# ethanabrooks/hsr-env

Measured on AMD Instinct MI355X. Metric: env-steps/sec (whole node), HSR+1-block, steps_per_action=300, 8192 envs, higher is better.
Workload: dtype f32; 1 GPU; BASELINE config 3: cfg3, all 7 DOFs + 1 block(s), 8192 envs per GPU x 1 GPU(s), steps_per_action=300, geofence=0.05, ctrl~U(ctrlrange) per env-step, done envs reset; envs_per_gpu=8192, global_envs=8192, substeps_per_env_step=300, parallelism=env-shard x1, persistent_kernel=True, hipgraph=False

## Files before the change

### hsr_env_amd/csrc/host_access.h

```cpp

template <typename T>
static int read_drained(hsr_batch *b, T *out, T *src, size_t count, bool clear = false) {
    HIPCHK(hipStreamSynchronize(b->stream));
    HIPCHK(hipMemcpy(out, src, count * sizeof(T), hipMemcpyDeviceToHost));
    if (clear) HIPCHK(hipMemset(src, 0, count * sizeof(T)));
    return HSR_OK;
}
extern "C" int hsr_batch_size(const hsr_batch *b) { ENTER(b); return b->N; }
extern "C" void *hsr_batch_stream(const hsr_batch *b) { return b ? (void *)b->stream : nullptr; }
extern "C" int hsr_batch_sync(hsr_batch *b) { ENTER_DEV(b); HIPCHK(hipStreamSynchronize(b->stream)); return queue_error(b); }
extern "C" int hsr_batch_set_profiling(hsr_batch *b, int on) { ENTER(b); b->profiling = on == 1; b->kernel_log = on == 2; return HSR_OK; }
extern "C" int hsr_batch_kernel_times(hsr_batch *b, float *out_ms, int cap) {
    ENTER_DEV(b);
    HIPCHK(hipStreamSynchronize(b->stream));
    int n = 0;
    for (auto &pr : b->klog) {
        float ms = 0;
        if (hipEventElapsedTime(&ms, pr.first, pr.second) == hipSuccess && out_ms && n < cap) out_ms[n] = ms;
        n++;
        hipEventDestroy(pr.first); hipEventDestroy(pr.second);
    }
    b->klog.clear();
    const int qe = queue_error(b);
    return qe ? qe : n;
}
extern "C" int hsr_batch_set_graph(hsr_batch *b, int on) { ENTER(b); b->use_graph = on != 0; return HSR_OK; }
static void clear_margins(hsr_batch *b) {
    hipLaunchKernelGGL(k_clear_margins, grid1((size_t)b->ds.npair_sep * b->N), dim3(256), 0, b->stream, b->ds);
}
extern "C" int hsr_batch_set_persistent(hsr_batch *b, int on) {
    ENTER(b);
    const bool want = on != 0 && b->kernel;
    if (want && !b->persist) { hipSetDevice(b->device); clear_margins(b); }
    b->persist = want;
    return b->persist ? 1 : 0;
}
extern "C" int hsr_batch_is_persistent(const hsr_batch *b) {
    ENTER(b);
    if (!b->persist) return 0;
    return 1 | (b->const_row >= 0 ? 2 : 0) | (b->kin3 ? 4 : 0);
}
extern "C" int hsr_batch_set_debug(hsr_batch *b, int on) {
    ENTER(b);
    b->debug_store = (on & 1) != 0;
    b->test_hooks = on & (6 | 16 | 32 | 64 | 128);
    return HSR_OK;
}
extern "C" int hsr_batch_set_schedule(hsr_batch *b, int on) { ENTER(b); b->schedule = on != 0; return HSR_OK; }
extern "C" int hsr_batch_set_mpr_warm(hsr_batch *b, int on) {
    ENTER_DEV(b);
    if ((on != 0) != b->mpr_warm) clear_margins(b);
    b->mpr_warm = on != 0;
    return HSR_OK;
}
extern "C" int hsr_batch_set_solo(hsr_batch *b, int servers, float trips) {
    ENTER(b);
    if (servers < 0 || trips < 0.f) return fail(HSR_EINVAL, "hsr_batch_set_solo: servers >= 0, trips >= 0");
    b->solo_servers = servers;
    if (trips > 0.f) b->solo_trips = trips;
    return b->kernel_sv ? HSR_OK : 1;
}
extern "C" int hsr_batch_solo_handovers(hsr_batch *b, int *out) {
    ENTER_DEV(b);
    if (!out) return fail(HSR_EINVAL, "null argument");
    const int rc = read_drained(b, out, b->ds.sq_ctl + 1, 1);
    return rc ? rc : queue_error(b);
}
extern "C" int hsr_batch_set_queue(hsr_batch *b, int mode, int chunk) {
    ENTER(b);
    if (mode < -1 || mode > 1 || chunk < 0) return fail(HSR_EINVAL, "hsr_batch_set_queue: mode -1 / 0 / 1, chunk >= 0");
    b->queue = mode;
    if (chunk > 0) { b->queue_chunk = chunk; b->queue_chunk_set = true; }
    return HSR_OK;
}
extern "C" int hsr_batch_set_goals(hsr_batch *b, int n, const int *body_a, const int *body_b, const float *dist) {
    ENTER_DEV(b);
    if (n < 0 || n > 4 || (n > 0 && (!body_a || !body_b || !dist))) return fail(HSR_EINVAL, "hsr_batch_set_goals: 0..4 terms");
    for (int k = 0; k < n; k++)
        if (body_a[k] < 0 || body_a[k] >= b->dm.nbody || body_b[k] < 0 || body_b[k] >= b->dm.nbody) return fail(HSR_EINVAL, "hsr_batch_set_goals: body id out of range");
    HIPCHK(hipStreamSynchronize(b->stream));
    b->ds.ngoal = n;
    for (int k = 0; k < n; k++) { b->ds.goal_a[k] = body_a[k]; b->ds.goal_b[k] = body_b[k]; b->ds.goal_d[k] = dist[k]; }
    for (auto &kv : b->graphs) hipGraphExecDestroy(kv.second);
    b->graphs.clear();
    return HSR_OK;
}
extern "C" int hsr_batch_cap_counts(hsr_batch *b, unsigned long long *out) {
    ENTER_DEV(b);
    if (!out) return fail(HSR_EINVAL, "null argument");
    const int rc = read_drained(b, out, b->ds.capstat, 4, true);
    return rc ? rc : queue_error(b);
}
extern "C" int hsr_batch_cap_histogram(hsr_batch *b, unsigned long long *out) {
    ENTER_DEV(b);
    if (!out) return fail(HSR_EINVAL, "null argument");
    return read_drained(b, out, b->ds.capstat + 4, 8, true);
}

extern "C" int hsr_batch_newton_trips(hsr_batch *b, int32_t *out) {
    ENTER_DEV(b);
    if (!out) return fail(HSR_EINVAL, "null argument");
    return read_drained(b, out, b->ds.trips, (size_t)b->N);
}
extern "C" int hsr_batch_packing(hsr_batch *b, int32_t *out) {
    ENTER_DEV(b);
    if (!out) return fail(HSR_EINVAL, "null argument");
    if (!b->persist || !b->schedule || !b->d_slot_env) return fail(HSR_EINVAL, "hsr_batch_packing: no packed persistent launch on this batch");
    const int epb = 64 / b->group, slots = (b->N + epb - 1) / epb * epb;
    const int rc = read_drained(b, out, b->d_slot_env, (size_t)slots);
    return rc ? rc : queue_error(b);
}
static int to_device_soa(hsr_batch *b, float *dst, const float *host, int rows) {
    const size_t n = (size_t)rows * b->N;
    if (n > b->stage_floats) return fail(HSR_EINVAL, "staging overflow");
    HIPCHK(hipMemcpyAsync(b->d_stage, host, n * sizeof(float), hipMemcpyHostToDevice, b->stream));
    hipLaunchKernelGGL(k_aos_to_soa, grid1(n), dim3(256), 0, b->stream, dst, (const float *)b->d_stage, rows, b->N);
    HIPCHK(hipStreamSynchronize(b->stream));
    return HSR_OK;
}
static int to_host_aos(hsr_batch *b, float *host, const float *src, int rows) {
    const size_t n = (size_t)rows * b->N;
    if (n > b->stage_floats) return fail(HSR_EINVAL, "staging overflow");
    hipLaunchKernelGGL(k_soa_to_aos, grid1(n), dim3(256), 0, b->stream, b->d_stage, src, rows, b->N, rows, 0);
    return stage_to_host(b, host, b->d_stage, n);
}

extern "C" int hsr_batch_get_state(hsr_batch *b, float *time, float *qpos, float *qvel) {
    ENTER_DEV(b);
    int rc;
    if (time && (rc = to_host_aos(b, time, b->ds.time, 1))) return rc;
    if (qpos && (rc = to_host_aos(b, qpos, b->ds.qpos, b->dm.nq))) return rc;
    if (qvel && (rc = to_host_aos(b, qvel, b->ds.qvel, b->dm.nv))) return rc;
    return queue_error(b);
}
extern "C" int hsr_batch_set_state(hsr_batch *b, const float *time, const float *qpos, const float *qvel) {
    ENTER_DEV(b);
    clear_margins(b);
    int rc;
    if (time && (rc = to_device_soa(b, b->ds.time, time, 1))) return rc;
    if (qpos && (rc = to_device_soa(b, b->ds.qpos, qpos, b->dm.nq))) return rc;
    if (qvel && (rc = to_device_soa(b, b->ds.qvel, qvel, b->dm.nv))) return rc;
    return hsr_batch_forward(b);
}
extern "C" int hsr_batch_set_mocap(hsr_batch *b, const float *mocap) { ENTER_DEV(b); return to_device_soa(b, b->ds.mocap, mocap, 3); }
extern "C" int hsr_batch_set_warmstart(hsr_batch *b, const float *w) { ENTER_DEV(b); return to_device_soa(b, b->ds.warm, w, b->dm.nv); }
extern "C" int hsr_batch_get_warmstart(hsr_batch *b, float *w) { ENTER_DEV(b); return to_host_aos(b, w, b->ds.warm, b->dm.nv); }
extern "C" int hsr_batch_body_xpos(hsr_batch *b, int body_id, float *out) {
    ENTER_DEV(b);
    if (body_id < 0 || body_id >= b->dm.nbody) return fail(HSR_EINVAL, "body id out of range");
    hipLaunchKernelGGL(k_body_xpos, grid1(b->N), dim3(256), 0, b->stream, b->dm, b->ds, body_id, b->d_stage);
    return stage_to_host(b, out, b->d_stage, (size_t)b->N * 3);
}

static int obs_openai_launch(hsr_batch *b, const int *ids, float *d_out) {
    if (!ids) return fail(HSR_EINVAL, "null argument");
    const DevModel &d = b->dm;
    for (int k = 0; k < 3; k++) if (ids[k] < 0 || ids[k] >= d.nbody || b->model->i32("body_mocap")[ids[k]]) return fail(HSR_EINVAL, "obs_openai: bad body id");
    if (ids[3] < 0 || ids[3] >= d.nq || ids[4] < 0 || ids[4] >= d.nq || ids[5] < 0 || ids[5] >= d.nv || ids[6] < 0 || ids[6] >= d.nv)
        return fail(HSR_EINVAL, "obs_openai: bad joint address");
    hipLaunchKernelGGL(k_obs_openai, grid1(b->N), dim3(256), 0, b->stream, b->dm, b->ds, ids[0], ids[1], ids[2], ids[3], ids[4], ids[5], ids[6], d.timestep, d_out);
    HIPCHK(hipGetLastError());
    return HSR_OK;
}
extern "C" int hsr_batch_obs_openai_dev(hsr_batch *b, const int *ids, float *d_out) {
    ENTER_DEV(b);
    return obs_openai_launch(b, ids, d_out);
}
extern "C" int hsr_batch_obs_openai(hsr_batch *b, const int *ids, float *out) {
    ENTER_DEV(b);
    const int rc = obs_openai_launch(b, ids, b->d_stage);
    return rc ? rc : stage_to_host(b, out, b->d_stage, (size_t)b->N * 25);
}

extern "C" int hsr_batch_bad_state(hsr_batch *b, uint8_t *out) {
    ENTER_DEV(b);
    std::vector<int> tmp(b->N);
    const int rc = stage_to_host(b, tmp.data(), b->ds.bad, (size_t)b->N);
    if (rc) return rc;
    int any = 0;
    for (int i = 0; i < b->N; i++) { out[i] = (uint8_t)(tmp[i] != 0); any |= tmp[i]; }
    const int qe = queue_error(b);
    return qe ? qe : (any ? HSR_EBADSTATE : HSR_OK);
}

extern "C" int hsr_batch_get_field(hsr_batch *b, int field, float *out) {
    ENTER_DEV(b);
    const DevModel &d = b->dm;
    const size_t N = b->N;
    switch (field) {
    case HSR_F_XPOS: return to_host_aos(b, out, b->ds.xpos, 3 * d.nlink);
    case HSR_F_XMAT: return to_host_aos(b, out, b->ds.xmat, 9 * d.nlink);
    case HSR_F_QACC: return to_host_aos(b, out, b->ds.qacc, d.nv);
    case HSR_F_QACC_SMOOTH: return to_host_aos(b, out, b->ds.qacc_smooth, d.nv);
    case HSR_F_QFRC_SMOOTH: return to_host_aos(b, out, b->ds.qfrc_smooth, d.nv);
    case HSR_F_QFRC_CONSTRAINT: return to_host_aos(b, out, b->ds.qfrc_constraint, d.nv);
    case HSR_F_M:
        hipLaunchKernelGGL(k_expand_M, grid1(N), dim3(256), 0, b->stream, b->ds, b->d_stage, d.nv);
        return stage_to_host(b, out, b->d_stage, N * d.nv * d.nv);
    case HSR_F_NCON: case HSR_F_NEFC: case HSR_F_NITER: {
        const int *src = field == HSR_F_NCON ? b->ds.ncon : (field == HSR_F_NEFC ? b->ds.nefc : b->ds.niter);
        hipLaunchKernelGGL(k_i32_to_f32, grid1(N), dim3(256), 0, b->stream, b->d_stage, src, N);
        return stage_to_host(b, out, b->d_stage, N); }
    case HSR_F_CONTACT:
        hipLaunchKernelGGL(k_contacts_out, grid1(N), dim3(256), 0, b->stream, b->dm, b->ds, b->d_stage);
        return stage_to_host(b, out, b->d_stage, N * d.nslot * 7);
    default: return fail(HSR_EINVAL, "unknown field");
    }
}

extern "C" int hsr_batch_phase_cycles(hsr_batch *b, unsigned long long *out ) {
    ENTER_DEV(b);
    return read_drained(b, out, b->ds.phase_cyc, 32, true);
}

extern "C" int hsr_batch_block_times(hsr_batch *b, unsigned long long *out, int nblocks) {
    ENTER_DEV(b);
    if (nblocks > 8192) nblocks = 8192;
    if (nblocks < 0) return read_drained(b, out, b->ds.phase_cyc + 32 + 40 * 4096, (size_t)2 * 8192, true);
// ... 10 lines not shown
```

### hsr_env_amd/csrc/host_batch.h

```cpp
static_assert(HSR_GEOM_MESH == GEOM_MESH, "host_model.h restates model.h's GEOM_MESH");

#define HIPCHK(x) do { hipError_t e_ = (x); if (e_ != hipSuccess) return fail(HSR_EDEVICE, "HIP error: %s", hipGetErrorString(e_)); } while (0)
#define ENTER(b) do { if (!(b)) return fail(HSR_EINVAL, "null batch"); } while (0)
#define ENTER_DEV(b) do { ENTER(b); HIPCHK(hipSetDevice((b)->device)); } while (0)

typedef void (*persist_fn)(const DevModel *, DevState, int, int, float, int, StepIO);
struct GraphKey {
    int nsub, goal_body; float geofence; int cap_every, cap_n; const void *cap;
    bool operator<(const GraphKey &o) const { return std::tie(nsub, goal_body, geofence, cap_every, cap_n, cap) < std::tie(o.nsub, o.goal_body, o.geofence, o.cap_every, o.cap_n, o.cap); }
};

struct CreateSwitches {
    bool no_const = false;
    int nfb_max = 1 << 30;
    bool tables_lds = false;
    bool debug = false;
};

struct hsr_batch {
    const hsr_model *model = nullptr;
    CreateSwitches sw;
    int N = 0, device = 0;
    hipStream_t stream = nullptr;
    DevModel dm{};
    DevModel *d_dm = nullptr;
    DevState ds{};
    std::vector<void *> allocs;
    float *d_qpos0 = nullptr;
    float *d_stage = nullptr;
    size_t stage_floats = 0;
    uint8_t *d_stage_u8 = nullptr;
    int32_t *d_stage_i32 = nullptr;
    int narrow_blocks = 2048;
    int pairs_per_wave = 4;
    int group = 16;
    size_t mf_lds_bytes = 0;
    bool persist = false;
    bool use_graph = true, profiling = false, debug_store = false;
    int const_row = -1;
    bool kin3 = false;
    bool persist_tg = false;
    persist_fn kernel = nullptr;
    persist_fn kernel_sv = nullptr;
    size_t persist_lds_bytes = 0;
    bool mpr_warm = true;
    int test_hooks = 0;
    bool schedule = true;
    int *d_slot_env = nullptr;
    std::map<GraphKey, hipGraphExec_t> graphs;
    float last_total_ms = 0, last_kernel_ms[3] = {0, 0, 0};
    int last_launches[3] = {0, 0, 0};
    hipEvent_t ev0 = nullptr, ev1 = nullptr;
    std::vector<hipEvent_t> kev;
    int slots = 0;
    int queue = -1;
    int queue_chunk = 20;
    bool queue_chunk_set = false;
    int solo_servers = 0;
    float solo_trips = 3.5f;
    bool kernel_log = false;
    std::vector<std::pair<hipEvent_t, hipEvent_t>> klog;
    float4 *d_planes = nullptr;
    int2 *d_prange = nullptr;
    float4 *d_rgba = nullptr;
    std::vector<float> rgba_host;
    void *d_rimg = nullptr;
    size_t rimg_bytes = 0;
    int cap_every = 0, cap_n = 0;
    CaptureDesc *d_cap_desc = nullptr;
    int *d_cap_slot = nullptr;
    int *d_cap_env = nullptr;
    int *d_cap_cnt = nullptr;
    float *d_cap = nullptr;
    size_t cap_floats = 0;
    int cap_rows = 0;
    EpisodeDev ep{};
    bool ep_set = false;
    float *d_ep_range = nullptr;
    int *d_ep_block_qadr = nullptr;
    std::vector<hsr_snapshot *> snapshots;
    hsr_snapshot *fork_scratch = nullptr;
    SnapTable snap_tab{};
    bool snap_tab_built = false;
    std::vector<hsr_replay *> replays;
    std::vector<hsr_rollout *> rollouts;
};
static void snap_release_all(hsr_batch *b);
static void replay_release_all(hsr_batch *b);
static void rollout_release_all(hsr_batch *b);
template <typename T>
static int dalloc(hsr_batch *b, T **p, size_t count) {
    void *q = nullptr;
    HIPCHK(hipMalloc(&q, (count ? count : 1) * sizeof(T)));
    HIPCHK(hipMemset(q, 0, (count ? count : 1) * sizeof(T)));
    b->allocs.push_back(q);
    *p = (T *)q;
    return HSR_OK;
}
template <typename D, typename T>
static int upload(hsr_batch *b, D *dst, const T *src, size_t count, size_t pad = 0) {
    T *d;
    const int rc = dalloc(b, &d, count + pad);
    if (rc) return rc;
    if (count) HIPCHK(hipMemcpy(d, src, count * sizeof(T), hipMemcpyHostToDevice));
    *dst = (D)d;
    return HSR_OK;
}
template <typename D, typename T>
static int upload(hsr_batch *b, D *dst, const std::vector<T> &v, size_t pad = 0) { return upload(b, dst, v.data(), v.size(), pad); }
template <typename T>
static int stage_to_host(hsr_batch *b, T *host, const T *d_src, size_t count) {
    HIPCHK(hipMemcpyAsync(host, d_src, count * sizeof(T), hipMemcpyDeviceToHost, b->stream));
    HIPCHK(hipStreamSynchronize(b->stream));
    return HSR_OK;
}
template <typename F>
static auto by_group(int group, F f) { return group == 16 ? f(std::integral_constant<int, 16>()) : f(std::integral_constant<int, 32>()); }
static int upload_capture_desc(hsr_batch *b, int every, int n) {
    const CaptureDesc cd{b->d_cap, b->d_cap_slot, every, n};
    HIPCHK(hipMemcpy(b->d_cap_desc, &cd, sizeof cd, hipMemcpyHostToDevice));
    return HSR_OK;
}
static int require_captured_step(const hsr_batch *b, const char *who) {
    if (b->cap_every <= 0 || b->cap_rows <= 0) return fail(HSR_EINVAL, "%s: no captured step (hsr_batch_set_capture, then a step)", who);
    return HSR_OK;
}
enum { QUEUE_ROUNDS = 64 };
static inline dim3 grid1(size_t n, int t = 256) { return dim3((unsigned)((n + t - 1) / t)); }
static int queue_error(hsr_batch *b) {
    int err = 0;
    if (b->ds.q_err && hipMemcpy(&err, b->ds.q_err, sizeof err, hipMemcpyDeviceToHost) == hipSuccess && err) {
        hipMemset(b->ds.q_err, 0, sizeof err);
        return fail(HSR_EDEVICE, "persistent kernel: a work-queue ticket was never served (launch drained by its watchdog)");
    }
    return HSR_OK;
}
```

### hsr_env_amd/csrc/host_create.h

```cpp

static void read_switches(hsr_batch *b) {
    auto env = [](const char *name) { const char *v = getenv(name); return v ? v : ""; };
    auto is0 = [&](const char *name) { return strcmp(env(name), "0") == 0; };
    auto set = [&](const char *name) { return getenv(name) != nullptr; };
    b->sw.no_const = set("HSR_NO_CONST") && !is0("HSR_NO_CONST");
    if (set("HSR_NFB")) b->sw.nfb_max = std::max(atoi(env("HSR_NFB")), 0);
    b->sw.tables_lds = is0("HSR_TABLES_GLOBAL");
    b->sw.debug = set("HSR_DEBUG");
    if (set("HSR_SOLO")) b->solo_servers = atoi(env("HSR_SOLO"));
    if (atof(env("HSR_SOLO_TRIPS")) > 0) b->solo_trips = (float)atof(env("HSR_SOLO_TRIPS"));
    if (set("HSR_QUEUE")) b->queue = atoi(env("HSR_QUEUE")) != 0;
    if (atoi(env("HSR_QUEUE_CHUNK")) > 0) b->queue_chunk = atoi(env("HSR_QUEUE_CHUNK"));
    b->queue_chunk_set = atoi(env("HSR_QUEUE_CHUNK")) > 0;
    if (set("HSR_MPR_WARM")) b->mpr_warm = atoi(env("HSR_MPR_WARM")) != 0;
    b->schedule = !is0("HSR_SCHEDULE");
    if (atoi(env("HSR_NARROW_BLOCKS")) > 0) b->narrow_blocks = atoi(env("HSR_NARROW_BLOCKS"));
    if (atoi(env("HSR_PPW")) > 0) b->pairs_per_wave = atoi(env("HSR_PPW"));
}

struct PersistInstance {
    int row;
    int group, nv;
    bool tg;
    persist_fn fn, sv;
};
static const PersistInstance kPersistInstances[] = {
#ifdef HSR_DEV_CFG3
    {2, 16, -1, false, k_env_step_mf<16, 13, true, 7, false, DevModel_cfg3>, k_env_step_mf<16, 13, true, 7, false, DevModel_cfg3, true>},
#else
    {0, 16, -1, false, k_env_step_mf<16, 2, true, 0, false, DevModel_cfg1>, nullptr},
    {1, 16, -1, false, k_env_step_mf<16, 8, true, 0, false, DevModel_cfg2>, k_env_step_mf<16, 8, true, 0, false, DevModel_cfg2, true>},
    {2, 16, -1, false, k_env_step_mf<16, 13, true, 7, false, DevModel_cfg3>, k_env_step_mf<16, 13, true, 7, false, DevModel_cfg3, true>},
    {3, 32, -1, false, k_env_step_mf<32, 25, true, 7, false, DevModel_cfg4>, nullptr},
    {3, 32, -1, true, k_env_step_mf<32, 25, true, 7, true, DevModel_cfg4>, nullptr},
    {4, 16, -1, false, k_env_step_mf<16, 13, true, -1, false, DevModel_cupboard>, k_env_step_mf<16, 13, true, -1, false, DevModel_cupboard, true>},
    {4, 16, -1, true, k_env_step_mf<16, 13, true, -1, true, DevModel_cupboard>, k_env_step_mf<16, 13, true, -1, true, DevModel_cupboard, true>},
    {-1, 16, 13, false, k_env_step_mf<16, 13, true>, nullptr},
    {-1, 16, -1, false, k_env_step_mf<16, 16, false>, nullptr},
    {-1, 32, -1, false, k_env_step_mf<32, 32, false>, nullptr},
#endif
};
static const PersistInstance *find_instance(int row, int group, int nv, bool tg) {
    for (const PersistInstance &p : kPersistInstances)
        if (p.row == row && p.group == group && (p.nv < 0 || p.nv == nv) && p.tg == tg) return &p;
    return nullptr;
}
static void quat2mat_h(const double *q, float *mt) {
    double n = sqrt(q[0]*q[0] + q[1]*q[1] + q[2]*q[2] + q[3]*q[3]);
    double w = q[0]/n, x = q[1]/n, y = q[2]/n, z = q[3]/n;
    mt[0] = (float)(1 - 2*(y*y + z*z)); mt[1] = (float)(2*(x*y - w*z)); mt[2] = (float)(2*(x*z + w*y));
    mt[3] = (float)(2*(x*y + w*z)); mt[4] = (float)(1 - 2*(x*x + z*z)); mt[5] = (float)(2*(y*z - w*x));
    mt[6] = (float)(2*(x*z - w*y)); mt[7] = (float)(2*(y*z + w*x)); mt[8] = (float)(1 - 2*(x*x + y*y));
}
static int cfg_const_row(const hsr_batch *b, const hsr_model *m, const DevModel &d) {
    if (b->sw.no_const) return -1;
    int iv[sizeof kCfgConsts[0].i / sizeof(int)]; float fv[sizeof kCfgConsts[0].f / sizeof(float)];
    cfg_const_values(d, iv, fv);
    int r = 0;
    const int nrows = (int)(sizeof kCfgConsts / sizeof kCfgConsts[0]);
    while (r < nrows && !(memcmp(iv, kCfgConsts[r].i, sizeof iv) == 0 && memcmp(fv, kCfgConsts[r].f, sizeof fv) == 0)) r++;
    if (r == nrows) return -1;
    const Kin3Check &k = kKin3Checks[r];
    if (!k.i) return r;
    std::vector<int> ti = {d.nlink, d.nv};
    for (const char *n : {"link_parent", "link_free", "link_dofadr", "link_dofnum", "link_qposadr", "dof_type", "dof_qposadr", "dof_link"}) {
        size_t cnt = 0; const int *p = m->i32(n, &cnt);
        ti.insert(ti.end(), p, p + cnt);
    }
    std::vector<float> tf;
    auto addf = [&](const char *n) { size_t cnt = 0; const double *p = m->f64(n, &cnt); for (size_t i = 0; i < cnt; i++) tf.push_back((float)p[i]); };
    addf("link_pos");
    { size_t cnt = 0; const double *q = m->f64("link_quat", &cnt); for (size_t i = 0; i < cnt / 4; i++) { float mt[9]; quat2mat_h(q + 4 * i, mt); tf.insert(tf.end(), mt, mt + 9); } }
    for (const char *n : {"link_com", "link_inertia", "link_mass", "dof_axis", "dof_pos"}) addf(n);
    return k.ni == (int)ti.size() && k.nf == (int)tf.size() && memcmp(k.i, ti.data(), ti.size() * sizeof(int)) == 0
           && memcmp(k.f, tf.data(), tf.size() * sizeof(float)) == 0 ? r : -1;
}
static int upload_f(hsr_batch *b, const float **dst, const hsr_model *m, const char *name) {
    size_t cnt = 0;
    const double *src = m->f64(name, &cnt);
    if (!src) return fail(HSR_EBLOB, "blob entry '%s' missing", name);
    std::vector<float> tmp(cnt ? cnt : 1, 0.f);
    for (size_t i = 0; i < cnt; i++) tmp[i] = (float)src[i];
    return upload(b, dst, tmp);
}
static int upload_i(hsr_batch *b, const int **dst, const hsr_model *m, const char *name) {
    size_t cnt = 0;
    const int *src = m->i32(name, &cnt);
    if (!src) return fail(HSR_EBLOB, "blob entry '%s' missing", name);
    return upload(b, dst, src, cnt, 16);
}
static int upload_mats(hsr_batch *b, const float **dst, const hsr_model *m, const char *quat_name) {
    size_t cnt = 0;
    const double *q = m->f64(quat_name, &cnt);
    if (!q) return fail(HSR_EBLOB, "blob entry '%s' missing", quat_name);
    size_t n = cnt / 4;
    std::vector<float> tmp(n * 9 + 1);
    for (size_t i = 0; i < n; i++) quat2mat_h(q + 4 * i, tmp.data() + 9 * i);
    return upload(b, dst, tmp);
}

static int trailing_free_bodies(const hsr_batch *b, const hsr_model *m) {
    const DevModel &d = b->dm;
    const int *dn = m->i32("link_dofnum"), *lf = m->i32("link_free"), *da = m->i32("link_dofadr"), *dt = m->i32("dof_type"), *dl = m->i32("dof_link");
    int nfb = 0;
    for (int k = 0; 6 * (k + 1) <= d.nv; k++) {
        const int a0 = d.nv - 6 * (k + 1), l = dl[a0];
        bool fb = l > 0 && lf[l] && da[l] == a0 && dn[l] == 6;
        for (int j = 0; fb && j < 6; j++) fb = dl[a0 + j] == l && dt[a0 + j] == (j < 3 ? DOF_FREE_LIN : DOF_FREE_ANG);
        if (!fb) break;
        nfb++;
    }
    if (nfb * 28 * (64 / b->group) > 4 * 48) nfb = 0;
    return std::min(nfb, b->sw.nfb_max);
}
static int stage_hulls(hsr_batch *b, const hsr_model *m) {
    DevModel &d = b->dm;
    const int *gl = m->i32("geom_link"), *gt = m->i32("geom_type"), *ma = m->i32("geom_meshadr"), *mn = m->i32("geom_meshnum"), *lp = m->i32("link_parent");
    std::vector<int> ldsv(std::max(d.ngeom, 1), -1), src;
    if (b->kin3) {
        const int budget = KIN2_FLOATS * d.nlink / 4;
        auto depth = [&](int l) { int k = 0; while (l > 0) { l = lp[l]; k++; } return k; };
        std::vector<int> order;
        for (int g = 0; g < d.ngeom; g++) if (gt[g] == GEOM_MESH && gl[g] > 0 && mn[g] > 0) order.push_back(g);
        std::stable_sort(order.begin(), order.end(), [&](int a, int bb) { const int da = depth(gl[a]), db = depth(gl[bb]); return da != db ? da > db : mn[a] < mn[bb]; });
        for (int g : order) if ((int)src.size() + mn[g] <= budget) { ldsv[g] = (int)src.size(); for (int k = 0; k < mn[g]; k++) src.push_back(ma[g] + k); }
    }
    d.nldsv = (int)src.size();
    const int rc = upload(b, &d.geom_ldsv, ldsv);
    return rc ? rc : upload(b, &d.ldsv_src, src, 1);
}
static bool fits_persist(const hsr_batch *b, const hsr_model *m) {
    const DevModel &d = b->dm;
    const int G = b->group;
    bool ok = d.nq <= G && d.nv <= G && d.nlink <= G && d.nlink <= NLMAX && d.ngeom <= 64 && d.npair < (1 << 14) && d.maxdepth <= 9;
    {
        const int *dp = m->i32("dof_parent");
        for (int c = 0; ok && c < d.nv; c++) { int depth = 0; for (int k = c; k >= 0 && depth <= 10; k = dp[k]) depth++; if (depth > 10) ok = false; }
    }
    {
        const int *dn = m->i32("link_dofnum"), *lf = m->i32("link_free"), *lp = m->i32("link_parent"), *gl = m->i32("geom_link");
        for (int l = 1; l < d.nlink; l++) {
            if (!lf[l] && dn[l] > 3) ok = false;
            if (lf[l] && lp[l] != 0) ok = false;
            if (lf[lp[l]]) ok = false;
        }
        for (int gi = d.nstatic_geom; gi < d.ngeom; gi++) if (gl[gi] == 0) ok = false;
    }
    return ok && b->persist_lds_bytes <= 160 * 1024;
}
static int plan_persist(hsr_batch *b, const hsr_model *m) {
    DevModel &d = b->dm;
    const int G = b->group;
    auto layout = [&](auto g, bool tg) {
        return PersistLayout<decltype(g)::value>(d.njmax, b->ds.kstride, d.npair_pad, d.nlink, d.ngeom, d.nstatic_geom, tg);
    };
    d.nfb = trailing_free_bodies(b, m);
    int row = cfg_const_row(b, m, d);
    if (row >= 0 && kKin3Checks[row].i) {
        const int *lf = m->i32("link_free"), *dl = m->i32("dof_link");
        int nrd = 0;
        for (int k = 0; k < d.nv; k++) nrd += lf[dl[k]] ? 0 : 1;
        const int stage = 12 * d.nv + ((nrd + 3) & ~3) * nrd;
        const int region = by_group(G, [&](auto g) { return layout(g, false).oCnt; });
        if (stage > region) row = -1;
    }
    b->const_row = row;
    b->kin3 = row >= 0 && kKin3Checks[row].i;
    const int rc = stage_hulls(b, m);
    if (rc) return rc;
    auto lds_total = [&](bool tg) { return (size_t)sizeof(float) * by_group(G, [&](auto g) { return layout(g, tg).total; }); };
    const PersistInstance *in_lds = find_instance(row, G, d.nv, false), *in_global = find_instance(row, G, d.nv, true);
    hipFuncAttributes fa;
    b->persist_tg = in_lds && in_global && !b->sw.tables_lds
                    && hipFuncGetAttributes(&fa, (const void *)in_lds->fn) == hipSuccess && lds_total(false) + fa.sharedSizeBytes > 20480
                    && hipFuncGetAttributes(&fa, (const void *)in_global->fn) == hipSuccess && lds_total(true) + fa.sharedSizeBytes <= 20480;
    b->persist_lds_bytes = lds_total(b->persist_tg);
    const PersistInstance *inst = b->persist_tg ? in_global : in_lds;
    if (!fits_persist(b, m) || !inst) { d.nfb = 0; return HSR_OK; }
    b->kernel = inst->fn;
    b->kernel_sv = inst->sv;
    b->persist = true;
    for (persist_fn f : {b->kernel, b->kernel_sv})
        if (f && b->persist_lds_bytes > 48 * 1024) HIPCHK(hipFuncSetAttribute((const void *)f, hipFuncAttributeMaxDynamicSharedMemorySize, (int)b->persist_lds_bytes));
    int pb = -1;
    hipDeviceProp_t prop;
    if (hipOccupancyMaxActiveBlocksPerMultiprocessor(&pb, b->kernel, 64, b->persist_lds_bytes) == hipSuccess && pb > 0
        && hipGetDeviceProperties(&prop, b->device) == hipSuccess) b->slots = pb * prop.multiProcessorCount;
    if (b->sw.debug && hipFuncGetAttributes(&fa, (const void *)b->kernel) == hipSuccess)
        fprintf(stderr, "[hsrsim] k_env_step_mf<%d>: regs %d, static LDS %zu, dyn LDS %zu, scratch %zu -> %d workgroups per CU\n", G, fa.numRegs, fa.sharedSizeBytes, b->persist_lds_bytes, fa.localSizeBytes, pb);
    return HSR_OK;
}

static int upload_model(hsr_batch *b, const hsr_model *m) {
    DevModel &d = b->dm;
    const int *sz = m->sizes;
    d.nq = sz[HSR_NQ]; d.nv = sz[HSR_NV]; d.nu = sz[HSR_NU]; d.nlink = sz[HSR_NLINK]; d.nbody = sz[HSR_NBODY];
    d.ngeom = sz[HSR_NGEOM]; d.npair = sz[HSR_NPAIR]; d.nslot = sz[HSR_NSLOT]; d.nconmax = sz[HSR_NCONMAX]; d.njmax = sz[HSR_NJMAX];
    if (d.npair > 384) return fail(HSR_EINVAL, "more than 384 candidate geom pairs");
    if (d.ngeom > 255) return fail(HSR_EINVAL, "more than 255 geoms");
    d.nM = d.nv * (d.nv + 1) / 2;
    d.ndense = sz[13];
    d.timestep = (float)m->opt[0]; d.impratio = (float)m->opt[1]; d.gravz = (float)m->opt[2]; d.tolerance = (float)m->opt[3];
    d.iterations = (int)m->opt[4]; d.ls_iterations = (int)m->opt[5]; d.ls_tolerance = (float)m->opt[6];
    d.mpr_tolerance = (float)m->opt[7]; d.mpr_iterations = (int)m->opt[8]; d.meaninertia = (float)m->opt[9];
    int rc = 0;
#define UI(f) if ((rc = upload_i(b, &d.f, m, #f))) { return rc; }
#define UF(f) if ((rc = upload_f(b, &d.f, m, #f))) { return rc; }
    UI(link_parent) UI(link_dofadr) UI(link_dofnum) UI(link_qposadr) UI(link_free)
    UF(link_pos) UF(link_mass) UF(link_com) UF(link_inertia) UI(link_dofmask)
    UI(dof_link) UI(dof_type) UI(dof_parent) UI(dof_qposadr) UI(dof_limited)
    UF(dof_axis) UF(dof_pos) UF(dof_damping) UF(dof_invweight0) UF(dof_range) UF(dof_solref) UF(dof_solimp)
    UI(body_link) UI(body_mocap) UF(body_pos)
    UI(geom_type) UI(geom_link) UI(geom_meshadr) UI(geom_meshnum)
    UF(geom_pos) UF(geom_size) UF(geom_rbound) UF(geom_invweight) UF(mesh_vert) UF(geom_aabb)
    UI(pair_geom1) UI(pair_geom2) UI(pair_fn) UI(pair_condim) UI(pair_slot)
    UF(pair_friction) UF(pair_solref) UF(pair_solimp)
    UI(act_dof) UF(act_gear) UF(act_kp) UF(act_ctrlrange) UF(act_forcerange)
#undef UI
#undef UF
    return HSR_OK;
}
static int derive_pair_rec(hsr_batch *b, const hsr_model *m) {
    DevModel &d = b->dm;
    const int *g1 = m->i32("pair_geom1"), *g2 = m->i32("pair_geom2"), *cd = m->i32("pair_condim"), *gl = m->i32("geom_link"), *ad = m->i32("act_dof");
    const double *fr = m->f64("pair_friction"), *sr = m->f64("pair_solref"), *si = m->f64("pair_solimp"), *iw = m->f64("geom_invweight");
    std::vector<float> rec((size_t)std::max(d.npair, 1) * 16, 0.f);
    for (int p = 0; p < d.npair; p++) {
        float *r = rec.data() + 16 * p;
        r[0] = (float)cd[p]; r[1] = (float)gl[g1[p]]; r[2] = (float)gl[g2[p]]; r[3] = (float)(iw[2 * g1[p]] + iw[2 * g2[p]]);
        for (int j = 0; j < 5; j++) r[4 + j] = (float)fr[5 * p + j];
        const double dmax = std::min(std::max(si[5 * p + 1], (double)HSR_MINIMP), (double)HSR_MAXIMP), tc = sr[2 * p], dr = sr[2 * p + 1];
        r[9] = (float)(2.0 / (dmax * tc)); r[10] = (float)(1.0 / (dmax * dmax * tc * tc * dr * dr));
        for (int j = 0; j < 5; j++) r[11 + j] = (float)si[5 * p + j];
    }
    std::vector<int> da(std::max(d.nv, 1), -1);
    for (int a = 0; a < d.nu; a++) da[ad[a]] = a;
    const int rc = upload(b, &d.pair_rec, rec);
    return rc ? rc : upload(b, &d.dof_act, da);
}
static int derive_collision_recs(hsr_batch *b, const hsr_model *m) {
    DevModel &d = b->dm;
    const int *g1 = m->i32("pair_geom1"), *g2 = m->i32("pair_geom2"), *fn = m->i32("pair_fn"), *sl = m->i32("pair_slot");
    const int *gl = m->i32("geom_link"), *gt = m->i32("geom_type"), *ma = m->i32("geom_meshadr"), *mn = m->i32("geom_meshnum");
    const double *gp = m->f64("geom_pos"), *gq = m->f64("geom_quat"), *gs = m->f64("geom_size"), *gb = m->f64("geom_aabb"), *gr = m->f64("geom_rbound");
    std::vector<float> rec((size_t)std::max(d.npair, 1) * 8, 0.f), grec((size_t)std::max(d.ngeom, 1) * 32, 0.f);
    for (int p = 0; p < d.npair; p++) {
        float *r = rec.data() + 8 * p;
        r[0] = (float)(g1[p] + 256 * (gt[g1[p]] == GEOM_PLANE ? 1 : 0)); r[1] = (float)g2[p]; r[2] = (float)gr[g1[p]]; r[3] = (float)gr[g2[p]];
        r[4] = (float)fn[p]; r[5] = (float)sl[p]; r[6] = (float)(sl[p + 1] - sl[p]); r[7] = (float)gt[g1[p]];
    }
    for (int gg = 0; gg < d.ngeom; gg++) {
        float *o = grec.data() + 32 * gg, lm[9];
        quat2mat_h(gq + 4 * gg, lm);
        o[0] = (float)gl[gg]; o[1] = (float)gt[gg]; o[2] = (float)mn[gg]; o[3] = (float)ma[gg];
        for (int k = 0; k < 3; k++) o[4 + k] = (float)gp[3 * gg + k];
        o[7] = (float)gr[gg];
        for (int k = 0; k < 9; k++) o[8 + k] = lm[k];
        for (int k = 0; k < 3; k++) o[17 + k] = (float)gs[3 * gg + k];
        for (int k = 0; k < 3; k++) { o[20 + k] = (float)gb[6 * gg + k]; o[24 + k] = (float)gb[6 * gg + 3 + k]; }
    }
    const int rc = upload(b, &d.pair_geo, rec);
    return rc ? rc : upload(b, &d.geom_rec, grec);
}
static int derive_tables(hsr_batch *b, const hsr_model *m) {
    DevModel &d = b->dm;
    int rc = 0;
    {
        const int *lp = m->i32("link_parent");
        std::vector<int> dep(std::max(d.nlink, 1), 0);
        d.maxdepth = 0;
        for (int l = 1; l < d.nlink; l++) { dep[l] = dep[lp[l]] + 1; d.maxdepth = std::max(d.maxdepth, dep[l]); }
        if ((rc = upload(b, &d.link_depth, dep))) return rc;
    }
    {
        size_t cnt = 0;
        const double *mv = m->f64("mesh_vert", &cnt);
        const size_t nvt = cnt / 3;
        std::vector<float> v4((nvt + 1) * 4, 0.f);
        for (size_t i = 0; i < nvt; i++) for (int k = 0; k < 3; k++) v4[4 * i + k] = (float)mv[3 * i + k];
        if ((rc = upload(b, &d.mesh_vert4, v4))) return rc;
        const int *mn = m->i32("geom_meshnum");
        for (int g = 0; g < d.ngeom; g++) if (mn[g] > 256) return fail(HSR_EINVAL, "mesh hull with more than 256 vertices");
    }
    {
        const int *gl = m->i32("geom_link");
        d.nstatic_geom = 0;
        while (d.nstatic_geom < d.ngeom && gl[d.nstatic_geom] == 0) d.nstatic_geom++;
    }
    d.npair_pad = (d.npair + 7) & ~7;
    if (d.npair_pad == 0) d.npair_pad = 8;
    if ((rc = derive_pair_rec(b, m)) || (rc = derive_collision_recs(b, m))) return rc;
    if ((rc = upload_mats(b, &d.link_mat, m, "link_quat"))) return rc;
    if ((rc = upload_mats(b, &d.geom_mat, m, "geom_quat"))) return rc;
    if ((rc = upload_mats(b, &d.body_mat, m, "body_quat"))) return rc;
    d.any_damping = 0;
    { size_t cnt; const double *dmp = m->f64("dof_damping", &cnt); for (size_t i = 0; i < cnt; i++) if (dmp[i] > 0) d.any_damping = 1; }
    d.solimp_general = 0;
    for (const char *nm : {"dof_solimp", "pair_solimp"}) {
        size_t cnt; const double *si = m->f64(nm, &cnt);
        for (size_t i = 4; si && i < cnt; i += 5) { const double pw = si[i] < 1 ? 1 : si[i]; if (pw != 1 && pw != 2) d.solimp_general = 1; }
    }
    d.cv_types = 0;
    {
        const int *g1 = m->i32("pair_geom1"), *g2 = m->i32("pair_geom2"), *fn = m->i32("pair_fn"), *gt = m->i32("geom_type");
        for (int p = 0; p < d.npair; p++) if (fn[p] == FN_CONVEX) d.cv_types |= (1 << (gt[g1[p]] & 7)) | (256 << (gt[g2[p]] & 7));
    }
    return HSR_OK;
}
static int alloc_state(hsr_batch *b) {
    const DevModel &d = b->dm;
    DevState &s = b->ds;
    const size_t N = (size_t)b->N;
    int rc = 0;
    s.N = b->N;
    s.npair_sep = std::max(d.npair, 1);
#define DA(field, rows) if ((rc = dalloc(b, &s.field, (size_t)(rows) * N))) return rc;
    DA(qpos, d.nq) DA(qvel, d.nv) DA(ctrl, d.nu) DA(mocap, 3) DA(warm, d.nv) DA(time, 1)
    DA(done, 1) DA(bad, 1) DA(nsteps, 1)
    DA(xpos, 3 * d.nlink) DA(xmat, 9 * d.nlink) DA(lvel, 6 * d.nlink)
    s.kstride = (9 * d.nv + 15 * d.nlink + 15) & ~15;
    DA(kin_aos, s.kstride)
    DA(con, 8 * d.nslot) DA(ncon_pair, d.npair_pad) DA(sepax, 4 * std::max(d.npair, 1)) DA(septick, std::max(d.npair, 1)) DA(tick, 1) DA(pair_list, std::max(d.npair, 1))
    if ((rc = dalloc(b, &s.pair_count, (size_t)d.npair_pad))) return rc;
    if ((rc = dalloc(b, &s.pair_pack, (size_t)((d.npair_pad + 7) & ~7)))) return rc;
    if ((rc = dalloc(b, &s.geom_c, (size_t)8 * std::max(d.ngeom, 1)))) return rc;
    DA(M, d.nM) DA(qacc, d.nv) DA(qacc_smooth, d.nv) DA(qfrc_smooth, d.nv) DA(qfrc_constraint, d.nv)
    DA(ncon, 1) DA(nefc, 1) DA(niter, 1)
#undef DA
    if ((rc = dalloc(b, &s.phase_cyc, 32 + 40 * 8192))) return rc;
    if ((rc = dalloc(b, &s.capstat, 12))) return rc;
    if ((rc = dalloc(b, &s.trips, N))) return rc;
    if ((rc = dalloc(b, &b->d_slot_env, N + 64))) return rc;
    const size_t tasks = (N + 1) / 2;
    if ((rc = dalloc(b, &s.q_head, QUEUE_ROUNDS))) return rc;
    if ((rc = dalloc(b, &s.q_wpos, QUEUE_ROUNDS))) return rc;
    if ((rc = dalloc(b, &s.q_items, (size_t)QUEUE_ROUNDS * tasks))) return rc;
    if ((rc = dalloc(b, &s.q_err, 1))) return rc;
    s.sq_cap = (int)N + 4096;
    if ((rc = dalloc(b, &s.sq_items, (size_t)s.sq_cap))) return rc;
    if ((rc = dalloc(b, &s.sq_ctl, 4))) return rc;
    s.solo_servers = 0; s.solo_trips_x4 = 14; s.solo_min_left = 40;
    s.q_chunk = 0;
    s.slot_env = nullptr;
    return HSR_OK;
}
static int size_solver(hsr_batch *b) {
    const DevModel &d = b->dm;
    b->group = d.nv <= 16 ? 16 : 32;
    if (d.nv > 32 || d.nq > 64 || d.nlink > NLMAX || d.nconmax > b->group || b->ds.kstride > 8 * 4 * b->group)
        return fail(HSR_EINVAL, "model exceeds the lane-group solver (nv <= 32, nlink <= 16, nconmax <= lanes per env)");
    const int total = by_group(b->group, [&](auto g) { return MfLayout<decltype(g)::value>(d.njmax, b->ds.kstride).total; });
    b->mf_lds_bytes = (size_t)total * (64 / b->group) * sizeof(float);
    if (b->mf_lds_bytes > 160 * 1024) return fail(HSR_EINVAL, "model exceeds the LDS budget of the solver");
    if (b->mf_lds_bytes <= 48 * 1024) return HSR_OK;
    const void *fn = by_group(b->group, [](auto g) { return (const void *)k_solve_mf<decltype(g)::value>; });
    HIPCHK(hipFuncSetAttribute(fn, hipFuncAttributeMaxDynamicSharedMemorySize, (int)b->mf_lds_bytes));
    return HSR_OK;
}
static int size_kinematics(hsr_batch *b) {
    const size_t kb = (size_t)64 * (b->ds.kstride + 24 * b->dm.nlink + 1) * sizeof(float);
    if (kb > 160 * 1024) return fail(HSR_EINVAL, "kinematics tile exceeds LDS");
    if (kb > 48 * 1024) HIPCHK(hipFuncSetAttribute((const void *)k_kinematics, hipFuncAttributeMaxDynamicSharedMemorySize, (int)kb));
    return HSR_OK;
}
static int alloc_staging_and_reset(hsr_batch *b, const hsr_model *m) {
    const DevModel &d = b->dm;
    const size_t N = (size_t)b->N;
    int rc = 0;
    b->stage_floats = N * (size_t)(std::max(std::max(std::max(d.nq + d.nv, 25), 7 * d.nslot), std::max(d.nv * d.nv, 9 * d.nlink)) + d.nu + d.nq + d.nv + 4) + 16;
    if ((rc = dalloc(b, &b->d_stage, b->stage_floats))) return rc;
    if ((rc = dalloc(b, &b->d_stage_u8, N))) return rc;
    if ((rc = dalloc(b, &b->d_stage_i32, N))) return rc;
    HIPCHK(hipEventCreate(&b->ev0));
    HIPCHK(hipEventCreate(&b->ev1));
    if ((rc = upload(b, &b->d_qpos0, m->qpos0.data(), (size_t)d.nq))) return rc;
    hipLaunchKernelGGL(k_build_tables, grid1((size_t)std::max(d.ngeom, (d.npair_pad + 7) & ~7)), dim3(256), 0, b->stream, b->dm, b->ds);
    hipLaunchKernelGGL(k_reset, grid1(N), dim3(256), 0, b->stream, b->dm, b->ds, (const uint8_t *)nullptr, (const float *)nullptr,
                       (const float *)b->d_qpos0, (const float *)nullptr, 0);
    HIPCHK(hipStreamSynchronize(b->stream));
    return HSR_OK;
}

static int batch_init(hsr_batch *b, const hsr_model *m) {
    int rc;
    HIPCHK(hipStreamCreateWithFlags(&b->stream, hipStreamNonBlocking));
    if ((rc = upload_model(b, m)) || (rc = derive_tables(b, m)) || (rc = alloc_state(b)) || (rc = size_solver(b))) return rc;
    if ((rc = plan_persist(b, m)) || (rc = size_kinematics(b))) return rc;
    return alloc_staging_and_reset(b, m);
}
extern "C" int hsr_batch_create(const hsr_model *m, int n_envs, int device_id, hsr_batch **out) {
    if (!m || !out || n_envs <= 0) return fail(HSR_EINVAL, "bad arguments to hsr_batch_create");
    int ndev = 0;
    if (hipGetDeviceCount(&ndev) != hipSuccess || ndev <= 0) return fail(HSR_EDEVICE, "no HIP device available%s");
    if (device_id < 0 || device_id >= ndev) return fail(HSR_EINVAL, "device id out of range");
    HIPCHK(hipSetDevice(device_id));
    hsr_batch *b = new hsr_batch();
    b->model = m; b->N = n_envs; b->device = device_id;
    read_switches(b);
    const int rc = batch_init(b, m);
    if (rc) { hsr_batch_destroy(b); return rc; }
    *out = b;
    return HSR_OK;
}

extern "C" void hsr_batch_destroy(hsr_batch *b) {
    if (!b) return;
    hipSetDevice(b->device);
    if (b->stream) hipStreamSynchronize(b->stream);
    for (auto &kv : b->graphs) hipGraphExecDestroy(kv.second);
    snap_release_all(b);
    replay_release_all(b);
    rollout_release_all(b);
    for (void *p : b->allocs) hipFree(p);
    if (b->d_rimg) hipFree(b->d_rimg);
    if (b->d_cap) hipFree(b->d_cap);
    for (hipEvent_t ev : b->kev) hipEventDestroy(ev);
    for (auto &pr : b->klog) { hipEventDestroy(pr.first); hipEventDestroy(pr.second); }
    if (b->ev0) hipEventDestroy(b->ev0);
    if (b->ev1) hipEventDestroy(b->ev1);
    if (b->stream) hipStreamDestroy(b->stream);
    delete b;
}
```

### hsr_env_amd/csrc/host_step.h

```cpp

static void launch_substep(hsr_batch *b, int mode, int goal_body, float geofence, int debug, hipStream_t st, bool timed, int sub = -1) {
    const int N = b->N;
    auto rec = [&](void) { if (timed) { hipEvent_t ev; hipEventCreate(&ev); hipEventRecord(ev, st); b->kev.push_back(ev); } };
    rec();
    hipLaunchKernelGGL(k_kinematics, dim3((N + 63) / 64), dim3(64), (size_t)64 * (b->ds.kstride + 24 * b->dm.nlink + 1) * sizeof(float), st, b->dm, b->ds);
    if (sub >= 0 && b->cap_every > 0 && sub % b->cap_every == 0)
        hipLaunchKernelGGL(k_capture, grid1((size_t)12 * b->dm.nlink * b->cap_n), dim3(256), 0, st, b->ds, b->dm.nlink, (const int *)b->d_cap_env, b->cap_n, b->d_cap,
                           sub / b->cap_every, 1, b->cap_every, (int *)nullptr);
    rec();
    if (b->dm.npair > 0) {
        hipLaunchKernelGGL(k_cull, dim3((N + 63) / 64, (b->dm.npair + b->pairs_per_wave - 1) / b->pairs_per_wave), dim3(64), 0, st, b->dm, b->ds);
        hipLaunchKernelGGL(k_narrow, dim3(b->narrow_blocks), dim3(64), 0, st, b->dm, b->ds);
    }
    rec();
    by_group(b->group, [&](auto g) {
        hipLaunchKernelGGL(k_solve_mf<decltype(g)::value>, dim3((N * g() + 63) / 64), dim3(64), b->mf_lds_bytes, st, b->dm, b->ds,
                           mode, goal_body, geofence, debug);
    });
    rec();
}

extern "C" int hsr_batch_forward(hsr_batch *b) {
    ENTER_DEV(b);
    hipLaunchKernelGGL(k_clear_done, grid1(b->N), dim3(256), 0, b->stream, b->ds);
    launch_substep(b, 0, -1, 0.f, 1, b->stream, false);
    HIPCHK(hipGetLastError());
    HIPCHK(hipStreamSynchronize(b->stream));
    return HSR_OK;
}

extern "C" int hsr_batch_reset(hsr_batch *b, const uint8_t *mask, const float *qpos0, const float *mocap) {
    ENTER_DEV(b);
    const size_t N = b->N;
    const int nq = b->dm.nq;
    float *d_q = nullptr, *d_m = nullptr, *d_q0m = b->d_qpos0;
    size_t off = 0;
    if (qpos0) { d_q = b->d_stage + off; off += N * nq; HIPCHK(hipMemcpyAsync(d_q, qpos0, N * nq * sizeof(float), hipMemcpyHostToDevice, b->stream)); }
    if (mocap) { d_m = b->d_stage + off; off += N * 3; HIPCHK(hipMemcpyAsync(d_m, mocap, N * 3 * sizeof(float), hipMemcpyHostToDevice, b->stream)); }
    if (off > b->stage_floats) return fail(HSR_EINVAL, "staging overflow in reset");
    if (mask) HIPCHK(hipMemcpyAsync(b->d_stage_u8, mask, N, hipMemcpyHostToDevice, b->stream));
    hipLaunchKernelGGL(k_reset, grid1(N), dim3(256), 0, b->stream, b->dm, b->ds, mask ? (const uint8_t *)b->d_stage_u8 : (const uint8_t *)nullptr,
                       (const float *)d_q, (const float *)d_q0m, (const float *)d_m, mask ? 1 : 0);
    launch_substep(b, 0, -1, 0.f, 1, b->stream, false);
    hipLaunchKernelGGL(k_clear_done, grid1(N), dim3(256), 0, b->stream, b->ds);
    HIPCHK(hipGetLastError());
    HIPCHK(hipStreamSynchronize(b->stream));
    return HSR_OK;
}

extern "C" int hsr_batch_reset_dev(hsr_batch *b, const uint8_t *d_mask, const float *d_qpos0, const float *d_mocap) {
    ENTER_DEV(b);
    const size_t N = b->N;
    hipLaunchKernelGGL(k_reset, grid1(N), dim3(256), 0, b->stream, b->dm, b->ds, d_mask, d_qpos0, (const float *)b->d_qpos0, d_mocap, 1);
    launch_substep(b, 0, -1, 0.f, 0, b->stream, false);
    hipLaunchKernelGGL(k_clear_done, grid1(N), dim3(256), 0, b->stream, b->ds);
    HIPCHK(hipGetLastError());
    return HSR_OK;
}
static int grow_capture(hsr_batch *b, int cap_rows) {
    const size_t need = (size_t)cap_rows * 12 * b->dm.nlink * b->cap_n;
    if (need <= b->cap_floats) return HSR_OK;
    HIPCHK(hipStreamSynchronize(b->stream));
    if (b->d_cap) { HIPCHK(hipFree(b->d_cap)); b->d_cap = nullptr; b->cap_floats = 0; }
    HIPCHK(hipMalloc(&b->d_cap, need * sizeof(float)));
    HIPCHK(hipMemsetD32Async((hipDeviceptr_t)b->d_cap, 0x7fc00000, need, b->stream));
    b->cap_floats = need;
    return upload_capture_desc(b, b->cap_every, b->cap_n);
}

struct PersistLaunch {
    int tasks, grid;
    int chunk, rounds;
    int solo_servers, solo_trips_x4, solo_min_left;
};
static PersistLaunch plan_launch(int N, int group, int slots, int n_substeps, int queue, int queue_chunk, bool queue_chunk_set,
                                 int solo_servers, float solo_trips, bool has_sv, bool schedule) {
    PersistLaunch p{};
    const int epb = 64 / group, T = (N + epb - 1) / epb;
    int chunk = queue_chunk;
    if (!queue_chunk_set && slots > 0 && T >= 4 * slots) chunk = 50;
    while ((n_substeps + chunk - 1) / chunk > QUEUE_ROUNDS) chunk *= 2;
    const bool solo = has_sv && solo_servers > 0 && solo_servers <= 4096 && schedule && slots > 0 && n_substeps >= 3 * chunk && n_substeps < 2048 && N <= (1 << 20)
                      && (T + solo_servers <= slots || 4 * solo_servers <= slots);
    const bool qon = slots > 0 && n_substeps >= 2 * chunk && (solo || queue == 1 || (queue < 0 && T > slots));
    p.tasks = T;
    p.grid = T;
    p.chunk = chunk;
    if (qon) {
        p.rounds = (n_substeps + chunk - 1) / chunk;
        p.grid = T < slots ? T : slots;
        if (solo) {
            p.solo_servers = solo_servers;
            p.solo_trips_x4 = (int)(4.f * solo_trips + 0.5f);
            p.solo_min_left = 2 * chunk;
            p.grid = std::min(slots, T + solo_servers);
        }
    }
    return p;
}

static int launch_persistent(hsr_batch *b, const StepIO &io, int n_substeps, int goal_body, float geofence) {
    hipStream_t st = b->stream;
    if (b->profiling) { hipEvent_t ev; for (int k = 0; k < 3; k++) { hipEventCreate(&ev); hipEventRecord(ev, st); b->kev.push_back(ev); } }
    if (!b->d_dm) {
        const int rc = upload(b, &b->d_dm, &b->dm, 1);
        if (rc) return rc;
    }
    if (b->schedule)
        hipLaunchKernelGGL(k_schedule, dim3((b->N + SCHED_CHUNK - 1) / SCHED_CHUNK), dim3(1024), 0, st, b->ds, 64 / b->group, b->d_slot_env);
    const PersistLaunch p = plan_launch(b->N, b->group, b->slots, n_substeps, b->queue, b->queue_chunk, b->queue_chunk_set,
                                        b->solo_servers, b->solo_trips, b->kernel_sv != nullptr, b->schedule);
    DevState dsl = b->ds;
    dsl.slot_env = b->schedule ? b->d_slot_env : nullptr;
    dsl.solo_servers = p.solo_servers;
    if (p.solo_servers > 0) { dsl.solo_trips_x4 = p.solo_trips_x4; dsl.solo_min_left = p.solo_min_left; }
    if (p.rounds > 0) {
        dsl.q_chunk = p.chunk;
        hipLaunchKernelGGL(k_queue_init, grid1((size_t)p.rounds * p.tasks), dim3(256), 0, st, dsl, p.tasks, p.rounds);
    }
    hipEvent_t k0 = nullptr, k1 = nullptr;
    if (b->kernel_log) { hipEventCreate(&k0); hipEventCreate(&k1); hipEventRecord(k0, st); }
    const int debug = (b->debug_store ? 1 : 0) | (b->test_hooks & ~32) | (b->mpr_warm ? 0 : 8);
    hipLaunchKernelGGL(p.solo_servers > 0 ? b->kernel_sv : b->kernel, dim3(p.grid), dim3(64), b->persist_lds_bytes, st,
                       (const DevModel *)b->d_dm, dsl, n_substeps, goal_body, geofence, debug, io);
    if ((b->test_hooks & 32) && b->ds.q_err) HIPCHK(hipMemsetD32Async((hipDeviceptr_t)b->ds.q_err, 1, 1, st));
    if (b->kernel_log) { hipEventRecord(k1, st); b->klog.push_back({k0, k1}); }
    if (b->profiling) { hipEvent_t ev; hipEventCreate(&ev); hipEventRecord(ev, st); b->kev.push_back(ev); }
    return HSR_OK;
}
static int launch_chain(hsr_batch *b, int n_substeps, int goal_body, float geofence) {
    hipStream_t st = b->stream;
    if (!b->use_graph || b->profiling || n_substeps <= 0) {
        for (int i = 0; i < n_substeps; i++) launch_substep(b, 1, goal_body, geofence, 0, st, b->profiling, i);
        return HSR_OK;
    }
    GraphKey key{n_substeps, goal_body, geofence, b->cap_every, b->cap_n, b->d_cap};
    auto it = b->graphs.find(key);
    if (it == b->graphs.end()) {
        hipGraph_t graph;
        HIPCHK(hipStreamBeginCapture(st, hipStreamCaptureModeThreadLocal));
        for (int i = 0; i < n_substeps; i++) launch_substep(b, 1, goal_body, geofence, 0, st, false, i);
        HIPCHK(hipStreamEndCapture(st, &graph));
        hipGraphExec_t exec;
        HIPCHK(hipGraphInstantiate(&exec, graph, nullptr, nullptr, 0));
        hipGraphDestroy(graph);
        if (b->graphs.size() >= 8) { for (auto &kv : b->graphs) hipGraphExecDestroy(kv.second); b->graphs.clear(); }
        it = b->graphs.emplace(key, exec).first;
    }
    HIPCHK(hipGraphLaunch(it->second, st));
    return HSR_OK;
}
static int finish_profiling(hsr_batch *b) {
    HIPCHK(hipEventRecord(b->ev1, b->stream));
    HIPCHK(hipEventSynchronize(b->ev1));
    HIPCHK(hipEventElapsedTime(&b->last_total_ms, b->ev0, b->ev1));
    for (int k = 0; k < 3; k++) { b->last_kernel_ms[k] = 0; b->last_launches[k] = 0; }
    for (size_t i = 0; i + 3 < b->kev.size(); i += 4)
        for (int k = 0; k < 3; k++) { float ms = 0; hipEventElapsedTime(&ms, b->kev[i + k], b->kev[i + k + 1]); b->last_kernel_ms[k] += ms; b->last_launches[k]++; }
    return HSR_OK;
}

extern "C" int hsr_batch_step_dev(hsr_batch *b, const float *d_ctrl, int n_substeps, int goal_body, float geofence,
                                  float *d_obs, float *d_reward, uint8_t *d_done, int32_t *d_nsteps) {
    ENTER_DEV(b);
    if (!d_ctrl || n_substeps < 0) return fail(HSR_EINVAL, "bad arguments to hsr_batch_step");
    if (goal_body >= b->dm.nbody) return fail(HSR_EINVAL, "goal body out of range");
    const int N = b->N;
    hipStream_t st = b->stream;
    int rc;
    if (b->profiling) {
        for (hipEvent_t ev : b->kev) hipEventDestroy(ev);
        b->kev.clear();
        HIPCHK(hipEventRecord(b->ev0, st));
    }
    const int cap_rows = b->cap_every > 0 ? (n_substeps > 0 ? (n_substeps - 1) / b->cap_every + 1 : 0) + 1 : 0;
    if (cap_rows > 0 && (rc = grow_capture(b, cap_rows))) return rc;
    if (b->persist && n_substeps > 0) {
        const StepIO io{d_ctrl, d_obs, d_reward, d_done, d_nsteps, b->cap_every > 0 ? b->d_cap_desc : nullptr};
        if ((rc = launch_persistent(b, io, n_substeps, goal_body, geofence))) return rc;
    } else {
        hipLaunchKernelGGL(k_begin_step, grid1(N), dim3(256), 0, st, b->ds, d_ctrl, b->dm.nu);
        if ((rc = launch_chain(b, n_substeps, goal_body, geofence))) return rc;
        if (d_obs) {
            const int nq = b->dm.nq, nv = b->dm.nv;
            hipLaunchKernelGGL(k_soa_to_aos, grid1((size_t)nq * N), dim3(256), 0, st, d_obs, (const float *)b->ds.qpos, nq, N, nq + nv, 0);
            hipLaunchKernelGGL(k_soa_to_aos, grid1((size_t)nv * N), dim3(256), 0, st, d_obs, (const float *)b->ds.qvel, nv, N, nq + nv, nq);
        }
        hipLaunchKernelGGL(k_end_step, grid1(N), dim3(256), 0, st, b->ds, d_reward, d_done, d_nsteps);
    }
    if (cap_rows > 0)
        hipLaunchKernelGGL(k_capture, grid1((size_t)12 * b->dm.nlink * b->cap_n), dim3(256), 0, st, b->ds, b->dm.nlink, (const int *)b->d_cap_env, b->cap_n, b->d_cap,
                           cap_rows - 1, 0, b->cap_every, b->d_cap_cnt);
    b->cap_rows = cap_rows;
    HIPCHK(hipGetLastError());
    return b->profiling ? finish_profiling(b) : HSR_OK;
}

extern "C" int hsr_batch_step(hsr_batch *b, const float *ctrl, int n_substeps, int goal_body, float geofence,
                              float *obs, float *reward, uint8_t *done, int32_t *nsteps) {
    ENTER_DEV(b);
    if (!ctrl) return fail(HSR_EINVAL, "bad arguments to hsr_batch_step");
    const size_t N = b->N;
    const int nu = b->dm.nu, no = b->dm.nq + b->dm.nv;
    if (N * (size_t)(nu + no + 1) > b->stage_floats) return fail(HSR_EINVAL, "staging overflow in step");
    float *d_ctrl = b->d_stage, *d_obs = b->d_stage + N * nu, *d_rew = d_obs + N * no;
    HIPCHK(hipMemcpyAsync(d_ctrl, ctrl, N * nu * sizeof(float), hipMemcpyHostToDevice, b->stream));
    int rc = hsr_batch_step_dev(b, d_ctrl, n_substeps, goal_body, geofence, obs ? d_obs : nullptr, reward ? d_rew : nullptr,
                                done ? b->d_stage_u8 : nullptr, nsteps ? b->d_stage_i32 : nullptr);
    if (rc) return rc;
    if (obs) HIPCHK(hipMemcpyAsync(obs, d_obs, N * no * sizeof(float), hipMemcpyDeviceToHost, b->stream));
    if (reward) HIPCHK(hipMemcpyAsync(reward, d_rew, N * sizeof(float), hipMemcpyDeviceToHost, b->stream));
    if (done) HIPCHK(hipMemcpyAsync(done, b->d_stage_u8, N, hipMemcpyDeviceToHost, b->stream));
    if (nsteps) HIPCHK(hipMemcpyAsync(nsteps, b->d_stage_i32, N * sizeof(int32_t), hipMemcpyDeviceToHost, b->stream));
    HIPCHK(hipStreamSynchronize(b->stream));
    return queue_error(b);
}
```

### hsr_env_amd/csrc/hsrsim.hip

```cpp
#include <hip/hip_runtime.h>
#include <math.h>
#include <algorithm>
#include <stdio.h>
#include <stdlib.h>
#include <string.h>

#include <map>
#include <string>
#include <tuple>
#include <type_traits>
#include <vector>

#include "../../include/hsrsim.h"
#include "collide.h"
#include "model.h"
#include "solve_g.h"
#include "solve_mf.h"
#include "persist.h"
#include "render.h"
#include "episode.h"
#include "snapshot.h"
#include "replay.h"
#include "replay_prio.h"
#include "rollout.h"
#include "cfg_consts.h"

#include "host_model.h"
#include "host_batch.h"
#include "util_kernels.h"
#include "host_create.h"
#include "host_step.h"
#include "host_episode.h"
#include "host_access.h"
#include "host_render.h"
#include "host_snapshot.h"
#include "host_replay.h"
#include "host_rollout.h"
```

### hsr_env_amd/csrc/model.h

```cpp
#pragma once
#include <stdint.h>
#include <hip/hip_runtime.h>

enum { DOF_SLIDE = 0, DOF_HINGE = 1, DOF_FREE_LIN = 2, DOF_FREE_ANG = 3 };
enum { GEOM_PLANE = 0, GEOM_SPHERE = 2, GEOM_CYLINDER = 5, GEOM_BOX = 6, GEOM_MESH = 7 };
enum { FN_PLANE_BOX = 0, FN_PLANE_CONVEX = 1, FN_BOX_BOX = 2, FN_CONVEX = 3 };

struct DevModel {
    int nq, nv, nu, nlink, nbody, ngeom, npair, nslot, nconmax, njmax, nM, ndense;
    float timestep, impratio, gravz, tolerance, ls_tolerance, mpr_tolerance, meaninertia;
    int iterations, ls_iterations, mpr_iterations, any_damping;
    int solimp_general;
    int cv_types;
    const int *link_parent, *link_dofadr, *link_dofnum, *link_qposadr, *link_free;
    const float *link_pos, *link_mat, *link_mass, *link_com, *link_inertia;
    const int *link_dofmask, *link_depth;
    int maxdepth;
    const int *dof_link, *dof_type, *dof_parent, *dof_qposadr, *dof_limited;
    const float *dof_axis, *dof_pos, *dof_damping, *dof_invweight0, *dof_range, *dof_solref, *dof_solimp;
    const int *body_link, *body_mocap;
    const float *body_pos, *body_mat;
    const int *geom_type, *geom_link, *geom_meshadr, *geom_meshnum;
    const float *geom_pos, *geom_mat, *geom_size, *geom_rbound, *geom_invweight, *mesh_vert;
    const float *geom_aabb;
    const float4 *mesh_vert4;
    const int *pair_geom1, *pair_geom2, *pair_fn, *pair_condim, *pair_slot;
    const float *pair_friction, *pair_solref, *pair_solimp;
    const int *act_dof, *dof_act;
    const float *pair_rec;
    const float *pair_geo;
    const float *geom_rec;
    int npair_pad;
    int nstatic_geom;
    int nfb;
    const float *act_gear, *act_kp, *act_ctrlrange, *act_forcerange;
    const int *geom_ldsv;
    const int *ldsv_src;
    int nldsv;
};

struct CaptureDesc { float *cap; const int *slot; int every, R; };
struct StepIO { const float *ctrl; float *obs, *reward; uint8_t *done; int32_t *nsteps; const CaptureDesc *cap; };

struct DevState {
    int N;
    float *qpos, *qvel, *ctrl, *mocap, *warm, *time;
    int *done, *bad, *nsteps;
    float *xpos, *xmat;
    float *lvel;
    float *kin_aos;
    int kstride;
    float *con;
    int *ncon_pair;
    int *pair_count, *pair_list;
    float *sepax;
    int npair_sep;
    int *septick, *tick;
    unsigned *pair_pack;
    float *geom_c;
    float *M, *qacc, *qacc_smooth, *qfrc_smooth, *qfrc_constraint;
    int *ncon, *nefc, *niter;
    int ngoal, goal_a[4], goal_b[4];
    float goal_d[4];
    int *slot_env, *trips;
    int q_chunk;
    int *q_head, *q_wpos, *q_items, *q_err;
    int solo_servers, solo_trips_x4, solo_min_left, sq_cap;
    int *sq_items, *sq_ctl;
    unsigned long long *capstat;
    unsigned long long *phase_cyc;
};
```

### hsr_env_amd/csrc/persist.h

```cpp
#pragma once
#include "collide.h"
#include "kin2.h"
#include "kin3.h"
#include "solve_mf.h"

template <int G> struct PersistLayout {
    int R, MS, oRows, oCnt, oB, envf, oPoly, oKin, oPair, oGeomC, oGeomS, oLinkTab, total;
    __host__ __device__ PersistLayout(int rows, int kstride, int npair_pad, int nlink, int ngeom, int nstatic, bool tables_global = false) {
        R = rows; MS = G + 1;
        int a = 5 * R > kstride ? 5 * R : kstride;
        oRows = 0; oCnt = (a + 3) & ~3;
        a = oCnt + (npair_pad + 3) / 4;
        int b = G * MS > C2_SIZE * G ? G * MS : C2_SIZE * G;
        const int nmov = ngeom - nstatic;
        const int kin_tmp = 24 * nlink + 2 * G + (16 * nmov > 8 * G ? 16 * nmov : 8 * G);
        if (kin_tmp > b) b = kin_tmp;
        oB = (a + 3) & ~3;
        envf = (oB + b + 3) & ~3;
        oPoly = envf * (64 / G);
        oKin = oPoly + 4 * 48;
        oPair = oKin + KIN2_FLOATS * nlink;
        oGeomC = oPair + (tables_global ? 0 : ((npair_pad + 7) & ~7));
        oGeomS = oGeomC + (tables_global ? 0 : 8 * ngeom);
        oLinkTab = oGeomS + 16 * nstatic;
        total = (oLinkTab + 2 * nlink + 3) & ~3;
    }
};

__device__ __forceinline__ bool q_claim(const DevState &s, int T, int R, int &rlo, int &task, int &round) {
    int t = -1, r = rlo;
    if (threadIdx.x == 0) {
        int h = 0;
        for (; r < R; r++) {
            if (__hip_atomic_load(&s.q_head[r], __ATOMIC_RELAXED, __HIP_MEMORY_SCOPE_AGENT) >= T) continue;
            h = __hip_atomic_fetch_add(&s.q_head[r], 1, __ATOMIC_RELAXED, __HIP_MEMORY_SCOPE_AGENT);
            if (h < T) break;
        }
        if (r < R) {
            const int *slot = s.q_items + (size_t)r * T + h;
            int spins = 0;
            while ((t = __hip_atomic_load(slot, __ATOMIC_RELAXED, __HIP_MEMORY_SCOPE_AGENT)) < 0) {
                __builtin_amdgcn_s_sleep(16);
                if (++spins > (1 << 22) || __hip_atomic_load(s.q_err, __ATOMIC_RELAXED, __HIP_MEMORY_SCOPE_AGENT) != 0) {
                    __hip_atomic_store(s.q_err, 1, __ATOMIC_RELAXED, __HIP_MEMORY_SCOPE_AGENT);
                    t = -1; r = R;
                    break;
                }
            }
        }
    }
    t = __builtin_amdgcn_readfirstlane(t); r = __builtin_amdgcn_readfirstlane(r);
    rlo = r;
    if (t < 0) return false;
    __builtin_amdgcn_fence(__ATOMIC_ACQUIRE, "agent");
    task = t; round = r;
    return true;
}
__device__ __forceinline__ void q_push(const DevState &s, int T, int task, int round, bool last) {
    __builtin_amdgcn_fence(__ATOMIC_RELEASE, "agent");
    __builtin_amdgcn_wave_barrier();
    if (threadIdx.x == 0 && !last) {
        const int p = __hip_atomic_fetch_add(&s.q_wpos[round + 1], 1, __ATOMIC_RELAXED, __HIP_MEMORY_SCOPE_AGENT);
        __hip_atomic_store(s.q_items + (size_t)(round + 1) * T + p, task, __ATOMIC_RELEASE, __HIP_MEMORY_SCOPE_AGENT);
    }
    if (threadIdx.x == 0 && last && s.sq_ctl) __hip_atomic_fetch_add(&s.sq_ctl[3], 1, __ATOMIC_RELEASE, __HIP_MEMORY_SCOPE_AGENT);
}

template <int G, int NVT, bool EXACT, int NDT = -1, bool TG = false, class MT = DevModel, bool SV = false>
__global__ void __launch_bounds__(64, 2) k_env_step_mf(const DevModel *__restrict__ mp, DevState s, int n_substeps, int goal_body, float geofence, int flags, StepIO io) {
    const MT &m = *static_cast<const MT *>(mp);
    extern __shared__ __align__(16) float lds[];
    constexpr int EPB = 64 / G, NK = NVT, NDK = EXACT ? NDT : -1;
    const PersistLayout<G> L(m.njmax, (9 * (EXACT ? NVT : m.nv) + 15 * m.nlink + 15) & ~15, m.npair_pad, m.nlink, m.ngeom, m.nstatic_geom, TG);
    const int tid0 = threadIdx.x;
    const int N = s.N, nv = EXACT ? NVT : m.nv, nq = m.nq, R = L.R, MS = L.MS;
    const int mode = 1, debug = 0;
    const bool dbg_store = flags & 1;
    const bool hook_jv_per_contact = flags & 2, hook_majorant = flags & 4;
    const bool hook_dense_chol = flags & 128;
    constexpr bool EXACT_CT = EXACT && !std::is_same<MT, DevModel>::value;
    const bool hook_no_item_list = flags & 64;
    const bool hook_ignore_stamps = flags & 16;
    const bool mpr_warm = !(flags & 8);
    int cap_con = 0, cap_row = 0, cap_item = 0, nsub_run = 0;
    int own_trips = 0;
    int task = s.q_chunk ? 0 : blockIdx.x, q_round = 0, q_rlo = 0;
    constexpr bool SOLO = false, REP = false;
    const int solo_env = -1;
    (void)solo_env;
#define PERSIST_LANE_VIEW(TID)                                                                                              \
    const int tid = (TID), g = tid / G, c = tid % G;                                                                         \
    const int e_raw = SOLO ? ((REP || g == 0) ? solo_env : -1) : (s.slot_env ? s.slot_env[task * EPB + g] : task * EPB + g); \
    const bool in_range = e_raw >= 0 && e_raw < N;                                                                           \
    const int e = in_range ? e_raw : 0;                                                                                      \
    float *E = lds + (size_t)g * L.envf;                                                                                     \
    float *rD = E + L.oRows, *rAref = rD + R, *rJar = rAref + R, *rJv = rJar + R, *rDw = rJv + R;            \
    float *kAng = E + L.oRows, *kLin = kAng + 3 * nv, *kAnc = kAng + 6 * nv, *lk = kAng + 9 * nv;                            \
    unsigned char *pcnt = reinterpret_cast<unsigned char *>(E + L.oCnt);                                                                       \
    float *M = E + L.oB, *con = E + L.oB;                                                                                    \
                                            \
    float *poseL = E + L.oB, *recL = poseL + 12 * m.nlink, *qposL = recL + 12 * m.nlink, *qvelL = qposL + G; \
    float *poly = lds + L.oPoly;                                                                                             \
    const bool isdof = c < nv;                                                                                               \
    (void)rD; (void)rAref; (void)rJar; (void)rJv; (void)rDw; (void)kLin; (void)kAnc; (void)lk; (void)pcnt; (void)M; (void)con; \
    (void)poseL; (void)recL; (void)qvelL; (void)poly; (void)isdof; (void)e; (void)in_range;
    int bad_acc = 0, trips_acc = 0;
    (void)q_rlo;
    __shared__ signed char sParent[32];
    int *sMask = reinterpret_cast<int *>(lds + L.oLinkTab);
    float *sMass = lds + L.oLinkTab + m.nlink;
    __shared__ unsigned short sItems[64 * (64 / G)];
    __shared__ unsigned char sMpr[64];
#ifdef HSR_PHASE_TIMING
    __shared__ int sDbg[4];
    if (tid0 < 4) sDbg[tid0] = 0;
#endif
    if (tid0 < nv) sParent[tid0] = (signed char)m.dof_parent[tid0];
    if (tid0 < m.nlink && tid0 < NLMAX) { sMask[tid0] = m.link_dofmask[tid0]; sMass[tid0] = m.link_mass[tid0]; }
    __shared__ unsigned char sDofLink[32];
    __shared__ int sEnv[64 / G];
    __shared__ int sTick[64 / G];
    if (tid0 < nv) sDofLink[tid0] = (unsigned char)m.dof_link[tid0];
    constexpr bool KIN3_INST = Kin3Of<MT>::type::ok && EXACT;
    const float4 *ldsv = reinterpret_cast<const float4 *>(lds + L.oKin);
    if constexpr (KIN3_INST) { for (int i = tid0; i < m.nldsv; i += 64) reinterpret_cast<float4 *>(lds + L.oKin)[i] = m.mesh_vert4[m.ldsv_src[i]]; }
    else if (tid0 < m.nlink) kin2_store(m, tid0, lds + L.oKin + KIN2_FLOATS * tid0);
    for (int gi = tid0; gi < m.ngeom; gi += 64) {
        if constexpr (!TG) { geom_consts_store(m.geom_rec + 32 * gi, lds + L.oGeomC + 8 * gi); if (KIN3_INST && m.geom_ldsv[gi] >= 0) hull_lds_patch(lds + L.oGeomC + 8 * gi, m.geom_ldsv[gi]); }
        if (gi < m.nstatic_geom) {
            m3 I3;
#pragma unroll
            for (int k = 0; k < 9; k++) I3.a[k] = (k % 4 == 0) ? 1.f : 0.f;
            geom_place3(geom_place_consts(m.geom_rec + 32 * gi), I3, mk3(0, 0, 0), lds + L.oGeomS + 16 * gi);
        }
    }
    if constexpr (!TG) for (int p = tid0; p < ((m.npair_pad + 7) & ~7); p += 64) {
        unsigned pk = 0;
        if (p < m.npair) {
            const float4 a = reinterpret_cast<const float4 *>(m.pair_geo)[2 * p], b = reinterpret_cast<const float4 *>(m.pair_geo)[2 * p + 1];
            const int code = (int)a.x;
            pk = pair_pack(code & 255, (int)a.y, (int)b.x, (code >> 8) ? a.w : a.z + a.w);
        }
        reinterpret_cast<unsigned *>(lds + L.oPair)[p] = pk;
    }

    float qpos_c = 0, qvel_c = 0, warm_c = 0;
    bool done;
    v3 goal;
    float time_e;
    int nsteps_e = 0;
    float my_ctrl = 0, damp_c = 0;
    int my_type = -1, my_qadr = 0, my_quat_lane = -1, my_limited = 0, my_act = -1;
    float act_p[6] = {0, 0, 0, 0, 0, 0};
    unsigned sub_c = 0;
    unsigned long long anc_c = 0;
    {
        PERSIST_LANE_VIEW(tid0)
        if (isdof) {
            for (int l = 1; l < m.nlink && l < 32; l++) sub_c |= ((unsigned)(m.link_dofmask[l] >> c) & 1u) << l;
            int sh = 0;
            for (int k = c; k >= 0 && sh < 60; k = m.dof_parent[k], sh += 6) anc_c |= (unsigned long long)(k + 1) << sh;
            my_type = m.dof_type[c]; my_qadr = m.dof_qposadr[c]; my_limited = m.dof_limited[c]; my_act = m.dof_act[c];
            my_quat_lane = m.link_dofadr[m.dof_link[c]] + 3;
            damp_c = m.dof_damping[c];
            if (my_act >= 0) {
                act_p[0] = m.act_kp[my_act]; act_p[1] = m.act_gear[my_act];
                act_p[2] = m.act_ctrlrange[2 * my_act]; act_p[3] = m.act_ctrlrange[2 * my_act + 1];
                act_p[4] = m.act_forcerange[2 * my_act]; act_p[5] = m.act_forcerange[2 * my_act + 1];
            }
        }
    }
    const int goal_link = (goal_body >= 0 && !m.body_mocap[goal_body]) ? m.body_link[goal_body] : -1;
    const v3 goal_off = goal_body >= 0 ? ld3(m.body_pos, goal_body) : mk3(0, 0, 0);
    PHASE_T0();

  constexpr bool HAS_SOLO = SV && EXACT && G == 16 && !std::is_same<MT, DevModel>::value;
  auto run_task = [&](auto solo_c, const int sub0, const int sub1, const int solo_env) {
    constexpr bool SOLO = decltype(solo_c)::value;
    constexpr bool REP = SOLO;
    (void)solo_env;
    const bool first_run = sub0 == 0, last_run = sub1 >= n_substeps;
    const bool fresh = io.ctrl != nullptr && first_run;
    cap_con = cap_row = cap_item = nsub_run = own_trips = 0; bad_acc = trips_acc = 0; nsteps_e = 0;
    int run_trips = 0;
    int nitems = 0;
    int trunc_mask = 0;
    bool list_ok = false;
    float acc_move = 0.f;
    {
        PERSIST_LANE_VIEW(tid0)
        if (c == 0) { sEnv[g] = e; sTick[g] = s.tick[e]; }
        done = !in_range || (fresh ? false : s.done[e] != 0);
        qpos_c = 0; qvel_c = 0; warm_c = 0;
        if (c < nq) qpos_c = s.qpos[(size_t)c * N + e];
        if (isdof) { qvel_c = s.qvel[(size_t)c * N + e]; warm_c = s.warm[(size_t)c * N + e]; }
        goal = mk3(s.mocap[e], s.mocap[N + e], s.mocap[2 * N + e]);
        time_e = s.time[e];
        if (isdof && my_act >= 0) {
            if (fresh) { my_ctrl = in_range ? io.ctrl[(size_t)e * m.nu + my_act] : 0.f; if (in_range) s.ctrl[(size_t)my_act * N + e] = my_ctrl; }
            else my_ctrl = s.ctrl[(size_t)my_act * N + e];
        }
    }
    wave_sync();

    for (int sub = sub0; sub < sub1; sub++) {
        if (sub - sub0 >= 4 && 2 * trips_acc > 5 * (sub - sub0)) __builtin_amdgcn_s_setprio(3); else __builtin_amdgcn_s_setprio(0);
        int tid_l = tid0;
        asm volatile("" : "+v"(tid_l));
        PERSIST_LANE_VIEW(tid_l)
        const bool valid = !done;
        if (!wave_any(valid)) break;
        if (valid && c == 0) sTick[g] += 1;
        int bad = 0;
        asm volatile("" ::: "memory");
        const int nstat = m.nstatic_geom, nmov = m.ngeom - nstat;
        const GeomPlaceC gpc = geom_place_consts(m.geom_rec + 32 * (nstat + (c < nmov ? c : 0)));
        qposL[c] = qpos_c; qvelL[c] = qvel_c;
        wave_sync();
        typedef typename Kin3Of<MT>::type KD;
        constexpr bool KIN3 = KD::ok && EXACT;
        if constexpr (KIN3) {
            static_assert(KD::NL <= G, "kin3_run: one lane per link");
            static_assert(16 * KD::NL <= (16 * (MT::ngeom - MT::nstatic_geom) > 8 * G ? 16 * (MT::ngeom - MT::nstatic_geom) : 8 * G),
                          "kin3_run: the link records fit the moving-geom placement area (PersistLayout: kin_tmp)");
#ifndef HSR_K3_NORUN
            kin3_run<KD, G, NK>(c, m.gravz, qposL, qvelL, poseL, recL, kAng, qvelL + G, m.link_com, m.link_inertia, m.link_mass);
#endif
            wave_sync();
            PHASE_K(26);
        } else {
            float *dwL = qvelL + G;
            Kin2 kin;
            kin.stageA(lds + L.oKin, m.nlink, c, qposL, recL);
            wave_sync();
            PHASE_K(26);
            kin.stageB(m.maxdepth, recL, poseL);
            wave_sync();
            PHASE_K(27);
            kin.stageC(lds + L.oKin, sDofLink, nv, poseL, qvelL, kAng, kLin, kAnc, dwL);
            wave_sync();
            PHASE_K(28);
            kin.stageD((c < m.nlink && c < NLMAX) ? sMask[c] : 0, qvelL, dwL, recL);
            PHASE_K(29);
            kin.stageE(m.gravz, lk);
            wave_sync();
        }
        PHASE(24);
        PHASE(16);
        if (valid) qpos_c = qposL[c];
        if (!(fabsf(qpos_c) <= 1e10f) || !(fabsf(qvel_c) <= 1e10f)) bad = 1;
        bool reach = false;
        if (goal_body >= 0 || s.ngoal > 0) {
            reach = true;
            if (goal_body >= 0) {
                v3 bp = goal;
                if (goal_link >= 0) { m3 Rg; v3 pg; pose_load(poseL + 12 * goal_link, Rg, pg); bp = pg + mulmv(Rg, goal_off); }
                reach = norm(bp - goal) < geofence;
            }
            for (int k = 0; k < s.ngoal; k++) {
                v3 pt[2];
#pragma unroll
                for (int w = 0; w < 2; w++) {
                    const int body = w == 0 ? s.goal_a[k] : s.goal_b[k];
                    pt[w] = goal;
                    if (!m.body_mocap[body]) { m3 Rg; v3 pg; pose_load(poseL + 12 * m.body_link[body], Rg, pg); pt[w] = pg + mulmv(Rg, ld3(m.body_pos, body)); }
                }
                reach = reach && norm(pt[0] - pt[1]) < s.goal_d[k];
            }
        }
        if (valid && (sub == n_substeps - 1 || reach)) {
            for (int i = c; i < 3 * m.nlink; i += G) s.xpos[(size_t)i * N + e] = poseL[12 * (i / 3) + 9 + i % 3];
            for (int i = c; i < 9 * m.nlink; i += G) s.xmat[(size_t)i * N + e] = poseL[12 * (i / 9) + i % 9];
            for (int i = c; i < 6 * m.nlink; i += G) { const int l = (i % (3 * m.nlink)) / 3; s.lvel[(size_t)i * N + e] = recL[12 * l + (i < 3 * m.nlink ? 0 : 3) + i % 3]; }
        }
        if (io.cap && valid && (!REP || g == 0)) {
            const CaptureDesc cd = *io.cap;
            const int slot = sub % cd.every == 0 ? cd.slot[e] : -1;
            if (slot >= 0) {
                float *f = cd.cap + (size_t)(sub / cd.every) * 12 * m.nlink * cd.R + slot;
                for (int i = c; i < 3 * m.nlink; i += G) f[(size_t)i * cd.R] = poseL[12 * (i / 3) + 9 + i % 3];
                for (int i = c; i < 9 * m.nlink; i += G) f[(size_t)(3 * m.nlink + i) * cd.R] = poseL[12 * (i / 9) + i % 9];
            }
        }
        PHASE_K(31);
        {
            float *gw = qvelL + G;
            const int oGw = (int)(gw - E);
            auto gaddr = [&](int gi, const float *Ei) -> const float * { return gi < nstat ? lds + L.oGeomS + 16 * gi : Ei + oGw + 16 * (gi - nstat); };
            const float *gcc;
            if constexpr (TG) gcc = s.geom_c; else gcc = lds + L.oGeomC;
            float mymove = 0.f;
            if (valid) {
                for (int gm = c; gm < nmov; gm += G) {
                    const GeomPlaceC k2 = gm < G ? gpc : geom_place_consts(m.geom_rec + 32 * (nstat + gm));
                    m3 Rl; v3 pl;
                    pose_load(poseL + 12 * k2.link, Rl, pl);
                    const float4 lv0 = kl4(recL + 12 * k2.link);
                    const v3 lw = mk3(lv0.x, lv0.y, lv0.z), lvo = mk3(lv0.w, recL[12 * k2.link + 4], recL[12 * k2.link + 5]);
                    const v3 vg = lvo + cross(lw, mulmv(Rl, mk3(k2.q1.x, k2.q1.y, k2.q1.z)));
                    const float smove = 1.25f * m.timestep * (norm(vg) + norm(lw) * k2.q1.w) + 1e-7f;
                    geom_place3(k2, Rl, pl, gw + 16 * gm, smove);
                    mymove = fmaxf(mymove, smove);
                }
            }
            acc_move += __int_as_float(gmax<G>(__float_as_int(mymove)));
            const float skin = hook_no_item_list ? 0.f : HSR_SKIN;
            const bool rebuild = skin <= 0.f || !list_ok || wave_any(valid && 2.f * acc_move >= skin);
            for (int p0 = 0; p0 < m.npair_pad / 4; p0 += G) { const int p = p0 + c; if (p < m.npair_pad / 4) reinterpret_cast<int *>(pcnt)[p] = 0; }
            wave_sync();
            PHASE_K(30);
            const float4 *pg4 = reinterpret_cast<const float4 *>(m.pair_geo);
            const unsigned *sPair;
            if constexpr (TG) sPair = s.pair_pack; else sPair = reinterpret_cast<const unsigned *>(lds + L.oPair);
            unsigned short *sCand = reinterpret_cast<unsigned short *>(poly);
            if (rebuild) {
            int ncand = 0;
            nitems = 0;
            int nit_env[EPB];
#pragma unroll
            for (int j = 0; j < EPB; j++) nit_env[j] = 0;
            auto box_round = [&]() {
                const int take = ncand < 64 ? ncand : 64;
                bool pass = false;
                int it = 0;
                if (tid < take) {
                    it = sCand[tid];
                    const float *Ei = lds + (size_t)(it >> 14) * L.envf;
                    const unsigned pk = sPair[it & 0x3fff];
                    const int g1 = pk_g1(pk), g2 = pk_g2(pk);
                    float rb1, rb2;
                    const Geom A = geom_cached3(gaddr(g1, Ei), gcc + 8 * g1, m.mesh_vert4, rb1, ldsv), B = geom_cached3(gaddr(g2, Ei), gcc + 8 * g2, m.mesh_vert4, rb2, ldsv);
                    pass = pair_cull_box_nb(A, B, rb1, rb2, skin);
                }
                PHASE_S(2, 28);
                const unsigned long long lower = (1ull << tid) - 1ull;
                const int ig = it >> 14;
                bool accept = false;
#pragma unroll
                for (int j = 0; j < EPB; j++) {
                    const unsigned long long bj = __ballot(pass && ig == j);
                    if (pass && ig == j) accept = nit_env[j] + __popcll(bj & lower) < 64;
                    nit_env[j] += __popcll(bj);
                }
                const unsigned long long bal = __ballot(accept);
                if (accept) sItems[nitems + __popcll(bal & lower)] = (unsigned short)it;
                nitems += __popcll(bal);
                const int rest = ncand - take;
                unsigned short mv = 0;
                if (tid < rest) mv = sCand[take + tid];
                wave_sync();
                if (tid < rest) sCand[tid] = mv;
                wave_sync();
                ncand = rest;
                PHASE_S(2, 29);
            };
            {
                const int npair8 = (m.npair_pad + 7) & ~7;
                int pb = 0, u = 8, p0 = 0;
                unsigned mybits = 0;
                for (;;) {
                    if (u == 8 && pb < m.npair) {
                        p0 = pb + 8 * c;
                        uint4 k0 = make_uint4(0, 0, 0, 0), k1 = k0;
                        if (p0 < npair8) { k0 = *reinterpret_cast<const uint4 *>(sPair + p0); k1 = *reinterpret_cast<const uint4 *>(sPair + p0 + 4); }
// ... 83 lines not shown
#ifdef HSR_PAIR_HIST
                        atomicAdd(&s.phase_cyc[32 + 40 * 4096 + p1], 1ull);
#endif
                    }
                    const unsigned long long cbal = __ballot(need);
                    if (need) sMpr[__popcll(cbal & ((1ull << tid) - 1ull))] = (unsigned char)tid;
                    const int ncv = __popcll(cbal);
                    wave_sync();
                    PHASE_M(26);
                    for (int r0 = 0; r0 < ncv; r0 += 64 / MW) {
                        const int k = r0 + tid / MW;
                        const int srcl = 4 * (int)sMpr[k < ncv ? k : 0];
                        v3 d = mk3(__int_as_float(__builtin_amdgcn_ds_bpermute(srcl, __float_as_int(cdx))), __int_as_float(__builtin_amdgcn_ds_bpermute(srcl, __float_as_int(cdy))),
                                   __int_as_float(__builtin_amdgcn_ds_bpermute(srcl, __float_as_int(cdz))));
                        const float mg0 = __int_as_float(__builtin_amdgcn_ds_bpermute(srcl, __float_as_int(cmg)));
                        const bool fresh_cache = __builtin_amdgcn_ds_bpermute(srcl, cfresh) != 0;
                        if (k < ncv) {
                            const int it2 = sItems[ib + sMpr[k]];
                            Geom H1, H2; ContactOut o2; unsigned char *cntp;
                            item_geoms(it2, H1, H2, o2, cntp);
                            float *sx = s.sepax + (size_t)(4 * (it2 & 0x3fff)) * N + sEnv[it2 >> 14];
                            int *stampp = s.septick + (size_t)(it2 & 0x3fff) * N + sEnv[it2 >> 14];
                            const int tick_now = sTick[it2 >> 14];
                            float mg = 0.f;
                            int wid[3] = {0, 0, 0};
                            if (mg0 < 0.f) {
                                if (fresh_cache && mpr_warm) { wid[0] = __float_as_int(d.x); wid[1] = __float_as_int(d.y); wid[2] = __float_as_int(d.z); }
                                d = mk3(0, 0, 0);
                            }
                            const bool have = d.x != 0.f || d.y != 0.f || d.z != 0.f;
                            bool still = false;
                            PHASE_M(27);
                            if (have) {
                                const float gap = -dot(support<MW, TM1>(H1, d) - support<MW, TM2>(H2, -d), d);
                                still = gap > 1e-7f;
                                mg = still ? 0.98f * gap : 0.f;
                            }
                            PHASE_M(28);
                            if (!still) {
                                float depth; v3 dir, pos, sep;
                                int nsup = 0;
                                const bool hit = mpr_penetration<MW, TM1, TM2>(H1, H2, m.mpr_tolerance, m.mpr_iterations, depth, dir, pos, sep, nsup, wid);
#ifdef HSR_PHASE_TIMING
                                if ((tid & (MW - 1)) == 0) { atomicAdd(&sDbg[0], nsup); atomicAdd(&sDbg[1], 1); atomicMax(&sDbg[2], nsup); }
#endif
#ifdef HSR_PAIR_HIST
                                if ((tid & (MW - 1)) == 0) atomicAdd(&s.phase_cyc[32 + 40 * 4096 + 512 + (it2 & 0x3fff)], 1ull);
#endif
                                PHASE_M(29);
                                mg = 0.f;
                                if ((tid & (MW - 1)) == 0) {
                                    if (hit) { o2.add(pos, dir, -depth); sep = mk3(0, 0, 0); }
                                    if (hit && wid[0] > 0 && mpr_warm) sep = mk3(__int_as_float(wid[0]), __int_as_float(wid[1]), __int_as_float(wid[2]));
                                    sx[0] = sep.x; sx[N] = sep.y; sx[2 * (size_t)N] = sep.z;
                                }
                                if (hit && wid[0] > 0 && mpr_warm) mg = -1.f;
                            }
                            if ((tid & (MW - 1)) == 0) { sx[3 * (size_t)N] = mg; *stampp = tick_now; }
                            if ((tid & (MW - 1)) == 0) *cntp = (unsigned char)o2.cnt;
                            PHASE_M(30);
                        }
                    }
                }
                PHASE(22);
                {
                    const bool bb = fn == FN_BOX_BOX;
                    const unsigned long long bbal = __ballot(bb);
                    wave_sync();
                    if (bb) sMpr[__popcll(bbal & ((1ull << tid) - 1ull))] = (unsigned char)tid;
                    const int nbb = __popcll(bbal);
                    wave_sync();
                    PHASE_S(3, 26);
                    for (int r0 = 0; r0 < nbb; r0 += 8) {
                        const int k = r0 + tid / 8;
                        if (k < nbb) {
                            Geom G1, G2; ContactOut out; unsigned char *cntp;
                            item_geoms(sItems[ib + sMpr[k]], G1, G2, out, cntp);
                            PHASE_S(3, 27);
                            const int cnt = collide_box_box_w8(G1, G2, out.con, out.slot, out.maxcnt, poly + 24 * (tid / 8), [&](int idx) { (void)idx; if (idx == 28) { PHASE_S(3, 28); } else if (idx == 29) { PHASE_S(3, 29); } else if (idx == 30) { PHASE_S(3, 30); } else { PHASE_S(3, 31); } });
                            if ((tid & 7) == 0) *cntp = (unsigned char)cnt;
                        }
                    }
                }
                PHASE(23);
            }
        }
        __threadfence_block();
        __syncthreads();
        if constexpr (REP) {
            if (g > 0) for (int i = c; i < m.npair_pad / 4; i += G) reinterpret_cast<int *>(pcnt)[i] = reinterpret_cast<const int *>(lds + L.oCnt)[i];
            wave_sync();
        }
        if (dbg_store && valid) for (int p = c; p < m.npair; p += G) s.ncon_pair[(size_t)e * m.npair_pad + p] = pcnt[p];
        PHASE(17);
        float my_q = 0;
        q4 quat0; quat0.w = 1; quat0.x = quat0.y = quat0.z = 0;
        if (isdof) {
            my_q = qposL[my_qadr];
            if (c == my_quat_lane && my_type == DOF_FREE_ANG) { quat0.w = qposL[my_qadr]; quat0.x = qposL[my_qadr + 1]; quat0.y = qposL[my_qadr + 2]; quat0.z = qposL[my_qadr + 3]; }
        }
        wave_sync();
        const int nfb = (EXACT && G == 32) ? m.nfb : 0;
        float *fbK = poly + (size_t)g * 28 * nfb;
        float *lvbuf = rAref;
        const int lvcap = (2 * R) / 6 < 16 ? (2 * R) / 6 : 16;
        {
#define SOLVE_STORE_DIAG dbg_store
#define SOLVE_COUNT_CAPS 1
#define PAIR_CNT8(p) (*reinterpret_cast<const unsigned long long *>(pcnt + (p)))
#define SOLVE_LANE_TABLES 1
#define SOLVE_LIMITS_FROM_MODEL 1
#include "solve_body.inc"
#undef SOLVE_LANE_TABLES
#undef SOLVE_LIMITS_FROM_MODEL
#undef PAIR_CNT8
#undef SOLVE_COUNT_CAPS
#undef SOLVE_STORE_DIAG
            const float v1 = __shfl_down(vnew, 1, G), v2 = __shfl_down(vnew, 2, G);
            wave_sync();
            float *qn = rJv;
            if (valid && isdof) {
                if (my_type == DOF_SLIDE || my_type == DOF_HINGE || my_type == DOF_FREE_LIN) qn[my_qadr] = my_q + h * vnew;
                else if (c == my_quat_lane) {
                    const v3 w = mk3(vnew, v1, v2);
                    const float wn = norm(w), angle = wn * h;
                    q4 q = quat0;
                    if (angle > 0) {
                        const v3 ax = w * (1.0f / wn);
                        float sn, cs;
                        fast_sincos(0.5f * angle, &sn, &cs);
                        q4 qr;
                        qr.w = cs; qr.x = ax.x * sn; qr.y = ax.y * sn; qr.z = ax.z * sn;
                        q = qnormalized(qmul(quat0, qr));
                    }
                    qn[my_qadr] = q.w; qn[my_qadr + 1] = q.x; qn[my_qadr + 2] = q.y; qn[my_qadr + 3] = q.z;
                }
            }
            wave_sync();
            if (valid) {
                if (c < nq) qpos_c = qn[c];
                qvel_c = vnew; warm_c = qacc_c;
                time_e += h; nsteps_e += 1; nsub_run += 1;
                if (bad) bad_acc = 1;
                if (reach) done = true;
            }
            if (wave_any(valid && reach)) list_ok = false;
            trips_acc += newton_trips;
            if (valid && n_substeps - sub <= 100) own_trips += iter;
            if (valid) run_trips += iter;
            wave_sync();
            PHASE(18);
        }
    }
    {
    PERSIST_LANE_VIEW(tid0)
    const int was_done = in_range ? s.done[e] : 0;
    if (in_range && (fresh || !(was_done != 0 && nsteps_e == 0))) {
        if (c < nq) s.qpos[(size_t)c * N + e] = qpos_c;
        if (isdof) { s.qvel[(size_t)c * N + e] = qvel_c; s.warm[(size_t)c * N + e] = warm_c; }
        const float bsum = gsum<G>((float)bad_acc);
        if (c == 0 && (!REP || g == 0)) {
            if (cap_con) atomicAdd(&s.capstat[0], (unsigned long long)cap_con);
            if (cap_row) atomicAdd(&s.capstat[1], (unsigned long long)cap_row);
            if (cap_item) atomicAdd(&s.capstat[2], (unsigned long long)cap_item);
            atomicAdd(&s.capstat[3], (unsigned long long)nsub_run);
            s.trips[e] = (sub0 <= n_substeps - 100 || first_run) ? own_trips : s.trips[e] + own_trips;
            s.tick[e] = sTick[g];
            s.time[e] = time_e;
            if (bsum > 0) s.bad[e] = 1;
            s.nsteps[e] = (fresh ? 0 : s.nsteps[e]) + nsteps_e;
            if (fresh) s.done[e] = done ? 1 : 0; else if (done) s.done[e] = 1;
        }
    }
    if (in_range && io.ctrl && last_run) {
        if (io.obs) {
            float *o = io.obs + (size_t)e * (nq + nv);
            if (c < nq) o[c] = qpos_c;
            if (isdof) o[nq + c] = qvel_c;
        }
        if (c == 0) {
            if (io.reward) io.reward[e] = done ? 1.f : 0.f;
            if (io.done) io.done[e] = done ? 1 : 0;
            if (io.nsteps) io.nsteps[e] = s.nsteps[e];
            ENV_STAMP(0, e, __builtin_amdgcn_s_memrealtime());
        }
    }
    if constexpr (!SOLO && HAS_SOLO) {
        if (s.q_chunk && s.solo_servers > 0 && !last_run) {
            const bool hard = in_range && !done && n_substeps - sub1 >= s.solo_min_left && 4 * run_trips >= s.solo_trips_x4 * (sub1 - sub0);
            if (wave_any(hard)) {
                __builtin_amdgcn_fence(__ATOMIC_RELEASE, "agent");
                __builtin_amdgcn_wave_barrier();
                if (hard && c == 0) {
                    const int old = __hip_atomic_fetch_sub(&s.sq_ctl[2], 1, __ATOMIC_RELAXED, __HIP_MEMORY_SCOPE_AGENT);
                    if (old > 0) {
                        const int pos = __hip_atomic_fetch_add(&s.sq_ctl[1], 1, __ATOMIC_RELAXED, __HIP_MEMORY_SCOPE_AGENT);
                        s.slot_env[task * EPB + g] = -1;
                        ENV_STAMP(1, e, (unsigned long long)sub1 | (__builtin_amdgcn_s_memrealtime() << 16));
                        __hip_atomic_store(&s.sq_items[pos], e | (sub1 << 20), __ATOMIC_RELEASE, __HIP_MEMORY_SCOPE_AGENT);
                    } else __hip_atomic_fetch_add(&s.sq_ctl[2], 1, __ATOMIC_RELAXED, __HIP_MEMORY_SCOPE_AGENT);
                }
            }
        }
    }
    }
  };
  if (HAS_SOLO && s.q_chunk && s.solo_servers > 0 && (int)blockIdx.x < s.solo_servers) {
    if constexpr (HAS_SOLO) {
      const int T = (N + EPB - 1) / EPB;
      for (;;) {
        int item = -1;
        if (threadIdx.x == 0) {
            const int h = __hip_atomic_fetch_add(&s.sq_ctl[0], 1, __ATOMIC_RELAXED, __HIP_MEMORY_SCOPE_AGENT);
            int spins = 0;
            for (; h < s.sq_cap;) {
                item = __hip_atomic_load(&s.sq_items[h], __ATOMIC_RELAXED, __HIP_MEMORY_SCOPE_AGENT);
                if (item >= 0) break;
                if (__hip_atomic_load(&s.sq_ctl[3], __ATOMIC_ACQUIRE, __HIP_MEMORY_SCOPE_AGENT) >= T) {
                    item = __hip_atomic_load(&s.sq_items[h], __ATOMIC_RELAXED, __HIP_MEMORY_SCOPE_AGENT);
                    break;
                }
                __builtin_amdgcn_s_sleep(32);
                if (++spins > (1 << 22) || __hip_atomic_load(s.q_err, __ATOMIC_RELAXED, __HIP_MEMORY_SCOPE_AGENT) != 0) {
                    __hip_atomic_store(s.q_err, 1, __ATOMIC_RELAXED, __HIP_MEMORY_SCOPE_AGENT);
                    break;
                }
            }
        }
        item = __builtin_amdgcn_readfirstlane(item);
        if (item < 0) break;
        __builtin_amdgcn_fence(__ATOMIC_ACQUIRE, "agent");
        run_task(std::true_type{}, item >> 20, n_substeps, item & 0xfffff);
        __builtin_amdgcn_fence(__ATOMIC_RELEASE, "agent");
        __builtin_amdgcn_wave_barrier();
        if (threadIdx.x == 0) __hip_atomic_fetch_add(&s.sq_ctl[2], 1, __ATOMIC_RELAXED, __HIP_MEMORY_SCOPE_AGENT);
      }
    }
  } else
  for (;;) {
    if (s.q_chunk) {
        if (!q_claim(s, (N + EPB - 1) / EPB, (n_substeps + s.q_chunk - 1) / s.q_chunk, q_rlo, task, q_round)) break;
    }
    const int sub0 = s.q_chunk ? q_round * s.q_chunk : 0, sub1 = s.q_chunk ? min(n_substeps, sub0 + s.q_chunk) : n_substeps;
    run_task(std::false_type{}, sub0, sub1, -1);
    if (!s.q_chunk) break;
    q_push(s, (N + EPB - 1) / EPB, task, q_round, sub1 >= n_substeps);
  }
    const int tid = tid0; (void)tid;
#ifdef HSR_PHASE_TIMING
    wave_sync();
    dc_[1] = (unsigned long long)sDbg[0] | ((unsigned long long)sDbg[1] << 24) | ((unsigned long long)sDbg[2] << 48);
#endif
    PHASE_FLUSH();
#undef PERSIST_LANE_VIEW
}
```

### hsr_env_amd/csrc/solve_g.h

```cpp
#pragma once
#include "devmath.h"
#include "model.h"
#include "solve.h"
#include <type_traits>

#ifndef HSR_LAST_DEC
#define HSR_LAST_DEC 1e-6f
#endif
#ifndef HSR_LS_FAR
#define HSR_LS_FAR 1e-4f
#endif
#ifndef HSR_LS_REL_FAR
#define HSR_LS_REL_FAR 0.05f
#endif
#ifndef HSR_LS_REL
#define HSR_LS_REL 1e-2f
#endif
#ifndef HSR_SKIN
#define HSR_SKIN 0.01f
#endif
#ifdef HSR_PHASE_TIMING
__device__ __forceinline__ unsigned long long stamp_() {
    unsigned long long t;
    __builtin_amdgcn_sched_barrier(0);
    asm volatile("s_memtime %0\n\ts_waitcnt lgkmcnt(0)" : "=s"(t) :: "memory");
    __builtin_amdgcn_sched_barrier(0);
    return t;
}
#define DBGCNT(i, v) do { dc_[i] += (v); } while (0)
#define ENV_STAMP(slot, e, val) do {} while (0)
#define PHASE_T0() unsigned long long dc_[4] = {0, 0, 0, 0}; unsigned int pt_v_ = 0; const unsigned int pt_lane_ = __builtin_amdgcn_mbcnt_hi(~0u, __builtin_amdgcn_mbcnt_lo(~0u, 0u)); unsigned long long t_prev_ = stamp_(); const unsigned long long t_first_ = t_prev_, r_first_ = __builtin_amdgcn_s_memrealtime()
#define PHASE(idx) do { const unsigned long long t_now_ = stamp_(); const unsigned int acc_ = (unsigned int)__builtin_amdgcn_readfirstlane((int)((unsigned int)__builtin_amdgcn_readlane((int)pt_v_, (idx)) + (unsigned int)(t_now_ - t_prev_))); asm volatile("v_writelane_b32 %0, %1, %2" : "+v"(pt_v_) : "s"(acc_), "i"(idx)); t_prev_ = t_now_; } while (0)
#define PHASE_FLUSH() do { if (blockIdx.x < 8192 && pt_lane_ < 32) { unsigned long long *bt_ = s.phase_cyc + 32 + 40 * blockIdx.x; bt_[8 + pt_lane_] = (unsigned long long)pt_v_; if (pt_lane_ < 26) atomicAdd(&s.phase_cyc[pt_lane_], (unsigned long long)pt_v_); } if (tid == 0) { if (blockIdx.x < 8192) { unsigned long long *bt_ = s.phase_cyc + 32 + 40 * blockIdx.x; bt_[4] = dc_[0]; bt_[5] = dc_[1]; bt_[6] = dc_[2]; bt_[7] = dc_[3]; bt_[0] = r_first_; bt_[1] = __builtin_amdgcn_s_memrealtime(); bt_[2] = __builtin_amdgcn_s_getreg(63492); bt_[3] = __builtin_amdgcn_s_getreg(63508); } atomicAdd(&s.phase_cyc[26], stamp_() - t_first_); atomicAdd(&s.phase_cyc[27], __builtin_amdgcn_s_memrealtime() - r_first_); } } while (0)
#elif defined(HSR_BLOCK_LIFE)
#define PHASE_T0() unsigned long long dc_[4] = {0, 0, 0, 0}; const unsigned long long r_first_ = __builtin_amdgcn_s_memrealtime()
#define DBGCNT(i, v) do { dc_[i] += (v); } while (0)
#define PHASE(idx) do {} while (0)
#define PHASE_FLUSH() do { if (tid == 0 && blockIdx.x < 8192) { unsigned long long *bt_ = s.phase_cyc + 32 + 40 * blockIdx.x; bt_[0] = r_first_; bt_[1] = __builtin_amdgcn_s_memrealtime(); bt_[4] = dc_[0]; bt_[5] = dc_[1]; bt_[6] = dc_[2]; bt_[7] = dc_[3]; } } while (0)
#define ENV_STAMP(slot, e, val) do { if ((e) < 8192) s.phase_cyc[32 + 40 * 4096 + 8192 * (slot) + (e)] = (val); } while (0)
#else
#define PHASE_T0() do {} while (0)
#define ENV_STAMP(slot, e, val) do {} while (0)
#define DBGCNT(i, v) do {} while (0)
#define PHASE(idx) do {} while (0)
#define PHASE_FLUSH() do {} while (0)
#endif
#ifdef HSR_MPR_PROFILE
#define HSR_SUBPROF 1
#endif
#ifndef HSR_SUBPROF
#define HSR_SUBPROF 0
#endif
#define PHASE_S(n, idx) do { if constexpr (HSR_SUBPROF == (n)) { PHASE(idx); } } while (0)
#define PHASE_K(idx) PHASE_S(0, idx)
#define PHASE_M(idx) PHASE_S(1, idx)
template <int CTRL, bool ZERO_OOB> __device__ __forceinline__ float dpp_f(float v) {
    return __builtin_bit_cast(float, __builtin_amdgcn_mov_dpp(__builtin_bit_cast(int, v), CTRL, 0xf, 0xf, ZERO_OOB));
}
template <int CTRL, bool ZERO_OOB> __device__ __forceinline__ int dpp_i(int v) { return __builtin_amdgcn_update_dpp(0, v, CTRL, 0xf, 0xf, ZERO_OOB); }
__device__ __forceinline__ int rl_(int v, int lane) { return __builtin_amdgcn_readlane(v, lane); }
template <int L0, int L1> __device__ __forceinline__ int pick32_(int v) { const int a = rl_(v, L0), b = rl_(v, L1); return (threadIdx.x & 32) ? b : a; }
template <int G, int LANE> __device__ __forceinline__ float gbcast(float v) {
    if constexpr (G == 16) return dpp_f<0x150 + LANE, true>(v);
    else return __builtin_bit_cast(float, pick32_<LANE, 32 + LANE>(__builtin_bit_cast(int, v)));
}
template <int G> struct BcSrc { float lo, hi; };
template <int G> __device__ __forceinline__ BcSrc<G> bc_prepare(float v) {
    BcSrc<G> r;
    if constexpr (G == 32) {
        const unsigned u = __builtin_bit_cast(unsigned, v);
        const auto sw = __builtin_amdgcn_permlane16_swap(u, u, false, false);
        r.lo = __builtin_bit_cast(float, (unsigned)sw[0]); r.hi = __builtin_bit_cast(float, (unsigned)sw[1]);
    } else { r.lo = v; r.hi = v; }
    return r;
}
template <int G, int LANE, bool FIRST = false> __device__ __forceinline__ void fmac_bcast(float &acc, float t, const BcSrc<G> &src) {
    const float sv = (G == 32 && LANE >= 16) ? src.hi : src.lo;
    if constexpr (FIRST) asm volatile("s_nop 1\n\tv_fmac_f32_dpp %0, %1, %2 row_newbcast:%3 row_mask:0xf bank_mask:0xf" : "+v"(acc) : "v"(sv), "v"(t), "n"(LANE % 16));
    else asm volatile("v_fmac_f32_dpp %0, %1, %2 row_newbcast:%3 row_mask:0xf bank_mask:0xf" : "+v"(acc) : "v"(sv), "v"(t), "n"(LANE % 16));
}
template <int G, int LANE, int FIRST_LANE> constexpr bool bc_first() { return LANE == FIRST_LANE || (G == 32 && LANE == 16 && FIRST_LANE < 16); }
template <int G, int LANE> __device__ __forceinline__ float gbcast_after_asm(float v) {
    if constexpr (G == 16) {
        float r;
        asm volatile("s_nop 1\n\tv_mov_b32_dpp %0, %1 row_newbcast:%2 row_mask:0xf bank_mask:0xf" : "=v"(r) : "v"(v), "n"(LANE));
        return r;
    } else return gbcast<G, LANE>(v);
}
template <int G> __device__ __forceinline__ float gsum(float v) {
    asm volatile("" : "+v"(v));
    v += dpp_f<0x128, true>(v); v += dpp_f<0x124, true>(v); v += dpp_f<0x122, true>(v); v += dpp_f<0x121, true>(v);
    if constexpr (G == 16) return v;
    else {
        const unsigned u = __builtin_bit_cast(unsigned, v);
        const auto sw = __builtin_amdgcn_permlane16_swap(u, u, false, false);
        return __builtin_bit_cast(float, (unsigned)sw[0]) + __builtin_bit_cast(float, (unsigned)sw[1]);
    }
}
__device__ __forceinline__ int gsum6_index(int c) { return ((c >> 3) & 1) + 2 * ((c >> 2) & 1) + 4 * ((c >> 1) & 1); }
template <int G> __device__ __forceinline__ float gsum6_packed(const float (&p)[6], int c) {
    float x[6];
#pragma unroll
    for (int q = 0; q < 6; q++) x[q] = p[q] + dpp_f<0x128, true>(p[q]);
    const bool h8 = c & 8, h4 = c & 4, h2 = c & 2;
    float r0 = h8 ? x[1] : x[0], r1 = h8 ? x[3] : x[2], r2 = h8 ? x[5] : x[4];
    r0 += dpp_f<0x141, true>(r0); r1 += dpp_f<0x141, true>(r1); r2 += dpp_f<0x141, true>(r2);
    float z0 = h4 ? r1 : r0, z1 = r2;
    z0 += dpp_f<0x1B, true>(z0); z1 += dpp_f<0x1B, true>(z1);
    float w = h2 ? z1 : z0;
    w += dpp_f<0xB1, true>(w);
    if constexpr (G == 32) {
        const unsigned u = __builtin_bit_cast(unsigned, w);
        const auto sw = __builtin_amdgcn_permlane16_swap(u, u, false, false);
        w = __builtin_bit_cast(float, (unsigned)sw[0]) + __builtin_bit_cast(float, (unsigned)sw[1]);
    }
    return w;
}
template <int G> __device__ __forceinline__ int gscan_incl(int v, int c) {
    v += dpp_i<0x111, true>(v); v += dpp_i<0x112, true>(v); v += dpp_i<0x114, true>(v); v += dpp_i<0x118, true>(v);
    if constexpr (G == 16) return v;
    else { const int first = pick32_<15, 47>(v); return (threadIdx.x & 16) ? v + first : v; }
}
template <int G> __device__ __forceinline__ int gor(int v) {
    v |= dpp_i<0x128, true>(v); v |= dpp_i<0x124, true>(v); v |= dpp_i<0x122, true>(v); v |= dpp_i<0x121, true>(v);
    if constexpr (G == 16) return v;
    else { const auto sw = __builtin_amdgcn_permlane16_swap((unsigned)v, (unsigned)v, false, false); return (int)(sw[0] | sw[1]); }
}
template <int G> __device__ __forceinline__ int gmax(int v) {
    { const int t = dpp_i<0x128, true>(v); v = t > v ? t : v; } { const int t = dpp_i<0x124, true>(v); v = t > v ? t : v; }
    { const int t = dpp_i<0x122, true>(v); v = t > v ? t : v; } { const int t = dpp_i<0x121, true>(v); v = t > v ? t : v; }
    if constexpr (G == 16) return v;
    else { const auto sw = __builtin_amdgcn_permlane16_swap((unsigned)v, (unsigned)v, false, false); const int a = (int)sw[0], b = (int)sw[1]; return a > b ? a : b; }
}
template <int G> __device__ __forceinline__ int wave_or_groups(int v) {
    if constexpr (G == 16) return rl_(v, 0) | rl_(v, 16) | rl_(v, 32) | rl_(v, 48); else return rl_(v, 0) | rl_(v, 32);
}
template <int G> __device__ __forceinline__ int wave_max_groups(int v) {
    if constexpr (G == 16) { const int a = rl_(v, 0), b = rl_(v, 16), c = rl_(v, 32), d = rl_(v, 48); const int x = a > b ? a : b, y = c > d ? c : d; return x > y ? x : y; }
    else { const int a = rl_(v, 0), b = rl_(v, 32); return a > b ? a : b; }
}
template <int G> __device__ __forceinline__ int glast(int v) {
    if constexpr (G == 16) return dpp_i<0x15F, false>(v); else return pick32_<31, 63>(v);
}

#define HSR_GSUM_STAGE_(CTRL) do { const float ta_ = dpp_f<CTRL, true>(a), tb_ = dpp_f<CTRL, true>(b); a += ta_; b += tb_; } while (0)
template <int G> __device__ __forceinline__ void gsum2(float a, float b, float &sa, float &sb) {
    asm volatile("" : "+v"(a)); asm volatile("" : "+v"(b));
    HSR_GSUM_STAGE_(0x128); HSR_GSUM_STAGE_(0x124); HSR_GSUM_STAGE_(0x122); HSR_GSUM_STAGE_(0x121);
    if constexpr (G == 16) { sa = a; sb = b; }
    else {
        const unsigned ua = __builtin_bit_cast(unsigned, a), ub = __builtin_bit_cast(unsigned, b);
        const auto wa = __builtin_amdgcn_permlane16_swap(ua, ua, false, false), wb = __builtin_amdgcn_permlane16_swap(ub, ub, false, false);
        sa = __builtin_bit_cast(float, (unsigned)wa[0]) + __builtin_bit_cast(float, (unsigned)wa[1]);
        sb = __builtin_bit_cast(float, (unsigned)wb[0]) + __builtin_bit_cast(float, (unsigned)wb[1]);
    }
}
#undef HSR_GSUM_STAGE_
#define HSR_GSUM_STAGE_(CTRL) do { const float ta_ = dpp_f<CTRL, true>(a), tb_ = dpp_f<CTRL, true>(b), tc_ = dpp_f<CTRL, true>(c); a += ta_; b += tb_; c += tc_; } while (0)
template <int G> __device__ __forceinline__ void gsum3(float a, float b, float c, float &sa, float &sb, float &sc) {
    asm volatile("" : "+v"(a)); asm volatile("" : "+v"(b)); asm volatile("" : "+v"(c));
    HSR_GSUM_STAGE_(0x128); HSR_GSUM_STAGE_(0x124); HSR_GSUM_STAGE_(0x122); HSR_GSUM_STAGE_(0x121);
    if constexpr (G == 16) { sa = a; sb = b; sc = c; }
    else {
        const unsigned ua = __builtin_bit_cast(unsigned, a), ub = __builtin_bit_cast(unsigned, b), uc = __builtin_bit_cast(unsigned, c);
        const auto wa = __builtin_amdgcn_permlane16_swap(ua, ua, false, false), wb = __builtin_amdgcn_permlane16_swap(ub, ub, false, false);
        const auto wc = __builtin_amdgcn_permlane16_swap(uc, uc, false, false);
        sa = __builtin_bit_cast(float, (unsigned)wa[0]) + __builtin_bit_cast(float, (unsigned)wa[1]);
        sb = __builtin_bit_cast(float, (unsigned)wb[0]) + __builtin_bit_cast(float, (unsigned)wb[1]);
        sc = __builtin_bit_cast(float, (unsigned)wc[0]) + __builtin_bit_cast(float, (unsigned)wc[1]);
    }
}
#undef HSR_GSUM_STAGE_

#define HSR_DPPB_(n) " row_newbcast:%[" #n "] row_mask:0xf bank_mask:0xf\n\t"
template <int J, bool LAST> __device__ __forceinline__ void chol_step16_fwd(float &p, float &rowj, float &rown, float &sacc, float &t, float &nl, float &invd, float &y, int c) {
#define HSR_STEP_HEAD_ "v_mul_f32 %[l], %[l], %[p]\n\tv_mul_f32 %[t], %[sacc], %[p]\n\tv_xor_b32 %[nl], 0x80000000, %[l]\n\tv_cmp_eq_u32 vcc, %[j], %[c]\n\t"
#define HSR_STEP_SEL_ "v_cndmask_b32 %[invd], %[invd], %[p], vcc\n\tv_cndmask_b32 %[y], %[y], %[t], vcc\n\t"
    if constexpr (J == 0) {
        static_assert(!LAST, "a one-column matrix needs no step");
        asm volatile("v_rsq_f32 %[p], %[p]\n\ts_nop 0\n\t" HSR_STEP_HEAD_ "v_fmac_f32_dpp %[n], %[l], %[nl]" HSR_DPPB_(jn) HSR_STEP_SEL_ "v_mov_b32_dpp %[p], %[n]" HSR_DPPB_(jn)
                     : [p] "+v"(p), [l] "+v"(rowj), [n] "+v"(rown), [t] "=&v"(t), [nl] "=&v"(nl), [invd] "+v"(invd), [y] "+v"(y)
                     : [sacc] "v"(sacc), [c] "v"(c), [j] "n"(J), [jn] "n"(J + 1) : "vcc");
    } else if constexpr (!LAST) {
        asm volatile("v_rsq_f32 %[p], %[p]\n\tv_fmac_f32_dpp %[sacc], %[t], %[nl]" HSR_DPPB_(jp) HSR_STEP_HEAD_ "v_fmac_f32_dpp %[n], %[l], %[nl]" HSR_DPPB_(jn) HSR_STEP_SEL_ "v_mov_b32_dpp %[p], %[n]" HSR_DPPB_(jn)
                     : [p] "+v"(p), [l] "+v"(rowj), [n] "+v"(rown), [sacc] "+v"(sacc), [t] "+v"(t), [nl] "+v"(nl), [invd] "+v"(invd), [y] "+v"(y)
                     : [c] "v"(c), [j] "n"(J), [jn] "n"(J + 1), [jp] "n"(J - 1) : "vcc");
    } else {
        asm volatile("v_rsq_f32 %[p], %[p]\n\tv_fmac_f32_dpp %[sacc], %[t], %[nl]" HSR_DPPB_(jp) HSR_STEP_HEAD_ HSR_STEP_SEL_
                     : [p] "+v"(p), [l] "+v"(rowj), [sacc] "+v"(sacc), [t] "+v"(t), [nl] "+v"(nl), [invd] "+v"(invd), [y] "+v"(y)
                     : [c] "v"(c), [j] "n"(J), [jp] "n"(J - 1) : "vcc");
    }
#undef HSR_STEP_HEAD_
#undef HSR_STEP_SEL_
}
template <int J, int T> __device__ __forceinline__ void chol_step16(float &p, float &rowj, float &r1, float &r2, float &r3, float &nl, float &invd, int c) {
#define HSR_STEP_HEAD_ "v_rsq_f32 %[p], %[p]\n\tv_cmp_eq_u32 vcc, %[j], %[c]\n\tv_mul_f32 %[l], %[l], %[p]\n\tv_xor_b32 %[nl], 0x80000000, %[l]\n\tv_cndmask_b32 %[invd], %[invd], %[p], vcc\n\t"
    if constexpr (T >= 3) {
        asm volatile(HSR_STEP_HEAD_ "v_fmac_f32_dpp %[n1], %[l], %[nl]" HSR_DPPB_(j1) "v_fmac_f32_dpp %[n2], %[l], %[nl]" HSR_DPPB_(j2) "v_fmac_f32_dpp %[n3], %[l], %[nl]" HSR_DPPB_(j3) "v_mov_b32_dpp %[p], %[n1]" HSR_DPPB_(j1)
// ... 344 lines not shown
```

### hsr_env_amd/csrc/util_kernels.h

```cpp
__global__ void k_build_tables(DevModel m, DevState s) {
    const int i = blockIdx.x * blockDim.x + threadIdx.x;
    if (i < m.ngeom) { geom_consts_store(m.geom_rec + 32 * i, s.geom_c + 8 * i); if (m.nldsv > 0 && m.geom_ldsv[i] >= 0) hull_lds_patch(s.geom_c + 8 * i, m.geom_ldsv[i]); }
    if (i < ((m.npair_pad + 7) & ~7)) {
        unsigned pk = 0;
        if (i < m.npair) {
            const float4 a = reinterpret_cast<const float4 *>(m.pair_geo)[2 * i], b = reinterpret_cast<const float4 *>(m.pair_geo)[2 * i + 1];
            const int code = (int)a.x;
            pk = pair_pack(code & 255, (int)a.y, (int)b.x, (code >> 8) ? a.w : a.z + a.w);
        }
        s.pair_pack[i] = pk;
    }
}
__global__ void k_aos_to_soa(float *dst, const float *src, int rows, int N) {
    size_t i = (size_t)blockIdx.x * blockDim.x + threadIdx.x;
    if (i >= (size_t)rows * N) return;
    int r = (int)(i / N), e = (int)(i % N);
    dst[i] = src[(size_t)e * rows + r];
}
__global__ void k_soa_to_aos(float *dst, const float *src, int rows, int N, int dst_stride, int dst_off) {
    size_t i = (size_t)blockIdx.x * blockDim.x + threadIdx.x;
    if (i >= (size_t)rows * N) return;
    int r = (int)(i / N), e = (int)(i % N);
    dst[(size_t)e * dst_stride + dst_off + r] = src[i];
}
__global__ void k_begin_step(DevState s, const float *ctrl_in, int nu) {
    int e = blockIdx.x * blockDim.x + threadIdx.x;
    if (e >= s.N) return;
    for (int a = 0; a < nu; a++) s.ctrl[(size_t)a * s.N + e] = ctrl_in[(size_t)e * nu + a];
    s.done[e] = 0;
    s.nsteps[e] = 0;
}
__global__ void k_end_step(DevState s, float *reward, uint8_t *done, int32_t *nsteps) {
    int e = blockIdx.x * blockDim.x + threadIdx.x;
    if (e >= s.N) return;
    if (reward) reward[e] = s.done[e] ? 1.f : 0.f;
    if (done) done[e] = (uint8_t)(s.done[e] != 0);
    if (nsteps) nsteps[e] = s.nsteps[e];
}
__global__ void k_clear_done(DevState s) {
    int e = blockIdx.x * blockDim.x + threadIdx.x;
    if (e < s.N) s.done[e] = 0;
}
__global__ void k_reset(DevModel m, DevState s, const uint8_t *mask, const float *qpos0_env, const float *qpos0_model, const float *mocap, int park) {
    int e = blockIdx.x * blockDim.x + threadIdx.x;
    if (e >= s.N) return;
    const bool sel = mask ? mask[e] != 0 : (park ? s.done[e] != 0 : true);
    s.done[e] = (park && !sel) ? 1 : 0;
    if (!sel) return;
    const int N = s.N;
    for (int i = 0; i < m.nq; i++) s.qpos[(size_t)i * N + e] = qpos0_env ? qpos0_env[(size_t)e * m.nq + i] : qpos0_model[i];
    for (int i = 0; i < m.nv; i++) { s.qvel[(size_t)i * N + e] = 0; s.warm[(size_t)i * N + e] = 0; s.qacc[(size_t)i * N + e] = 0; }
    for (int i = 0; i < m.nu; i++) s.ctrl[(size_t)i * N + e] = 0;
    for (int k = 0; k < 3; k++) s.mocap[(size_t)k * N + e] = mocap ? mocap[(size_t)e * 3 + k] : 0.f;
    s.time[e] = 0; s.bad[e] = 0; s.nsteps[e] = 0;
    for (int p = 0; p < m.npair; p++) {
        float *mg = s.sepax + (size_t)(4 * p + 3) * N + e;
        if (*mg < 0.f) { mg[-(ptrdiff_t)N] = 0.f; mg[-2 * (ptrdiff_t)N] = 0.f; mg[-3 * (ptrdiff_t)N] = 0.f; }
        *mg = 0.f;
    }
}
__global__ void k_body_xpos(DevModel m, DevState s, int body, float *out) {
    int e = blockIdx.x * blockDim.x + threadIdx.x;
    if (e >= s.N) return;
    const int N = s.N;
    v3 p;
    if (m.body_mocap[body]) p = mk3(s.mocap[e], s.mocap[N + e], s.mocap[2 * N + e]);
    else {
        const int l = m.body_link[body];
        View xpos{s.xpos + e, N}, xmat{s.xmat + e, N};
        p = xpos.get3(l) + mulmv(xmat.getm(l), ld3(m.body_pos, body));
    }
    out[3 * e] = p.x; out[3 * e + 1] = p.y; out[3 * e + 2] = p.z;
}
__device__ __forceinline__ void body_pose_vel(const DevModel &m, const DevState &s, int body, int e, v3 &p, v3 &v, v3 &w, m3 &R) {
    const int N = s.N, l = m.body_link[body], nl = m.nlink;
    const View xpos{s.xpos + e, N}, xmat{s.xmat + e, N};
    const m3 Rl = xmat.getm(l);
    const v3 off = mulmv(Rl, ld3(m.body_pos, body));
    p = xpos.get3(l) + off;
    R = mulmm(Rl, ldm(m.body_mat, body));
    w = mk3(s.lvel[(size_t)(3 * l) * N + e], s.lvel[(size_t)(3 * l + 1) * N + e], s.lvel[(size_t)(3 * l + 2) * N + e]);
    const v3 vo = mk3(s.lvel[(size_t)(3 * nl + 3 * l) * N + e], s.lvel[(size_t)(3 * nl + 3 * l + 1) * N + e], s.lvel[(size_t)(3 * nl + 3 * l + 2) * N + e]);
    v = vo + cross(w, off);
}
__global__ void k_obs_openai(DevModel m, DevState s, int body_l, int body_r, int body_obj, int qadr_l, int qadr_r, int dadr_l, int dadr_r,
                             float dt, float *out) {
    const int e = blockIdx.x * blockDim.x + threadIdx.x;
    if (e >= s.N) return;
    const int N = s.N;
    v3 pl, vl, wl, pr, vr, wr, po, vo, wo;
    m3 Rl, Rr, Ro;
    body_pose_vel(m, s, body_l, e, pl, vl, wl, Rl);
    body_pose_vel(m, s, body_r, e, pr, vr, wr, Rr);
    body_pose_vel(m, s, body_obj, e, po, vo, wo, Ro);
    const v3 grip = (pl + pr) * 0.5f, gvel = (vl + vr) * (0.5f * dt);
    const v3 rel = po - grip, ovel = vo * dt - gvel, orot = wo * dt;
    const float cy = sqrtf(Ro.a[8] * Ro.a[8] + Ro.a[5] * Ro.a[5]);
    const bool cond = cy > 4.f * 2.220446049250313e-16f;
    const float ez = cond ? -atan2f(Ro.a[1], Ro.a[0]) : -atan2f(-Ro.a[3], Ro.a[4]);
    const float ey = -atan2f(-Ro.a[2], cy);
    const float ex = cond ? -atan2f(Ro.a[5], Ro.a[8]) : 0.f;
    float *o = out + (size_t)25 * e;
    o[0] = grip.x; o[1] = grip.y; o[2] = grip.z; o[3] = po.x; o[4] = po.y; o[5] = po.z; o[6] = rel.x; o[7] = rel.y; o[8] = rel.z;
    o[9] = s.qpos[(size_t)qadr_l * N + e]; o[10] = s.qpos[(size_t)qadr_r * N + e];
    o[11] = ex; o[12] = ey; o[13] = ez;
    o[14] = ovel.x; o[15] = ovel.y; o[16] = ovel.z; o[17] = orot.x; o[18] = orot.y; o[19] = orot.z;
    o[20] = gvel.x; o[21] = gvel.y; o[22] = gvel.z;
    o[23] = 0.5f * dt * s.qvel[(size_t)dadr_l * N + e]; o[24] = 0.5f * dt * s.qvel[(size_t)dadr_r * N + e];
}
__global__ void k_i32_to_f32(float *dst, const int *src, size_t n) {
    size_t i = (size_t)blockIdx.x * blockDim.x + threadIdx.x;
    if (i < n) dst[i] = (float)src[i];
}
__global__ void k_contacts_out(DevModel m, DevState s, float *out) {
    int e = blockIdx.x * blockDim.x + threadIdx.x;
    if (e >= s.N) return;
    const int N = s.N;
    for (int p = 0; p < m.npair; p++) {
        const int cnt = s.ncon_pair[(size_t)e * m.npair_pad + p];
        for (int slot = m.pair_slot[p]; slot < m.pair_slot[p + 1]; slot++) {
            float *o = out + ((size_t)e * m.nslot + slot) * 7;
            const bool used = slot - m.pair_slot[p] < cnt;
            for (int k = 0; k < 7; k++) o[k] = used ? s.con[((size_t)e * m.nslot + slot) * 8 + k] : (k == 6 ? 1.f : 0.f);
        }
    }
}
__global__ void k_expand_M(DevState s, float *out, int nv) {
    int e = blockIdx.x * blockDim.x + threadIdx.x;
    if (e >= s.N) return;
    for (int i = 0; i < nv; i++) for (int j = 0; j <= i; j++) {
        const float v = s.M[(size_t)(i * (i + 1) / 2 + j) * s.N + e];
        out[((size_t)e * nv + i) * nv + j] = v; out[((size_t)e * nv + j) * nv + i] = v;
    }
}
__global__ void k_clear_margins(DevState s) {
    const size_t i = (size_t)blockIdx.x * blockDim.x + threadIdx.x;
    if (i < (size_t)s.npair_sep * s.N) {
        float *mg = s.sepax + (4 * (i / s.N) + 3) * s.N + i % s.N;
        if (*mg < 0.f) { mg[-(ptrdiff_t)s.N] = 0.f; mg[-2 * (ptrdiff_t)s.N] = 0.f; mg[-3 * (ptrdiff_t)s.N] = 0.f; }
        *mg = 0.f;
    }
}
__global__ void k_capture(DevState s, int nlink, const int *cap_env, int R, float *cap, int frame, int live_only, int every, int *cnt) {
    const int i = blockIdx.x * blockDim.x + threadIdx.x;
    if (i >= 12 * nlink * R) return;
    const int row = i / R, r = i % R, e = cap_env[r];
    if (live_only && s.done[e]) return;
    cap[(size_t)frame * 12 * nlink * R + i] = row < 3 * nlink ? s.xpos[(size_t)row * s.N + e] : s.xmat[(size_t)(row - 3 * nlink) * s.N + e];
    if (cnt && row == 0) { const int n = s.nsteps[e]; cnt[r] = n == 0 ? 0 : (n - 1) / every + 1; }
}
enum { SCHED_CHUNK = 8192 };
__global__ void k_queue_init(DevState s, int T, int R) {
    const int i = blockIdx.x * blockDim.x + threadIdx.x;
    if (i < R) { s.q_head[i] = 0; s.q_wpos[i] = i == 0 ? T : 0; }
    if (i < 4) s.sq_ctl[i] = i == 2 ? s.solo_servers : 0;
    if (s.solo_servers > 0) for (int k = i; k < s.sq_cap; k += gridDim.x * blockDim.x) s.sq_items[k] = -1;
    if (i < R * T) s.q_items[i] = i < T ? i : -1;
}
template <int J> __device__ __forceinline__ void sched_local_stage(unsigned (&v)[8], int tid, int k) {
    unsigned w[8];
#pragma unroll
    for (int r = 0; r < 8; r++) {
        const int i = 8 * tid + r;
        const unsigned a = v[r], c = v[r ^ J];
        w[r] = (((i & J) == 0) == ((i & k) == 0)) ? (a > c ? a : c) : (a < c ? a : c);
    }
#pragma unroll
    for (int r = 0; r < 8; r++) v[r] = w[r];
}
__global__ void __launch_bounds__(1024) k_schedule(DevState s, int epb, int *slot_env) {
    __shared__ unsigned key[SCHED_CHUNK];
    const int tid = threadIdx.x;
    const int e0 = blockIdx.x * SCHED_CHUNK, n = min(SCHED_CHUNK, s.N - e0);
    unsigned v[8];
#pragma unroll
    for (int r = 0; r < 8; r++) {
        const int i = 8 * tid + r;
        const int t = i < n ? min(s.trips[e0 + i], 0x1fffe) : 0;
        v[r] = i < n ? ((unsigned)(t + 1) << 13) | (unsigned)(SCHED_CHUNK - 1 - i) : 0u;
    }
    for (int k = 2; k <= SCHED_CHUNK; k <<= 1) {
        for (int j = k >> 1; j >= 512; j >>= 1) {
#pragma unroll
            for (int r = 0; r < 8; r++) key[1024 * r + tid] = v[r];
            __syncthreads();
#pragma unroll
            for (int r = 0; r < 8; r++) {
                const int i = 8 * tid + r;
                const unsigned a = v[r], c = key[1024 * r + (tid ^ (j >> 3))];
                v[r] = (((i & j) == 0) == ((i & k) == 0)) ? (a > c ? a : c) : (a < c ? a : c);
            }
            __syncthreads();
        }
        for (int j = (k >> 1) < 256 ? (k >> 1) : 256; j >= 8; j >>= 1) {
#pragma unroll
            for (int r = 0; r < 8; r++) {
                const int i = 8 * tid + r;
                const unsigned a = v[r], c = (unsigned)__shfl_xor((int)v[r], j >> 3, 64);
                v[r] = (((i & j) == 0) == ((i & k) == 0)) ? (a > c ? a : c) : (a < c ? a : c);
            }
        }
        if (k >= 8) sched_local_stage<4>(v, tid, k);
        if (k >= 4) sched_local_stage<2>(v, tid, k);
        sched_local_stage<1>(v, tid, k);
    }
#pragma unroll
    for (int r = 0; r < 8; r++) key[8 * tid + r] = v[r];
    __syncthreads();
    const int nw = (n + epb - 1) / epb;
    for (int sl = threadIdx.x; sl < nw * epb; sl += blockDim.x) {
        const int w = sl / epb, j = sl % epb;
        int idx;
        if (j == 0) idx = w;
        else { const int r = (j - 1) * nw + w; idx = r < n - nw ? n - 1 - r : -1; }
        slot_env[(size_t)e0 / epb * epb + sl] = (idx >= 0 && idx < n) ? e0 + (SCHED_CHUNK - 1 - (int)(key[idx] & (SCHED_CHUNK - 1))) : -1;
    }
}
```

### hsr_env_amd/sim.py

```python
from __future__ import annotations

import ctypes as C
from pathlib import Path

import numpy as np

from .model import Model

_HERE = Path(__file__).parent
import os
LIB_PATH = Path(os.environ.get("HSR_LIB", _HERE / "libhsrsim.so"))


class DependencyNotInstalled(ImportError):
    """Raised when libhsrsim.so (or a GPU) is unavailable - reference: gym.error.DependencyNotInstalled
    raised by hsr/mujoco_env.py:12-15 when mujoco_py is missing."""


class MujocoException(RuntimeError):
    """Some env reached a non-finite state (reference: mujoco_py.MujocoException on MuJoCo warnings)."""


def raise_if_diverged(sim):
    bad_state = getattr(sim, "bad_state", None)
    if bad_state is not None:
        bad, any_bad = bad_state()
        if any_bad:
            raise MujocoException(f"simulation diverged in env(s) {np.flatnonzero(bad)[:8].tolist()} (non-finite or |q| > 1e10)")


_vp, _fp_t, _u8p, _i32p = C.c_void_p, C.POINTER(C.c_float), C.POINTER(C.c_uint8), C.POINTER(C.c_int32)
_ip, _ullp = C.POINTER(C.c_int), C.POINTER(C.c_ulonglong)
_int, _float = C.c_int, C.c_float
_RENDER = [_vp, _fp_t, _int, _int, _int, _fp_t]
PROTOTYPES = {
    "hsr_last_error": (C.c_char_p, []),
    "hsr_model_load": (_int, [C.c_char_p, C.c_size_t, C.POINTER(_vp)]),
    "hsr_model_destroy": (None, [_vp]),
    "hsr_model_size": (_int, [_vp, _int]),
    "hsr_model_timestep": (C.c_double, [_vp]),
    "hsr_model_ctrlrange": (_int, [_vp, _fp_t]),
    "hsr_model_qpos0": (_int, [_vp, _fp_t]),
    "hsr_model_body_id": (_int, [_vp, C.c_char_p]),
    "hsr_model_joint_qpos_addr": (_int, [_vp, C.c_char_p, _ip, _ip]),
    "hsr_model_hull_planes": (_int, [_vp, _int, _fp_t, _int]),
    "hsr_batch_create": (_int, [_vp, _int, _int, C.POINTER(_vp)]),
    "hsr_batch_destroy": (None, [_vp]),
    "hsr_batch_size": (_int, [_vp]),
    "hsr_batch_stream": (_vp, [_vp]),
    "hsr_batch_sync": (_int, [_vp]),
    "hsr_batch_reset": (_int, [_vp, _u8p, _fp_t, _fp_t]),
    "hsr_batch_reset_dev": (_int, [_vp, _vp, _vp, _vp]),
    "hsr_batch_get_state": (_int, [_vp, _fp_t, _fp_t, _fp_t]),
    "hsr_batch_set_state": (_int, [_vp, _fp_t, _fp_t, _fp_t]),
    "hsr_batch_set_mocap": (_int, [_vp, _fp_t]),
    "hsr_batch_set_warmstart": (_int, [_vp, _fp_t]),
    "hsr_batch_get_warmstart": (_int, [_vp, _fp_t]),
    "hsr_batch_forward": (_int, [_vp]),
    "hsr_batch_step": (_int, [_vp, _fp_t, _int, _int, _float, _fp_t, _fp_t, _u8p, _i32p]),
    "hsr_batch_step_dev": (_int, [_vp, _vp, _int, _int, _float, _vp, _vp, _vp, _vp]),
    "hsr_batch_set_goals": (_int, [_vp, _int, _ip, _ip, _fp_t]),
    "hsr_batch_body_xpos": (_int, [_vp, _int, _fp_t]),
    "hsr_batch_obs_openai": (_int, [_vp, _ip, _fp_t]),
    "hsr_batch_obs_openai_dev": (_int, [_vp, _ip, _vp]),
    "hsr_batch_render": (_int, _RENDER + [_u8p, _fp_t, _i32p]),
    "hsr_batch_render_dev": (_int, _RENDER + [_vp, _vp, _vp]),
    "hsr_batch_set_capture": (_int, [_vp, _int, _int, _i32p]),
    "hsr_batch_capture_counts": (_int, [_vp, _i32p]),
    "hsr_batch_capture_poses": (_int, [_vp, _fp_t, _fp_t]),
    "hsr_batch_render_frames": (_int, _RENDER + [_u8p, _fp_t, _i32p]),
    "hsr_batch_render_frames_dev": (_int, _RENDER + [_vp, _vp, _vp]),
    "hsr_batch_bad_state": (_int, [_vp, _u8p]),
    "hsr_batch_get_field": (_int, [_vp, _int, _fp_t]),
    "hsr_batch_set_profiling": (_int, [_vp, _int]),
    "hsr_batch_last_timing": (_int, [_vp, _fp_t, _fp_t, _ip]),
    "hsr_batch_kernel_times": (_int, [_vp, _fp_t, _int]),
    "hsr_batch_set_graph": (_int, [_vp, _int]),
    "hsr_batch_set_persistent": (_int, [_vp, _int]),
    "hsr_batch_is_persistent": (_int, [_vp]),
    "hsr_batch_set_debug": (_int, [_vp, _int]),
    "hsr_batch_set_solo": (_int, [_vp, _int, _float]),
    "hsr_batch_solo_handovers": (_int, [_vp, _ip]),
    "hsr_batch_set_schedule": (_int, [_vp, _int]),
    "hsr_batch_set_mpr_warm": (_int, [_vp, _int]),
    "hsr_batch_set_queue": (_int, [_vp, _int, _int]),
    "hsr_batch_cap_counts": (_int, [_vp, _ullp]),
    "hsr_batch_cap_histogram": (_int, [_vp, _ullp]),
    "hsr_batch_newton_trips": (_int, [_vp, _i32p]),
    "hsr_batch_packing": (_int, [_vp, _i32p]),
    "hsr_batch_set_episodes": (_int, [_vp, _vp]),
    "hsr_batch_reset_sampled_dev": (_int, [_vp, _vp]),
    "hsr_batch_reset_sampled": (_int, [_vp, _u8p]),
    "hsr_batch_episode_end_dev": (_int, [_vp, _vp, _vp, _vp, _vp, _vp, _vp, _vp]),
    "hsr_batch_sample_ctrl_dev": (_int, [_vp, C.c_uint32, _vp]),
    "hsr_batch_episode_state": (_int, [_vp, C.POINTER(C.c_uint32), _i32p, _fp_t]),
    "hsr_batch_phase_cycles": (_int, [_vp, _ullp]),
    "hsr_batch_block_times": (_int, [_vp, _ullp, _int]),
    "hsr_batch_snapshot_create": (_int, [_vp, _int, C.POINTER(_vp)]),
    "hsr_snapshot_destroy": (None, [_vp]),
    "hsr_snapshot_capacity": (_int, [_vp]),
    "hsr_batch_snapshot_save": (_int, [_vp, _vp, _i32p, _i32p, _int]),
    "hsr_batch_snapshot_save_dev": (_int, [_vp, _vp, _vp, _vp, _int]),
    "hsr_batch_snapshot_load": (_int, [_vp, _vp, _i32p, _i32p, _int]),
    "hsr_batch_snapshot_load_dev": (_int, [_vp, _vp, _vp, _vp, _int]),
    "hsr_batch_copy_envs": (_int, [_vp, _i32p, _i32p, _int]),
    "hsr_batch_copy_envs_dev": (_int, [_vp, _vp, _vp, _int]),
    "hsr_snapshot_image_bytes": (_int, [_vp, C.POINTER(C.c_longlong)]),
    "hsr_snapshot_export": (_int, [_vp, _vp, C.c_longlong]),
    "hsr_snapshot_import": (_int, [_vp, C.c_char_p, C.c_longlong]),
    "hsr_model_snapshot_record_words": (_int, [_vp]),
    "hsr_model_snapshot_image_check": (_int, [_vp, C.c_char_p, C.c_longlong, _ip]),
    "hsr_batch_replay_create": (_int, [_vp, _vp, C.POINTER(_vp)]),
    "hsr_replay_destroy": (None, [_vp]),
    "hsr_replay_clear": (_int, [_vp]),
    "hsr_replay_commit_dev": (_int, [_vp, _vp, _vp]),
    "hsr_replay_record_dev": (_int, [_vp, _vp, _vp, _vp, _vp]),
    "hsr_replay_state": (_int, [_vp, _i32p, _i32p, C.POINTER(C.c_uint32)]),
    "hsr_replay_sample_dev": (_int, [_vp, C.c_uint32, _int, _float, _vp, _vp, _vp, _vp, _vp, _vp, _vp, _vp]),
    "hsr_replay_sample_seq_dev": (_int, [_vp, C.c_uint32, _int, _int, _float, _float, _vp]),
    "hsr_replay_priority_enable": (_int, [_vp, _vp]),
    "hsr_replay_priority_state": (_int, [_vp, C.POINTER(C.c_uint64), C.POINTER(C.c_double), C.POINTER(C.c_float)]),
    "hsr_replay_priority_sample_dev": (_int, [_vp, C.c_uint32, _int, _float, _vp, _vp, _vp, _vp, _vp, _vp, _vp, _vp, _vp]),
    "hsr_replay_priority_sample_seq_dev": (_int, [_vp, C.c_uint32, _int, _int, _float, _float, _vp, _vp]),
    "hsr_replay_priority_update_dev": (_int, [_vp, C.c_uint64, _int, _vp, _vp]),
    "hsr_replay_priority_read_dev": (_int, [_vp, _vp]),
    "hsr_batch_rollout_create": (_int, [_vp, _vp, C.POINTER(_vp)]),
    "hsr_rollout_destroy": (None, [_vp]),
    "hsr_rollout_begin_dev": (_int, [_vp, _vp]),
    "hsr_rollout_stage_dev": (_int, [_vp, _vp, _vp, _vp]),
    "hsr_rollout_close_dev": (_int, [_vp, _vp, _vp, _vp]),
    "hsr_rollout_bootstrap_dev": (_int, [_vp, _vp]),
    "hsr_rollout_finish_dev": (_int, [_vp, _vp]),
    "hsr_rollout_next": (_int, [_vp]),
    "hsr_rollout_state": (_int, [_vp, _i32p, _i32p]),
    "hsr_rollout_stats": (_int, [_vp, _fp_t, _fp_t, _fp_t]),
    "hsr_rollout_minibatch_dev": (_int, [_vp, C.c_uint32, _int, _int, _int, _vp, _vp, _vp, _vp, _vp, _vp, _vp]),
    "hsr_rollout_planes_dev": (_int, [_vp, _vp, _vp]),
}
EXPORTS = list(PROTOTYPES)

CAPTURE_MAX = 1024

F_XPOS, F_XMAT, F_M, F_QACC, F_QACC_SMOOTH, F_QFRC_SMOOTH, F_QFRC_CONSTRAINT, F_NCON, F_NEFC, F_CONTACT, F_NITER = range(11)

_lib = None


def load_library():
    global _lib
    if _lib is not None:
        return _lib
    if not LIB_PATH.exists():
        raise DependencyNotInstalled(
            f"{LIB_PATH} not built. Run `python -c 'import __graft_entry__ as g; g.build()'` "
            "(hipcc --offload-arch=gfx950); there is no CPU fallback for the product path.")
    L = C.CDLL(str(LIB_PATH))
    for name, (restype, argtypes) in PROTOTYPES.items():
        f = getattr(L, name)
        f.restype, f.argtypes = restype, argtypes
    _lib = L
    return L


def _fp(a):
    return None if a is None else a.ctypes.data_as(C.POINTER(C.c_float))


def _f32(a, shape=None):
    if a is None:
        return None
    a = np.ascontiguousarray(a, dtype=np.float32)
    if shape is not None:
        assert a.shape == tuple(shape), f"expected shape {tuple(shape)}, got {a.shape}"
    return a


def _check(L, rc):
    if rc == 0:
        return
    msg = L.hsr_last_error().decode()
    if rc == -3:
        raise DependencyNotInstalled(f"libhsrsim: {msg}")
    if rc == -2:
        raise IOError(f"libhsrsim: {msg}")
    if rc == -5:
        raise MujocoException(f"libhsrsim: {msg}")
    if rc == -4:
        raise KeyError(msg)
    raise AssertionError(f"libhsrsim: {msg}")


class BatchSim:

    def __init__(self, model: Model, n_envs: int, device: int = 0):
        self.model = model
        self.n = int(n_envs)
        self._L = L = load_library()
        raw = model.to_bytes()
        self._m = C.c_void_p()
        _check(L, L.hsr_model_load(raw, len(raw), C.byref(self._m)))
        self._b = C.c_void_p()
        _check(L, L.hsr_batch_create(self._m, self.n, int(device), C.byref(self._b)))
        self.nq, self.nv, self.nu = model.nq, model.nv, model.nu
        self.device = device

    def close(self):
        if getattr(self, "_b", None):
            self._L.hsr_batch_destroy(self._b); self._b = None
        if getattr(self, "_m", None):
            self._L.hsr_model_destroy(self._m); self._m = None

    __del__ = close

    def reset(self, mask=None, qpos0=None, mocap=None):
        m = None if mask is None else np.ascontiguousarray(mask, dtype=np.uint8)
        q = _f32(qpos0, (self.n, self.nq)); mc = _f32(mocap, (self.n, 3))
        _check(self._L, self._L.hsr_batch_reset(self._b, None if m is None else m.ctypes.data_as(C.POINTER(C.c_uint8)), _fp(q), _fp(mc)))

    def reset_dev(self, d_mask, d_qpos0, d_mocap):
        _check(self._L, self._L.hsr_batch_reset_dev(self._b, d_mask, d_qpos0, d_mocap))

    def forward(self):
        _check(self._L, self._L.hsr_batch_forward(self._b))

    def set_episodes(self, spec):
        c, keep = spec.to_c()
        _check(self._L, self._L.hsr_batch_set_episodes(self._b, C.byref(c)))
        del keep

    def reset_sampled(self, mask=None):
        m = None if mask is None else np.ascontiguousarray(np.asarray(mask).reshape(self.n) != 0, dtype=np.uint8)
        _check(self._L, self._L.hsr_batch_reset_sampled(self._b, None if m is None else m.ctypes.data_as(_u8p)))

    def reset_sampled_dev(self, d_mask=None):
        _check(self._L, self._L.hsr_batch_reset_sampled_dev(self._b, d_mask))
# ... 71 lines not shown
                   finger_joints=("hand_l_proximal_joint", "hand_r_proximal_joint")):
        m = self.model
        jn, qa, da = m.names["joint"], m.meta["joint_qposadr"], m.meta["joint_dofadr"]
        ids = [m.body_id(finger_bodies[0]), m.body_id(finger_bodies[1]), m.body_id(object_body or m.block_body())]
        ids += [qa[jn.index(j)][0] for j in finger_joints] + [da[jn.index(j)] for j in finger_joints]
        return (C.c_int * 7)(*ids)

    def obs_openai(self, ids=None):
        out = np.empty((self.n, 25), np.float32)
        _check(self._L, self._L.hsr_batch_obs_openai(self._b, ids or self.openai_ids(), _fp(out)))
        return out

    def obs_openai_dev(self, d_out, ids=None):
        _check(self._L, self._L.hsr_batch_obs_openai_dev(self._b, ids or self.openai_ids(), C.c_void_p(int(d_out))))

    def _render_args(self, camera, geom_rgba):
        from .render import default_camera
        cam = camera if camera is not None else default_camera(self.model)
        pal = None if geom_rgba is None else _f32(geom_rgba, (self.model.ngeom, 4))
        return cam.as_array(), int(cam.track_body), pal

    def _render_host(self, fn, lead, fill, width, height, camera, rgb, depth, segmentation, geom_rgba):
        cam, track, pal = self._render_args(camera, geom_rgba)
        w, h = int(width), int(height)
        ok = 1 <= w <= 4096 and 1 <= h <= 4096
        new = lambda shape, dt, v: np.empty(shape, dt) if v is None else np.full(shape, v, dt)
        o_rgb = new(lead + (h, w, 3), np.uint8, fill[0]) if rgb and ok else None
        o_dep = new(lead + (h, w), np.float32, fill[1]) if depth and ok else None
        o_seg = new(lead + (h, w), np.int32, fill[2]) if segmentation and ok else None
        _check(self._L, fn(self._b, _fp(cam), track, w, h, _fp(pal), None if o_rgb is None else o_rgb.ctypes.data_as(C.POINTER(C.c_uint8)),
                           _fp(o_dep), None if o_seg is None else o_seg.ctypes.data_as(C.POINTER(C.c_int32))))
        outs = [o for o, want in ((o_rgb, rgb), (o_dep, depth), (o_seg, segmentation)) if want]
        return outs[0] if len(outs) == 1 else tuple(outs)

    def _render_dev(self, who, fn, lead, width, height, camera, rgb, depth, segmentation, geom_rgba):
        cam, track, pal = self._render_args(camera, geom_rgba)
        w, h = int(width), int(height)
        for t, shape, dt in ((rgb, lead + (h, w, 3), "torch.uint8"), (depth, lead + (h, w), "torch.float32"),
                             (segmentation, lead + (h, w), "torch.int32")):
            if t is not None:
                if tuple(t.shape) != shape or str(t.dtype) != dt or not t.is_contiguous() or t.device.type != "cuda":
                    raise AssertionError(f"{who}: expected a contiguous {dt} tensor of shape {shape} on the GPU")
                if t.device.index != self.device:
                    raise AssertionError(f"{who}: tensor on cuda:{t.device.index}, the batch is on cuda:{self.device}")
        ptr = lambda t: None if t is None else C.c_void_p(t.data_ptr())
        _check(self._L, fn(self._b, _fp(cam), track, w, h, _fp(pal), ptr(rgb), ptr(depth), ptr(segmentation)))

    def render(self, width, height, camera=None, rgb=True, depth=False, segmentation=False, geom_rgba=None):
        fn = self._L.hsr_batch_render
        return self._render_host(fn, (self.n,), (None, None, None), width, height, camera, rgb, depth, segmentation, geom_rgba)

    def render_dev(self, width, height, camera=None, rgb=None, depth=None, segmentation=None, geom_rgba=None):
        self._render_dev("render_dev", self._L.hsr_batch_render_dev, (self.n,), width, height, camera, rgb, depth, segmentation, geom_rgba)

    def set_capture(self, env_ids, every):
        ids = np.ascontiguousarray(np.atleast_1d(np.asarray(env_ids if every else [], dtype=np.int32)))
        self._cap_n = len(ids) if every else 0
        _check(self._L, self._L.hsr_batch_set_capture(self._b, int(every), len(ids), ids.ctypes.data_as(C.POINTER(C.c_int32)) if len(ids) else None))

    def capture_counts(self):
        out = np.empty(max(getattr(self, "_cap_n", 0), 1), np.int32)
        rc = self._L.hsr_batch_capture_counts(self._b, out.ctypes.data_as(C.POINTER(C.c_int32)))
        if rc < 0:
            _check(self._L, rc)
        return out[:self._cap_n]

    def capture_rows(self):
        rc = self._L.hsr_batch_capture_counts(self._b, None)
        if rc < 0:
            _check(self._L, rc)
        return rc

    def capture_poses(self):
        rows, nl = self.capture_rows(), self.model.nlink
        xpos = np.empty((self._cap_n, rows, nl, 3), np.float32); xmat = np.empty((self._cap_n, rows, nl, 3, 3), np.float32)
        _check(self._L, self._L.hsr_batch_capture_poses(self._b, _fp(xpos), _fp(xmat)))
        return xpos, xmat

    def render_frames(self, width, height, camera=None, rgb=True, depth=False, segmentation=False, geom_rgba=None):
        fn, lead = self._L.hsr_batch_render_frames, (self._cap_n, self.capture_rows())
        return self._render_host(fn, lead, (0, np.nan, -2), width, height, camera, rgb, depth, segmentation, geom_rgba)

    def render_frames_dev(self, width, height, camera=None, rgb=None, depth=None, segmentation=None, geom_rgba=None):
        fn, lead = self._L.hsr_batch_render_frames_dev, (self._cap_n, self.capture_rows())
        self._render_dev("render_frames_dev", fn, lead, width, height, camera, rgb, depth, segmentation, geom_rgba)

    def bad_state(self):
        out = np.empty(self.n, np.uint8)
        rc = self._L.hsr_batch_bad_state(self._b, out.ctypes.data_as(C.POINTER(C.c_uint8)))
        if rc not in (0, -5):
            _check(self._L, rc)
        return out.astype(bool), rc == -5

    def get_field(self, field: int):
        m = self.model
        shapes = {F_XPOS: (self.n, m.nlink, 3), F_XMAT: (self.n, m.nlink, 3, 3), F_M: (self.n, m.nv, m.nv),
                  F_QACC: (self.n, m.nv), F_QACC_SMOOTH: (self.n, m.nv), F_QFRC_SMOOTH: (self.n, m.nv),
                  F_QFRC_CONSTRAINT: (self.n, m.nv), F_NCON: (self.n,), F_NEFC: (self.n,), F_NITER: (self.n,),
                  F_CONTACT: (self.n, m.nslot, 7)}
        out = np.empty(shapes[field], np.float32)
        _check(self._L, self._L.hsr_batch_get_field(self._b, field, _fp(out)))
        return out

    def set_profiling(self, on):
        _check(self._L, self._L.hsr_batch_set_profiling(self._b, int(on)))

    def set_mpr_warm(self, on: bool):
        _check(self._L, self._L.hsr_batch_set_mpr_warm(self._b, int(on)))

    def set_queue(self, mode: int, chunk: int = 0):
        _check(self._L, self._L.hsr_batch_set_queue(self._b, int(mode), int(chunk)))

    def kernel_times(self, cap: int = 4096):
        buf = (C.c_float * cap)()
        n = self._L.hsr_batch_kernel_times(self._b, buf, cap)
        if n < 0:
            _check(self._L, n)
        if n > cap:
            raise ValueError(f"{n} launches were logged, the buffer holds {cap}: pass cap >= the number of launches since the last call")
        return np.array(buf[:n], dtype=np.float64)

    def set_graph(self, on: bool):
        _check(self._L, self._L.hsr_batch_set_graph(self._b, int(on)))

    def set_persistent(self, on: bool) -> bool:
        return bool(self._L.hsr_batch_set_persistent(self._b, int(on)))

    def is_persistent(self) -> bool:
        return bool(self._L.hsr_batch_is_persistent(self._b))

    def kernel_flags(self) -> int:
        return int(self._L.hsr_batch_is_persistent(self._b))

    def set_debug(self, on):
        _check(self._L, self._L.hsr_batch_set_debug(self._b, int(on)))

    def set_goals(self, terms):
        n = len(terms)
        a = (C.c_int * max(n, 1))(*[int(t[0]) for t in terms]); b = (C.c_int * max(n, 1))(*[int(t[1]) for t in terms])
        d = (C.c_float * max(n, 1))(*[float(t[2]) for t in terms])
        _check(self._L, self._L.hsr_batch_set_goals(self._b, n, a, b, d))

    def set_solo(self, servers: int, trips: float = 0.0) -> bool:
        rc = self._L.hsr_batch_set_solo(self._b, int(servers), float(trips))
        if rc < 0:
            _check(self._L, rc)
        return rc == 0

    def solo_handovers(self) -> int:
        out = C.c_int(0)
        _check(self._L, self._L.hsr_batch_solo_handovers(self._b, C.byref(out)))
        return int(out.value)

    def set_schedule(self, on: bool):
        _check(self._L, self._L.hsr_batch_set_schedule(self._b, int(on)))

    def cap_counts(self):
        out = (C.c_ulonglong * 4)()
        _check(self._L, self._L.hsr_batch_cap_counts(self._b, out))
        return tuple(int(x) for x in out)

    def cap_histogram(self):
        out = (C.c_ulonglong * 8)()
        _check(self._L, self._L.hsr_batch_cap_histogram(self._b, out))
        return [int(x) for x in out]

    def newton_trips(self):
        out = np.empty(self.n, np.int32)
        _check(self._L, self._L.hsr_batch_newton_trips(self._b, out.ctypes.data_as(C.POINTER(C.c_int32))))
        return out

    def packing(self, envs_per_wave: int):
        if envs_per_wave not in (2, 4):
            raise ValueError("envs_per_wave is 4 (16 lanes per env) or 2 (32 lanes per env)")
        out = np.full(self.n + 64, -1, np.int32)
        _check(self._L, self._L.hsr_batch_packing(self._b, out.ctypes.data_as(C.POINTER(C.c_int32))))
        slots = (self.n + envs_per_wave - 1) // envs_per_wave * envs_per_wave
        return out[:slots].reshape(-1, envs_per_wave)

    def last_timing(self):
        tot = C.c_float(0); k = (C.c_float * 3)(); n = (C.c_int * 3)()
        _check(self._L, self._L.hsr_batch_last_timing(self._b, C.byref(tot), k, n))
        return float(tot.value), [float(x) for x in k], [int(x) for x in n]


def _id_pair(sim, a, b):
    dev = [x is not None and hasattr(x, "data_ptr") for x in (a, b)]
    if any(dev):
        for x in (a, b):
            if x is None:
                continue
            if not hasattr(x, "data_ptr"):
                raise AssertionError("ids: device tensors and host arrays cannot be mixed in one call")
            if str(x.dtype) != "torch.int32" or x.dim() != 1 or not x.is_contiguous() or x.device.type != "cuda" or x.device.index != sim.device:
                raise AssertionError(f"ids: expected a contiguous 1-d torch.int32 tensor on cuda:{sim.device}")
        ptr = lambda x: None if x is None else C.c_void_p(x.data_ptr())
        keep = (a, b)
    else:
        a, b = [None if x is None else np.ascontiguousarray(np.atleast_1d(x), dtype=np.int32) for x in (a, b)]
        for x in (a, b):
            if x is not None and x.ndim != 1:
                raise AssertionError("ids: expected 1-d arrays")
        ptr = lambda x: None if x is None else x.ctypes.data_as(_i32p)
        keep = (a, b)
    lens = {int(x.shape[0]) for x in keep if x is not None}
    if len(lens) > 1:
        raise AssertionError("ids: the two arrays differ in length")
    return any(dev), ptr(keep[0]), ptr(keep[1]), (lens.pop() if lens else sim.n), keep


class Snapshot:

    def __init__(self, sim: BatchSim, capacity: int):
        self.sim = sim
        self._s = C.c_void_p()
        _check(sim._L, sim._L.hsr_batch_snapshot_create(sim._b, int(capacity), C.byref(self._s)))
        self.capacity = int(capacity)

    def close(self):
        if getattr(self, "_s", None):
            self.sim._L.hsr_snapshot_destroy(self._s); self._s = None

    __del__ = close

    def save(self, envs=None, slots=None):
        dev, e, s, n, keep = _id_pair(self.sim, envs, slots)
        L = self.sim._L
        _check(L, (L.hsr_batch_snapshot_save_dev if dev else L.hsr_batch_snapshot_save)(self.sim._b, self._s, e, s, n))
        del keep

    def load(self, slots=None, envs=None, into: BatchSim = None):
        sim = into if into is not None else self.sim
        dev, s, e, n, keep = _id_pair(sim, slots, envs)
        L = sim._L
        _check(L, (L.hsr_batch_snapshot_load_dev if dev else L.hsr_batch_snapshot_load)(sim._b, self._s, s, e, n))
        del keep

    def to_bytes(self) -> bytes:
        L = self.sim._L
        size = C.c_longlong(0)
        _check(L, L.hsr_snapshot_image_bytes(self._s, C.byref(size)))
        buf = C.create_string_buffer(size.value)
        _check(L, L.hsr_snapshot_export(self._s, buf, size.value))
        return buf.raw

    def _from_image(self, data: bytes):
        L = self.sim._L
        _check(L, L.hsr_snapshot_import(self._s, bytes(data), len(data)))
        return self

    @classmethod
    def from_bytes(cls, sim: BatchSim, data: bytes) -> "Snapshot":
        L = sim._L
        cap = C.c_int(0)
        _check(L, L.hsr_model_snapshot_image_check(sim._m, bytes(data), len(data), C.byref(cap)))
        return cls(sim, cap.value)._from_image(data)


class ReplaySpec(C.Structure):
    _fields_ = [("seed", C.c_uint64), ("env_offset", C.c_uint32), ("capacity_steps", C.c_int32), ("obs_dim", C.c_int32),
                ("goal_body", C.c_int32), ("geofence", C.c_float)]


class PrioritySpec(C.Structure):
    _fields_ = [("p_init", C.c_float), ("p_min", C.c_float), ("p_max", C.c_float), ("max_batch", C.c_int32)]


class ReplaySeqOut(C.Structure):
    _fields_ = [(name, C.c_void_p) for name in ("obs", "act", "next_obs", "achieved_next", "goal", "reward", "done", "length", "nstep", "nstep_return",
                                                "nstep_discount", "nstep_obs", "nstep_done", "index")]


class Replay:

    def __init__(self, sim: BatchSim, spec: ReplaySpec):
        self.sim, self.spec = sim, spec
        self._r = C.c_void_p()
        _check(sim._L, sim._L.hsr_batch_replay_create(sim._b, C.byref(spec), C.byref(self._r)))

    def close(self):
        if getattr(self, "_r", None):
            self.sim._L.hsr_replay_destroy(self._r); self._r = None

    __del__ = close

    def clear(self):
        _check(self.sim._L, self.sim._L.hsr_replay_clear(self._r))

    def commit_dev(self, d_obs, d_reset=None):
        _check(self.sim._L, self.sim._L.hsr_replay_commit_dev(self._r, d_obs, d_reset))

    def record_dev(self, d_ctrl, d_next_obs, d_reward=None, d_done=None):
        _check(self.sim._L, self.sim._L.hsr_replay_record_dev(self._r, d_ctrl, d_next_obs, d_reward, d_done))

    def state(self):
        c, h, p = C.c_int32(0), C.c_int32(0), C.c_uint32(0)
        _check(self.sim._L, self.sim._L.hsr_replay_state(self._r, C.byref(c), C.byref(h), C.byref(p)))
        return int(c.value), int(h.value), int(p.value)

    def sample_dev(self, draw, batch, her_ratio, d_obs=None, d_act=None, d_next_obs=None, d_goal=None, d_achieved_next=None, d_reward=None,
                   d_done=None, d_index=None):
        _check(self.sim._L, self.sim._L.hsr_replay_sample_dev(self._r, int(draw) & 0xffffffff, int(batch), float(her_ratio), d_obs, d_act, d_next_obs,
                                                              d_goal, d_achieved_next, d_reward, d_done, d_index))

    def sample_seq_dev(self, draw, batch, seq_len, her_ratio, gamma, out: "ReplaySeqOut"):
        _check(self.sim._L, self.sim._L.hsr_replay_sample_seq_dev(self._r, int(draw) & 0xffffffff, int(batch), int(seq_len), float(her_ratio), float(gamma),
# ... 82 lines not shown
```

### include/hsrsim.h

```cpp
#ifndef HSRSIM_H
#define HSRSIM_H

#include <stddef.h>
#include <stdint.h>

#ifdef __cplusplus
extern "C" {
#endif

#define HSR_OK 0
#define HSR_EINVAL (-1)
#define HSR_EBLOB (-2)
#define HSR_EDEVICE (-3)
#define HSR_ENAME (-4)
#define HSR_EBADSTATE (-5)

typedef struct hsr_model hsr_model;
typedef struct hsr_batch hsr_batch;
typedef struct hsr_snapshot hsr_snapshot;
typedef struct hsr_replay hsr_replay;

enum hsr_size { HSR_NQ = 0, HSR_NV, HSR_NU, HSR_NLINK, HSR_NBODY, HSR_NGEOM, HSR_NPAIR, HSR_NMESHVERT,
                HSR_NSLOT, HSR_NLIMIT, HSR_NCONMAX, HSR_NJMAX, HSR_NMOCAP };

const char *hsr_last_error(void);

int hsr_model_load(const void *blob, size_t len, hsr_model **out);
void hsr_model_destroy(hsr_model *m);
int hsr_model_size(const hsr_model *m, int which);
double hsr_model_timestep(const hsr_model *m);
int hsr_model_ctrlrange(const hsr_model *m, float *out );
int hsr_model_qpos0(const hsr_model *m, float *out );
int hsr_model_body_id(const hsr_model *m, const char *name);
int hsr_model_joint_qpos_addr(const hsr_model *m, const char *name, int *start, int *end);
int hsr_model_hull_planes(const hsr_model *m, int geom, float *out , int cap);

int hsr_batch_create(const hsr_model *m, int n_envs, int device_id, hsr_batch **out);
void hsr_batch_destroy(hsr_batch *b);
int hsr_batch_size(const hsr_batch *b);
void *hsr_batch_stream(const hsr_batch *b);
int hsr_batch_sync(hsr_batch *b);

int hsr_batch_reset(hsr_batch *b, const uint8_t *mask, const float *qpos0 , const float *mocap );

int hsr_batch_reset_dev(hsr_batch *b, const uint8_t *d_mask, const float *d_qpos0, const float *d_mocap);

int hsr_batch_get_state(hsr_batch *b, float *time , float *qpos , float *qvel );
int hsr_batch_set_state(hsr_batch *b, const float *time, const float *qpos, const float *qvel);
int hsr_batch_set_mocap(hsr_batch *b, const float *mocap );
int hsr_batch_set_warmstart(hsr_batch *b, const float *qacc_warmstart );
int hsr_batch_get_warmstart(hsr_batch *b, float *qacc_warmstart );
int hsr_batch_forward(hsr_batch *b);

int hsr_batch_step(hsr_batch *b, const float *ctrl , int n_substeps, int goal_body, float geofence,
                   float *obs , float *reward , uint8_t *done , int32_t *nsteps );
int hsr_batch_step_dev(hsr_batch *b, const float *d_ctrl, int n_substeps, int goal_body, float geofence,
                       float *d_obs, float *d_reward, uint8_t *d_done, int32_t *d_nsteps);

int hsr_batch_set_goals(hsr_batch *b, int n, const int *body_a, const int *body_b, const float *dist);

int hsr_batch_body_xpos(hsr_batch *b, int body_id, float *out );


int hsr_batch_obs_openai(hsr_batch *b, const int *ids, float *out );
int hsr_batch_obs_openai_dev(hsr_batch *b, const int *ids, float *d_out);
int hsr_batch_render(hsr_batch *b, const float *cam, int track_body, int width, int height, const float *geom_rgba,
                     uint8_t *rgb , float *depth , int32_t *segid );
int hsr_batch_render_dev(hsr_batch *b, const float *cam, int track_body, int width, int height, const float *geom_rgba,
                         uint8_t *d_rgb, float *d_depth, int32_t *d_segid);
#define HSR_CAPTURE_MAX 1024
int hsr_batch_set_capture(hsr_batch *b, int every, int n, const int *env_ids);
int hsr_batch_capture_counts(hsr_batch *b, int32_t *counts);
int hsr_batch_capture_poses(hsr_batch *b, float *xpos, float *xmat);
int hsr_batch_render_frames(hsr_batch *b, const float *cam, int track_body, int width, int height, const float *geom_rgba,
                            uint8_t *rgb, float *depth, int32_t *segid);
int hsr_batch_render_frames_dev(hsr_batch *b, const float *cam, int track_body, int width, int height, const float *geom_rgba,
                                uint8_t *d_rgb, float *d_depth, int32_t *d_segid);
int hsr_batch_bad_state(hsr_batch *b, uint8_t *out );

enum hsr_field { HSR_F_XPOS = 0 , HSR_F_XMAT , HSR_F_M ,
                 HSR_F_QACC , HSR_F_QACC_SMOOTH , HSR_F_QFRC_SMOOTH ,
                 HSR_F_QFRC_CONSTRAINT , HSR_F_NCON , HSR_F_NEFC ,
                 HSR_F_CONTACT ,
                 HSR_F_NITER  };
int hsr_batch_get_field(hsr_batch *b, int field, float *out);
int hsr_batch_set_profiling(hsr_batch *b, int on);
int hsr_batch_last_timing(hsr_batch *b, float *total_ms, float *kernel_ms , int *launches );
int hsr_batch_kernel_times(hsr_batch *b, float *out_ms, int cap);
int hsr_batch_set_graph(hsr_batch *b, int on);
int hsr_batch_set_persistent(hsr_batch *b, int on);
int hsr_batch_is_persistent(const hsr_batch *b);
int hsr_batch_set_debug(hsr_batch *b, int on);
int hsr_batch_set_solo(hsr_batch *b, int servers, float trips);
int hsr_batch_solo_handovers(hsr_batch *b, int *out);
int hsr_batch_set_schedule(hsr_batch *b, int on);
int hsr_batch_set_mpr_warm(hsr_batch *b, int on);
int hsr_batch_set_queue(hsr_batch *b, int mode, int chunk);
int hsr_batch_cap_counts(hsr_batch *b, unsigned long long *out );
int hsr_batch_cap_histogram(hsr_batch *b, unsigned long long *out );
int hsr_batch_newton_trips(hsr_batch *b, int32_t *out );
int hsr_batch_packing(hsr_batch *b, int32_t *out );

typedef struct hsr_episode_spec {
    uint64_t seed;
    uint32_t env_offset;
    int32_t max_episode_steps;
    const float *qpos_lo, *qpos_hi;
    int32_t has_goal;
    float goal_lo[3], goal_hi[3];
    int32_t nblock;
    const int32_t *block_qadr;
    float block_lo[4], block_hi[4];
} hsr_episode_spec;
int hsr_batch_set_episodes(hsr_batch *b, const hsr_episode_spec *spec);
int hsr_batch_reset_sampled_dev(hsr_batch *b, const uint8_t *d_mask);
int hsr_batch_reset_sampled(hsr_batch *b, const uint8_t *mask);
int hsr_batch_episode_end_dev(hsr_batch *b, float *d_obs, const float *d_reward, const uint8_t *d_done, float *d_final_obs,
                              uint8_t *d_reset_kind, float *d_fin_return, int32_t *d_fin_length);
int hsr_batch_sample_ctrl_dev(hsr_batch *b, uint32_t step, float *d_ctrl);
int hsr_batch_episode_state(hsr_batch *b, uint32_t *ep_index, int32_t *ep_length, float *ep_return);

int hsr_batch_snapshot_create(hsr_batch *b, int capacity, hsr_snapshot **out);
void hsr_snapshot_destroy(hsr_snapshot *s);
int hsr_snapshot_capacity(const hsr_snapshot *s);
int hsr_batch_snapshot_save(hsr_batch *b, hsr_snapshot *s, const int32_t *env, const int32_t *slot, int n);
int hsr_batch_snapshot_save_dev(hsr_batch *b, hsr_snapshot *s, const int32_t *d_env, const int32_t *d_slot, int n);
int hsr_batch_snapshot_load(hsr_batch *b, const hsr_snapshot *s, const int32_t *slot, const int32_t *env, int n);
int hsr_batch_snapshot_load_dev(hsr_batch *b, const hsr_snapshot *s, const int32_t *d_slot, const int32_t *d_env, int n);
int hsr_batch_copy_envs(hsr_batch *b, const int32_t *src, const int32_t *dst, int n);
int hsr_batch_copy_envs_dev(hsr_batch *b, const int32_t *d_src, const int32_t *d_dst, int n);
int hsr_snapshot_image_bytes(const hsr_snapshot *s, long long *out);
int hsr_snapshot_export(const hsr_snapshot *s, void *out, long long len);
int hsr_snapshot_import(hsr_snapshot *s, const void *image, long long len);
int hsr_model_snapshot_record_words(const hsr_model *m);
int hsr_model_snapshot_image_check(const hsr_model *m, const void *image, long long len, int *capacity);

typedef struct hsr_replay_spec {
    uint64_t seed;
    uint32_t env_offset;
    int32_t  capacity_steps;
    int32_t  obs_dim;
    int32_t  goal_body;
    float    geofence;
} hsr_replay_spec;
int  hsr_batch_replay_create(hsr_batch *b, const hsr_replay_spec *spec, hsr_replay **out);
void hsr_replay_destroy(hsr_replay *r);
int  hsr_replay_clear(hsr_replay *r);
int  hsr_replay_commit_dev(hsr_replay *r, const float *d_obs, const uint8_t *d_reset);
int  hsr_replay_record_dev(hsr_replay *r, const float *d_ctrl, const float *d_next_obs, const float *d_reward, const uint8_t *d_done);
int  hsr_replay_state(hsr_replay *r, int32_t *count, int32_t *head_slot, uint32_t *pushed_lo);
int  hsr_replay_sample_dev(hsr_replay *r, uint32_t draw, int batch, float her_ratio,
                           float *d_obs, float *d_act, float *d_next_obs, float *d_goal, float *d_achieved_next,
                           float *d_reward, uint8_t *d_done, int32_t *d_index );
typedef struct hsr_replay_seq_out {
    float *obs;
    float *act;
    float *next_obs;
    float *achieved_next;
    float *goal;
    float *reward;
    uint8_t *done;
    int32_t *length;
    int32_t *nstep;
    float *nstep_return;
    float *nstep_discount;
    float *nstep_obs;
    uint8_t *nstep_done;
    int32_t *index;
} hsr_replay_seq_out;
int  hsr_replay_sample_seq_dev(hsr_replay *r, uint32_t draw, int batch, int seq_len, float her_ratio, float gamma,
                               const hsr_replay_seq_out *out);
typedef struct hsr_priority_spec {
    float   p_init;
    float   p_min, p_max;
    int32_t max_batch;
} hsr_priority_spec;
int  hsr_replay_priority_enable(hsr_replay *r, const hsr_priority_spec *spec);
int  hsr_replay_priority_state(hsr_replay *r, uint64_t *pushed, double *total, float *p_new);
int  hsr_replay_priority_sample_dev(hsr_replay *r, uint32_t draw, int batch, float her_ratio,
                                    float *d_obs, float *d_act, float *d_next_obs, float *d_goal, float *d_achieved_next,
                                    float *d_reward, uint8_t *d_done, int32_t *d_index , float *d_prob );
int  hsr_replay_priority_sample_seq_dev(hsr_replay *r, uint32_t draw, int batch, int seq_len, float her_ratio, float gamma,
                                        const hsr_replay_seq_out *out, float *d_prob );
int  hsr_replay_priority_update_dev(hsr_replay *r, uint64_t sampled_at, int batch, const int32_t *d_index , const float *d_priority );
int  hsr_replay_priority_read_dev(hsr_replay *r, float *d_leaves );

typedef struct hsr_rollout hsr_rollout;
typedef struct hsr_rollout_spec {
    uint64_t seed;
    uint32_t env_offset;
    int32_t  horizon;
    int32_t  obs_dim;
    float    gamma;
    float    lam;
} hsr_rollout_spec;
int  hsr_batch_rollout_create(hsr_batch *b, const hsr_rollout_spec *spec, hsr_rollout **out);
void hsr_rollout_destroy(hsr_rollout *r);
int  hsr_rollout_begin_dev(hsr_rollout *r, const float *d_obs);
int  hsr_rollout_stage_dev(hsr_rollout *r, const float *d_act, const float *d_logp, const float *d_value);
int  hsr_rollout_close_dev(hsr_rollout *r, const float *d_reward, const uint8_t *d_kind, const float *d_next_obs);
int  hsr_rollout_bootstrap_dev(hsr_rollout *r, const float *d_value_terminal);
int  hsr_rollout_finish_dev(hsr_rollout *r, const float *d_last_value);
int  hsr_rollout_next(hsr_rollout *r);
int  hsr_rollout_state(hsr_rollout *r, int32_t *state, int32_t *t);
int  hsr_rollout_stats(hsr_rollout *r, float *mean, float *std, float *rstd);
int  hsr_rollout_minibatch_dev(hsr_rollout *r, uint32_t epoch, int first, int count, int normalize,
                               float *d_obs, float *d_act, float *d_logp, float *d_value, float *d_adv, float *d_ret, int32_t *d_index );
int  hsr_rollout_planes_dev(hsr_rollout *r, float *d_adv, float *d_ret);

int hsr_batch_phase_cycles(hsr_batch *b, unsigned long long *out );
int hsr_batch_block_times(hsr_batch *b, unsigned long long *out , int nblocks);

#ifdef __cplusplus
}
#endif
#endif
```

Measured before the change: 512,100 env-steps/s.

## Split slow env groups off persistent blocks to idle helper blocks

Adds a work-splitting mode to the persistent env-step kernel. Every few substeps a block checks per-group solver trip counts, and when two or more of its env groups are expensive it hands all but the most expensive off, through a device queue, to blocks that have already finished their own tasks. Finished blocks become helpers that spin on credits and claim these items, so the tail is shortened when env costs are imbalanced. The mode is on by default for cfg3 and cupboard. In exchange it adds periodic decision overhead, atomics and spin-waiting, and more code and register pressure in the hot kernel.

```diff
diff --git a/hsr_env_amd/csrc/host_access.h b/hsr_env_amd/csrc/host_access.h
--- a/hsr_env_amd/csrc/host_access.h
+++ b/hsr_env_amd/csrc/host_access.h
@@ -60,10 +60,22 @@
     if (trips > 0.f) b->solo_trips = trips;
     return b->kernel_sv ? HSR_OK : 1;
 }
+extern "C" int hsr_batch_set_split(hsr_batch *b, int on, int period, float trips, int min_left, int extra_helpers) {
+    ENTER(b);
+    if (period < 0 || period >= SPLIT_MAX_SUBSTEPS || trips > 1000.f || min_left < 0 || extra_helpers < 0 || extra_helpers > SPLIT_MAX_EXTRA)
+        return fail(HSR_EINVAL, "hsr_batch_set_split: period 0..2047, trips <= 1000, min_left >= 0, extra_helpers 0..4096");
+    b->split = on != 0;
+    if (period > 0) b->split_period = period;
+    if (trips >= 0.f) b->split_trips = trips;
+    if (min_left > 0) b->split_min_left = min_left;
+    b->split_extra = extra_helpers;
+    return b->kernel && b->split_inst ? HSR_OK : 1;
+}
 extern "C" int hsr_batch_solo_handovers(hsr_batch *b, int *out) {
     ENTER_DEV(b);
     if (!out) return fail(HSR_EINVAL, "null argument");
     const int rc = read_drained(b, out, b->ds.sq_ctl + 1, 1);
+    if (!b->handovers_counted) *out = 0;
     return rc ? rc : queue_error(b);
 }
 extern "C" int hsr_batch_set_queue(hsr_batch *b, int mode, int chunk) {
diff --git a/hsr_env_amd/csrc/host_batch.h b/hsr_env_amd/csrc/host_batch.h
--- a/hsr_env_amd/csrc/host_batch.h
+++ b/hsr_env_amd/csrc/host_batch.h
@@ -58,6 +58,13 @@
     bool queue_chunk_set = false;
     int solo_servers = 0;
     float solo_trips = 3.5f;
+    bool handovers_counted = false;
+    bool split_inst = false;
+    bool split = true;
+    int split_period = 8;
+    float split_trips = 2.5f;
+    int split_min_left = 40;
+    int split_extra = 0;
     bool kernel_log = false;
     std::vector<std::pair<hipEvent_t, hipEvent_t>> klog;
     float4 *d_planes = nullptr;
@@ -125,7 +132,6 @@
     if (b->cap_every <= 0 || b->cap_rows <= 0) return fail(HSR_EINVAL, "%s: no captured step (hsr_batch_set_capture, then a step)", who);
     return HSR_OK;
 }
-enum { QUEUE_ROUNDS = 64 };
 static inline dim3 grid1(size_t n, int t = 256) { return dim3((unsigned)((n + t - 1) / t)); }
 static int queue_error(hsr_batch *b) {
     int err = 0;
diff --git a/hsr_env_amd/csrc/host_create.h b/hsr_env_amd/csrc/host_create.h
--- a/hsr_env_amd/csrc/host_create.h
+++ b/hsr_env_amd/csrc/host_create.h
@@ -9,6 +9,10 @@
     b->sw.debug = set("HSR_DEBUG");
     if (set("HSR_SOLO")) b->solo_servers = atoi(env("HSR_SOLO"));
     if (atof(env("HSR_SOLO_TRIPS")) > 0) b->solo_trips = (float)atof(env("HSR_SOLO_TRIPS"));
+    if (set("HSR_SPLIT")) b->split = atoi(env("HSR_SPLIT")) != 0;
+    if (atoi(env("HSR_SPLIT_PERIOD")) > 0) b->split_period = atoi(env("HSR_SPLIT_PERIOD"));
+    if (set("HSR_SPLIT_TRIPS") && atof(env("HSR_SPLIT_TRIPS")) >= 0) b->split_trips = (float)atof(env("HSR_SPLIT_TRIPS"));
+    if (atoi(env("HSR_SPLIT_MIN_LEFT")) > 0) b->split_min_left = atoi(env("HSR_SPLIT_MIN_LEFT"));
     if (set("HSR_QUEUE")) b->queue = atoi(env("HSR_QUEUE")) != 0;
     if (atoi(env("HSR_QUEUE_CHUNK")) > 0) b->queue_chunk = atoi(env("HSR_QUEUE_CHUNK"));
     b->queue_chunk_set = atoi(env("HSR_QUEUE_CHUNK")) > 0;
@@ -23,18 +27,21 @@
     int group, nv;
     bool tg;
     persist_fn fn, sv;
+    bool split = false;
 };
+template <> struct SplitOf<DevModel_cfg3> : std::true_type {};
+template <> struct SplitOf<DevModel_cupboard> : std::true_type {};
 static const PersistInstance kPersistInstances[] = {
 #ifdef HSR_DEV_CFG3
-    {2, 16, -1, false, k_env_step_mf<16, 13, true, 7, false, DevModel_cfg3>, k_env_step_mf<16, 13, true, 7, false, DevModel_cfg3, true>},
+    {2, 16, -1, false, k_env_step_mf<16, 13, true, 7, false, DevModel_cfg3>, k_env_step_mf<16, 13, true, 7, false, DevModel_cfg3, true>, true},
 #else
     {0, 16, -1, false, k_env_step_mf<16, 2, true, 0, false, DevModel_cfg1>, nullptr},
     {1, 16, -1, false, k_env_step_mf<16, 8, true, 0, false, DevModel_cfg2>, k_env_step_mf<16, 8, true, 0, false, DevModel_cfg2, true>},
-    {2, 16, -1, false, k_env_step_mf<16, 13, true, 7, false, DevModel_cfg3>, k_env_step_mf<16, 13, true, 7, false, DevModel_cfg3, true>},
+    {2, 16, -1, false, k_env_step_mf<16, 13, true, 7, false, DevModel_cfg3>, k_env_step_mf<16, 13, true, 7, false, DevModel_cfg3, true>, true},
     {3, 32, -1, false, k_env_step_mf<32, 25, true, 7, false, DevModel_cfg4>, nullptr},
     {3, 32, -1, true, k_env_step_mf<32, 25, true, 7, true, DevModel_cfg4>, nullptr},
-    {4, 16, -1, false, k_env_step_mf<16, 13, true, -1, false, DevModel_cupboard>, k_env_step_mf<16, 13, true, -1, false, DevModel_cupboard, true>},
-    {4, 16, -1, true, k_env_step_mf<16, 13, true, -1, true, DevModel_cupboard>, k_env_step_mf<16, 13, true, -1, true, DevModel_cupboard, true>},
+    {4, 16, -1, false, k_env_step_mf<16, 13, true, -1, false, DevModel_cupboard>, k_env_step_mf<16, 13, true, -1, false, DevModel_cupboard, true>, true},
+    {4, 16, -1, true, k_env_step_mf<16, 13, true, -1, true, DevModel_cupboard>, k_env_step_mf<16, 13, true, -1, true, DevModel_cupboard, true>, true},
     {-1, 16, 13, false, k_env_step_mf<16, 13, true>, nullptr},
     {-1, 16, -1, false, k_env_step_mf<16, 16, false>, nullptr},
     {-1, 32, -1, false, k_env_step_mf<32, 32, false>, nullptr},
@@ -179,6 +186,7 @@
     if (!fits_persist(b, m) || !inst) { d.nfb = 0; return HSR_OK; }
     b->kernel = inst->fn;
     b->kernel_sv = inst->sv;
+    b->split_inst = inst->split;
     b->persist = true;
     for (persist_fn f : {b->kernel, b->kernel_sv})
         if (f && b->persist_lds_bytes > 48 * 1024) HIPCHK(hipFuncSetAttribute((const void *)f, hipFuncAttributeMaxDynamicSharedMemorySize, (int)b->persist_lds_bytes));
@@ -330,7 +338,7 @@
     if ((rc = dalloc(b, &s.phase_cyc, 32 + 40 * 8192))) return rc;
     if ((rc = dalloc(b, &s.capstat, 12))) return rc;
     if ((rc = dalloc(b, &s.trips, N))) return rc;
-    if ((rc = dalloc(b, &b->d_slot_env, N + 64))) return rc;
+    if ((rc = dalloc(b, &b->d_slot_env, 2 * (N + 64) + 4 * (size_t)SPLIT_MAX_EXTRA))) return rc;
     const size_t tasks = (N + 1) / 2;
     if ((rc = dalloc(b, &s.q_head, QUEUE_ROUNDS))) return rc;
     if ((rc = dalloc(b, &s.q_wpos, QUEUE_ROUNDS))) return rc;
@@ -338,8 +346,9 @@
     if ((rc = dalloc(b, &s.q_err, 1))) return rc;
     s.sq_cap = (int)N + 4096;
     if ((rc = dalloc(b, &s.sq_items, (size_t)s.sq_cap))) return rc;
-    if ((rc = dalloc(b, &s.sq_ctl, 4))) return rc;
+    if ((rc = dalloc(b, &s.sq_ctl, SPLIT_CTL_WORDS))) return rc;
     s.solo_servers = 0; s.solo_trips_x4 = 14; s.solo_min_left = 40;
+    s.split_period = 0; s.split_trips_x4 = 14; s.split_min_left = 40;
     s.q_chunk = 0;
     s.slot_env = nullptr;
     return HSR_OK;
diff --git a/hsr_env_amd/csrc/host_step.h b/hsr_env_amd/csrc/host_step.h
--- a/hsr_env_amd/csrc/host_step.h
+++ b/hsr_env_amd/csrc/host_step.h
@@ -68,36 +68,6 @@
     return upload_capture_desc(b, b->cap_every, b->cap_n);
 }
 
-struct PersistLaunch {
-    int tasks, grid;
-    int chunk, rounds;
-    int solo_servers, solo_trips_x4, solo_min_left;
-};
-static PersistLaunch plan_launch(int N, int group, int slots, int n_substeps, int queue, int queue_chunk, bool queue_chunk_set,
-                                 int solo_servers, float solo_trips, bool has_sv, bool schedule) {
-    PersistLaunch p{};
-    const int epb = 64 / group, T = (N + epb - 1) / epb;
-    int chunk = queue_chunk;
-    if (!queue_chunk_set && slots > 0 && T >= 4 * slots) chunk = 50;
-    while ((n_substeps + chunk - 1) / chunk > QUEUE_ROUNDS) chunk *= 2;
-    const bool solo = has_sv && solo_servers > 0 && solo_servers <= 4096 && schedule && slots > 0 && n_substeps >= 3 * chunk && n_substeps < 2048 && N <= (1 << 20)
-                      && (T + solo_servers <= slots || 4 * solo_servers <= slots);
-    const bool qon = slots > 0 && n_substeps >= 2 * chunk && (solo || queue == 1 || (queue < 0 && T > slots));
-    p.tasks = T;
-    p.grid = T;
-    p.chunk = chunk;
-    if (qon) {
-        p.rounds = (n_substeps + chunk - 1) / chunk;
-        p.grid = T < slots ? T : slots;
-        if (solo) {
-            p.solo_servers = solo_servers;
-            p.solo_trips_x4 = (int)(4.f * solo_trips + 0.5f);
-            p.solo_min_left = 2 * chunk;
-            p.grid = std::min(slots, T + solo_servers);
-        }
-    }
-    return p;
-}
 
 static int launch_persistent(hsr_batch *b, const StepIO &io, int n_substeps, int goal_body, float geofence) {
     hipStream_t st = b->stream;
@@ -109,14 +79,20 @@
     if (b->schedule)
         hipLaunchKernelGGL(k_schedule, dim3((b->N + SCHED_CHUNK - 1) / SCHED_CHUNK), dim3(1024), 0, st, b->ds, 64 / b->group, b->d_slot_env);
     const PersistLaunch p = plan_launch(b->N, b->group, b->slots, n_substeps, b->queue, b->queue_chunk, b->queue_chunk_set,
-                                        b->solo_servers, b->solo_trips, b->kernel_sv != nullptr, b->schedule);
+                                        b->solo_servers, b->solo_trips, b->kernel_sv != nullptr, b->schedule,
+                                        SplitSettings{b->split, b->split_inst, b->split_period, b->split_trips, b->split_min_left, b->split_extra});
     DevState dsl = b->ds;
+    b->handovers_counted = p.rounds > 0 || p.split.on;
     dsl.slot_env = b->schedule ? b->d_slot_env : nullptr;
     dsl.solo_servers = p.solo_servers;
     if (p.solo_servers > 0) { dsl.solo_trips_x4 = p.solo_trips_x4; dsl.solo_min_left = p.solo_min_left; }
     if (p.rounds > 0) {
         dsl.q_chunk = p.chunk;
         hipLaunchKernelGGL(k_queue_init, grid1((size_t)p.rounds * p.tasks), dim3(256), 0, st, dsl, p.tasks, p.rounds);
+    }
+    if (p.split.on) {
+        dsl.split_period = p.split.period; dsl.split_trips_x4 = p.split.trips_x4; dsl.split_min_left = p.split.min_left;
+        hipLaunchKernelGGL(k_split_init, dim3(8), dim3(256), 0, st, dsl);
     }
     hipEvent_t k0 = nullptr, k1 = nullptr;
     if (b->kernel_log) { hipEventCreate(&k0); hipEventCreate(&k1); hipEventRecord(k0, st); }
diff --git a/hsr_env_amd/csrc/hsrsim.hip b/hsr_env_amd/csrc/hsrsim.hip
--- a/hsr_env_amd/csrc/hsrsim.hip
+++ b/hsr_env_amd/csrc/hsrsim.hip
@@ -26,6 +26,7 @@
 #include "cfg_consts.h"
 
 #include "host_model.h"
+#include "launch_plan.h"
 #include "host_batch.h"
 #include "util_kernels.h"
 #include "host_create.h"
diff --git a/hsr_env_amd/csrc/launch_plan.h b/hsr_env_amd/csrc/launch_plan.h
--- /dev/null
+++ b/hsr_env_amd/csrc/launch_plan.h
@@ -0,0 +1,39 @@
+#pragma once
+#include "split_logic.h"
+
+enum { QUEUE_ROUNDS = 64 };
+
+struct PersistLaunch {
+    int tasks, grid;
+    int chunk, rounds;
+    int solo_servers, solo_trips_x4, solo_min_left;
+    SplitPlan split;
+};
+struct SplitSettings { bool on, const_instance; int period; float trips; int min_left, extra; };
+static inline PersistLaunch plan_launch(int N, int group, int slots, int n_substeps, int queue, int queue_chunk, bool queue_chunk_set,
+                                 int solo_servers, float solo_trips, bool has_sv, bool schedule, const SplitSettings &sp) {
+    PersistLaunch p{};
+    const int epb = 64 / group, T = (N + epb - 1) / epb;
+    int chunk = queue_chunk;
+    if (!queue_chunk_set && slots > 0 && T >= 4 * slots) chunk = 50;
+    while ((n_substeps + chunk - 1) / chunk > QUEUE_ROUNDS) chunk *= 2;
+    const bool solo = has_sv && solo_servers > 0 && solo_servers <= 4096 && schedule && slots > 0 && n_substeps >= 3 * chunk && n_substeps < 2048 && N <= (1 << 20)
+                      && (T + solo_servers <= slots || 4 * solo_servers <= slots);
+    const bool qon = slots > 0 && n_substeps >= 2 * chunk && (solo || queue == 1 || (queue < 0 && T > slots));
+    p.tasks = T;
+    p.grid = T;
+    p.chunk = chunk;
+    if (qon) {
+        p.rounds = (n_substeps + chunk - 1) / chunk;
+        p.grid = T < slots ? T : slots;
+        if (solo) {
+            p.solo_servers = solo_servers;
+            p.solo_trips_x4 = (int)(4.f * solo_trips + 0.5f);
+            p.solo_min_left = 2 * chunk;
+            p.grid = (slots < T + solo_servers ? slots : T + solo_servers);
+        }
+    }
+    p.split = split_plan(sp.on, group, sp.const_instance, schedule, qon, T, N, slots, n_substeps, sp.period, sp.trips, sp.min_left, sp.extra);
+    if (p.split.on) p.grid = T + p.split.extra;
+    return p;
+}
diff --git a/hsr_env_amd/csrc/model.h b/hsr_env_amd/csrc/model.h
--- a/hsr_env_amd/csrc/model.h
+++ b/hsr_env_amd/csrc/model.h
@@ -67,6 +67,7 @@
     int *q_head, *q_wpos, *q_items, *q_err;
     int solo_servers, solo_trips_x4, solo_min_left, sq_cap;
     int *sq_items, *sq_ctl;
+    int split_period, split_trips_x4, split_min_left;
     unsigned long long *capstat;
     unsigned long long *phase_cyc;
 };
diff --git a/hsr_env_amd/csrc/persist.h b/hsr_env_amd/csrc/persist.h
--- a/hsr_env_amd/csrc/persist.h
+++ b/hsr_env_amd/csrc/persist.h
@@ -3,6 +3,7 @@
 #include "kin2.h"
 #include "kin3.h"
 #include "solve_mf.h"
+#include "split_logic.h"
 
 template <int G> struct PersistLayout {
     int R, MS, oRows, oCnt, oB, envf, oPoly, oKin, oPair, oGeomC, oGeomS, oLinkTab, total;
@@ -66,6 +67,56 @@
     if (threadIdx.x == 0 && last && s.sq_ctl) __hip_atomic_fetch_add(&s.sq_ctl[3], 1, __ATOMIC_RELEASE, __HIP_MEMORY_SCOPE_AGENT);
 }
 
+enum { SPLIT_CLAIMED = 0, SPLIT_RESERVED = 1, SPLIT_CREDITS = 2, SPLIT_FINISHED = 3, SPLIT_STARTED = 4, SPLIT_CTL_WORDS = 8 };
+__device__ __forceinline__ unsigned split_acquire(const DevState &s, unsigned want) {
+    unsigned got = 0;
+    if (threadIdx.x == 0 && __hip_atomic_load(s.q_err, __ATOMIC_RELAXED, __HIP_MEMORY_SCOPE_AGENT) == 0) {
+        for (int j = 0; j < SPLIT_MAX_GROUPS; j++) {
+            if (!((want >> j) & 1u)) continue;
+            if (__hip_atomic_fetch_sub(&s.sq_ctl[SPLIT_CREDITS], 1, __ATOMIC_RELAXED, __HIP_MEMORY_SCOPE_AGENT) > 0) got |= 1u << j;
+            else { __hip_atomic_fetch_add(&s.sq_ctl[SPLIT_CREDITS], 1, __ATOMIC_RELAXED, __HIP_MEMORY_SCOPE_AGENT); break; }
+        }
+    }
+    return (unsigned)__builtin_amdgcn_readfirstlane((int)got);
+}
+__device__ __forceinline__ int split_wait(const DevState &s, bool no_task) {
+    auto uni = [](int v) { return __builtin_amdgcn_readfirstlane(v); };
+    const int lane = threadIdx.x;
+    if (lane == 0) __hip_atomic_fetch_add(&s.sq_ctl[SPLIT_CREDITS], 1, __ATOMIC_RELAXED, __HIP_MEMORY_SCOPE_AGENT);
+    int item = -1;
+    bool err = false;
+    for (int spins = 0;; spins++) {
+        if (spins > (1 << 18) || ((spins & 15) == 0 && uni(__hip_atomic_load(s.q_err, __ATOMIC_RELAXED, __HIP_MEMORY_SCOPE_AGENT)) != 0)) { err = true; break; }
+        const int ctl = __hip_atomic_load(&s.sq_ctl[lane & (SPLIT_CTL_WORDS - 1)], __ATOMIC_RELAXED, __HIP_MEMORY_SCOPE_AGENT);
+        const int h = __builtin_amdgcn_readlane(ctl, SPLIT_CLAIMED);
+        if (h < __builtin_amdgcn_readlane(ctl, SPLIT_RESERVED)) {
+            int won = 0;
+            if (lane == 0) { int expect = h; won = __hip_atomic_compare_exchange_strong(&s.sq_ctl[SPLIT_CLAIMED], &expect, h + 1, __ATOMIC_RELAXED, __ATOMIC_RELAXED, __HIP_MEMORY_SCOPE_AGENT) ? 1 : 0; }
+            if (!uni(won)) { __builtin_amdgcn_s_sleep(8); continue; }
+            for (int w = 0; h < s.sq_cap; w++) {
+                item = uni(__hip_atomic_load(&s.sq_items[h], __ATOMIC_RELAXED, __HIP_MEMORY_SCOPE_AGENT));
+                if (item >= 0) break;
+                __builtin_amdgcn_s_sleep(32);
+                if (w > (1 << 22) || uni(__hip_atomic_load(s.q_err, __ATOMIC_RELAXED, __HIP_MEMORY_SCOPE_AGENT)) != 0) { err = true; break; }
+            }
+            break;
+        }
+        if (__builtin_amdgcn_readlane(ctl, SPLIT_FINISHED) >= __builtin_amdgcn_readlane(ctl, SPLIT_STARTED) && !(no_task && __builtin_amdgcn_readlane(ctl, SPLIT_STARTED) == 0)) {
+            int gone = 0;
+            if (lane == 0) {
+                if (__hip_atomic_fetch_sub(&s.sq_ctl[SPLIT_CREDITS], 1, __ATOMIC_RELAXED, __HIP_MEMORY_SCOPE_AGENT) > 0) gone = 1;
+                else __hip_atomic_fetch_add(&s.sq_ctl[SPLIT_CREDITS], 1, __ATOMIC_RELAXED, __HIP_MEMORY_SCOPE_AGENT);
+            }
+            if (uni(gone)) break;
+        }
+        for (int k = 0; k < 4; k++) __builtin_amdgcn_s_sleep(127);
+    }
+    if (err) { if (lane == 0) __hip_atomic_store(s.q_err, 1, __ATOMIC_RELAXED, __HIP_MEMORY_SCOPE_AGENT); return -1; }
+    if (item >= 0) __builtin_amdgcn_fence(__ATOMIC_ACQUIRE, "agent");
+    return item;
+}
+
+template <class MT> struct SplitOf : std::false_type {};
 template <int G, int NVT, bool EXACT, int NDT = -1, bool TG = false, class MT = DevModel, bool SV = false>
 __global__ void __launch_bounds__(64, 2) k_env_step_mf(const DevModel *__restrict__ mp, DevState s, int n_substeps, int goal_body, float geofence, int flags, StepIO io) {
     const MT &m = *static_cast<const MT *>(mp);
@@ -79,6 +130,9 @@
     const bool hook_jv_per_contact = flags & 2, hook_majorant = flags & 4;
     const bool hook_dense_chol = flags & 128;
     constexpr bool EXACT_CT = EXACT && !std::is_same<MT, DevModel>::value;
+    constexpr bool SPLIT_INST = !SV && G == 16 && EXACT_CT && SplitOf<MT>::value;
+    const bool split_on = SPLIT_INST && s.split_period > 0 && s.q_chunk == 0 && s.slot_env != nullptr;
+    if (split_on && tid0 == 0 && (int)blockIdx.x < (N + EPB - 1) / EPB) __hip_atomic_fetch_add(&s.sq_ctl[SPLIT_STARTED], 1, __ATOMIC_RELAXED, __HIP_MEMORY_SCOPE_AGENT);
     const bool hook_no_item_list = flags & 64;
     const bool hook_ignore_stamps = flags & 16;
     const bool mpr_warm = !(flags & 8);
@@ -175,11 +229,16 @@
     PHASE_T0();
 
   constexpr bool HAS_SOLO = SV && EXACT && G == 16 && !std::is_same<MT, DevModel>::value;
+  int run_stop = 0;
   auto run_task = [&](auto solo_c, const int sub0, const int sub1, const int solo_env) {
     constexpr bool SOLO = decltype(solo_c)::value;
     constexpr bool REP = SOLO;
     (void)solo_env;
-    const bool first_run = sub0 == 0, last_run = sub1 >= n_substeps;
+    const bool first_run = sub0 == 0;
+    int sub_stop = sub1;
+    unsigned give = 0;
+    int split_check = split_on ? sub0 + s.split_period : -1;
+    (void)give; (void)split_check;
     const bool fresh = io.ctrl != nullptr && first_run;
     cap_con = cap_row = cap_item = nsub_run = own_trips = 0; bad_acc = trips_acc = 0; nsteps_e = 0;
     int run_trips = 0;
@@ -188,7 +247,9 @@
     bool list_ok = false;
     float acc_move = 0.f;
     {
-        PERSIST_LANE_VIEW(tid0)
+        int tid_r = tid0;
+        asm volatile("" : "+v"(tid_r));
+        PERSIST_LANE_VIEW(tid_r)
         if (c == 0) { sEnv[g] = e; sTick[g] = s.tick[e]; }
         done = !in_range || (fresh ? false : s.done[e] != 0);
         qpos_c = 0; qvel_c = 0; warm_c = 0;
@@ -205,11 +266,29 @@
 
     for (int sub = sub0; sub < sub1; sub++) {
         if (sub - sub0 >= 4 && 2 * trips_acc > 5 * (sub - sub0)) __builtin_amdgcn_s_setprio(3); else __builtin_amdgcn_s_setprio(0);
+        if constexpr (SPLIT_INST && !SOLO) {
+            if (sub == split_check) {
+                split_check += s.split_period;
+                int wt[EPB];
+#pragma unroll
+                for (int j = 0; j < EPB; j++) wt[j] = __builtin_amdgcn_readlane(run_trips, j * G);
+                run_trips = 0;
+                const unsigned long long ab = __ballot(!done && tid0 % G == 0);
+                unsigned alive = 0;
+#pragma unroll
+                for (int j = 0; j < EPB; j++) alive |= (unsigned)((ab >> (j * G)) & 1ull) << j;
+                const unsigned want = split_decide(wt, alive, EPB, sub, n_substeps - sub, s.split_period, s.split_trips_x4, s.split_min_left);
+                if (want) {
+                    give = split_acquire(s, want);
+                    if (give) sub_stop = sub;
+                }
+            }
+        }
         int tid_l = tid0;
         asm volatile("" : "+v"(tid_l));
         PERSIST_LANE_VIEW(tid_l)
         const bool valid = !done;
-        if (!wave_any(valid)) break;
+        if (!wave_any(valid) || give) break;
         if (valid && c == 0) sTick[g] += 1;
         int bad = 0;
         asm volatile("" ::: "memory");
@@ -599,8 +678,11 @@
             PHASE(18);
         }
     }
+    const bool last_run = sub_stop >= n_substeps;
     {
-    PERSIST_LANE_VIEW(tid0)
+    int tid_w = tid0;
+    asm volatile("" : "+v"(tid_w));
+    PERSIST_LANE_VIEW(tid_w)
     const int was_done = in_range ? s.done[e] : 0;
     if (in_range && (fresh || !(was_done != 0 && nsteps_e == 0))) {
         if (c < nq) s.qpos[(size_t)c * N + e] = qpos_c;
@@ -650,7 +732,23 @@
             }
         }
     }
-    }
+    if constexpr (SPLIT_INST && !SOLO) {
+        if (give) {
+            __builtin_amdgcn_fence(__ATOMIC_RELEASE, "agent");
+            __builtin_amdgcn_wave_barrier();
+            if (c == 0 && ((give >> g) & 1u)) {
+                const int pos = __hip_atomic_fetch_add(&s.sq_ctl[SPLIT_RESERVED], 1, __ATOMIC_RELAXED, __HIP_MEMORY_SCOPE_AGENT);
+                s.slot_env[task * EPB + g] = -1;
+                ENV_STAMP(1, e, (unsigned long long)sub_stop | (__builtin_amdgcn_s_memrealtime() << 16));
+                if (pos < s.sq_cap) __hip_atomic_store(&s.sq_items[pos], e | (sub_stop << 20), __ATOMIC_RELEASE, __HIP_MEMORY_SCOPE_AGENT);
+                else __hip_atomic_store(s.q_err, 1, __ATOMIC_RELAXED, __HIP_MEMORY_SCOPE_AGENT);
+            }
+            __threadfence_block();
+            wave_sync();
+        }
+    }
+    }
+    run_stop = sub_stop;
   };
   if (HAS_SOLO && s.q_chunk && s.solo_servers > 0 && (int)blockIdx.x < s.solo_servers) {
     if constexpr (HAS_SOLO) {
@@ -683,15 +781,37 @@
         if (threadIdx.x == 0) __hip_atomic_fetch_add(&s.sq_ctl[2], 1, __ATOMIC_RELAXED, __HIP_MEMORY_SCOPE_AGENT);
       }
     }
-  } else
+  } else {
+  const int n_tasks = (N + EPB - 1) / EPB;
+  bool helper = split_on && (int)blockIdx.x >= n_tasks;
+  int sub_next = 0;
   for (;;) {
     if (s.q_chunk) {
-        if (!q_claim(s, (N + EPB - 1) / EPB, (n_substeps + s.q_chunk - 1) / s.q_chunk, q_rlo, task, q_round)) break;
-    }
-    const int sub0 = s.q_chunk ? q_round * s.q_chunk : 0, sub1 = s.q_chunk ? min(n_substeps, sub0 + s.q_chunk) : n_substeps;
+        if (!q_claim(s, n_tasks, (n_substeps + s.q_chunk - 1) / s.q_chunk, q_rlo, task, q_round)) break;
+    } else if (helper) {
+        const int item = split_wait(s, (int)blockIdx.x >= n_tasks);
+        if (item < 0) break;
+        task = n_tasks + (int)blockIdx.x;
+        int tid_h = tid0;
+        asm volatile("" : "+v"(tid_h));
+        if (tid_h < EPB) s.slot_env[task * EPB + tid_h] = tid_h == 0 ? (item & 0xfffff) : -1;
+        __threadfence_block();
+        wave_sync();
+        sub_next = item >> 20;
+    }
+    const int sub0 = s.q_chunk ? q_round * s.q_chunk : sub_next, sub1 = s.q_chunk ? min(n_substeps, sub0 + s.q_chunk) : n_substeps;
     run_task(std::false_type{}, sub0, sub1, -1);
-    if (!s.q_chunk) break;
-    q_push(s, (N + EPB - 1) / EPB, task, q_round, sub1 >= n_substeps);
+    sub_next = run_stop;
+    if (s.q_chunk) { q_push(s, n_tasks, task, q_round, sub1 >= n_substeps); continue; }
+    if (!split_on) break;
+    if (sub_next < n_substeps) continue;
+    __builtin_amdgcn_s_setprio(0);
+    LIFE_WORK_END();
+    if (!helper) {
+        helper = true;
+        if (tid0 == 0) __hip_atomic_fetch_add(&s.sq_ctl[SPLIT_FINISHED], 1, __ATOMIC_RELAXED, __HIP_MEMORY_SCOPE_AGENT);
+    }
+  }
   }
     const int tid = tid0; (void)tid;
 #ifdef HSR_PHASE_TIMING
diff --git a/hsr_env_amd/csrc/solve_g.h b/hsr_env_amd/csrc/solve_g.h
--- a/hsr_env_amd/csrc/solve_g.h
+++ b/hsr_env_amd/csrc/solve_g.h
@@ -33,10 +33,11 @@
 #define PHASE(idx) do { const unsigned long long t_now_ = stamp_(); const unsigned int acc_ = (unsigned int)__builtin_amdgcn_readfirstlane((int)((unsigned int)__builtin_amdgcn_readlane((int)pt_v_, (idx)) + (unsigned int)(t_now_ - t_prev_))); asm volatile("v_writelane_b32 %0, %1, %2" : "+v"(pt_v_) : "s"(acc_), "i"(idx)); t_prev_ = t_now_; } while (0)
 #define PHASE_FLUSH() do { if (blockIdx.x < 8192 && pt_lane_ < 32) { unsigned long long *bt_ = s.phase_cyc + 32 + 40 * blockIdx.x; bt_[8 + pt_lane_] = (unsigned long long)pt_v_; if (pt_lane_ < 26) atomicAdd(&s.phase_cyc[pt_lane_], (unsigned long long)pt_v_); } if (tid == 0) { if (blockIdx.x < 8192) { unsigned long long *bt_ = s.phase_cyc + 32 + 40 * blockIdx.x; bt_[4] = dc_[0]; bt_[5] = dc_[1]; bt_[6] = dc_[2]; bt_[7] = dc_[3]; bt_[0] = r_first_; bt_[1] = __builtin_amdgcn_s_memrealtime(); bt_[2] = __builtin_amdgcn_s_getreg(63492); bt_[3] = __builtin_amdgcn_s_getreg(63508); } atomicAdd(&s.phase_cyc[26], stamp_() - t_first_); atomicAdd(&s.phase_cyc[27], __builtin_amdgcn_s_memrealtime() - r_first_); } } while (0)
 #elif defined(HSR_BLOCK_LIFE)
-#define PHASE_T0() unsigned long long dc_[4] = {0, 0, 0, 0}; const unsigned long long r_first_ = __builtin_amdgcn_s_memrealtime()
+#define PHASE_T0() unsigned long long dc_[4] = {0, 0, 0, 0}; unsigned long long r_last_ = 0; const unsigned long long r_first_ = __builtin_amdgcn_s_memrealtime()
+#define LIFE_WORK_END() do { r_last_ = __builtin_amdgcn_s_memrealtime(); } while (0)
 #define DBGCNT(i, v) do { dc_[i] += (v); } while (0)
 #define PHASE(idx) do {} while (0)
-#define PHASE_FLUSH() do { if (tid == 0 && blockIdx.x < 8192) { unsigned long long *bt_ = s.phase_cyc + 32 + 40 * blockIdx.x; bt_[0] = r_first_; bt_[1] = __builtin_amdgcn_s_memrealtime(); bt_[4] = dc_[0]; bt_[5] = dc_[1]; bt_[6] = dc_[2]; bt_[7] = dc_[3]; } } while (0)
+#define PHASE_FLUSH() do { if (tid == 0 && blockIdx.x < 8192) { unsigned long long *bt_ = s.phase_cyc + 32 + 40 * blockIdx.x; bt_[0] = r_first_; bt_[1] = r_last_ ? r_last_ : __builtin_amdgcn_s_memrealtime(); bt_[4] = dc_[0]; bt_[5] = dc_[1]; bt_[6] = dc_[2]; bt_[7] = dc_[3]; } } while (0)
 #define ENV_STAMP(slot, e, val) do { if ((e) < 8192) s.phase_cyc[32 + 40 * 4096 + 8192 * (slot) + (e)] = (val); } while (0)
 #else
 #define PHASE_T0() do {} while (0)
@@ -44,6 +45,9 @@
 #define DBGCNT(i, v) do {} while (0)
 #define PHASE(idx) do {} while (0)
 #define PHASE_FLUSH() do {} while (0)
+#endif
+#ifndef LIFE_WORK_END
+#define LIFE_WORK_END() do {} while (0)
 #endif
 #ifdef HSR_MPR_PROFILE
 #define HSR_SUBPROF 1
diff --git a/hsr_env_amd/csrc/split_logic.h b/hsr_env_amd/csrc/split_logic.h
--- /dev/null
+++ b/hsr_env_amd/csrc/split_logic.h
@@ -0,0 +1,47 @@
+#pragma once
+
+#ifdef __HIPCC__
+#define SPLIT_HD __host__ __device__
+#else
+#define SPLIT_HD
+#endif
+
+enum {
+    SPLIT_MAX_GROUPS = 4,
+    SPLIT_MAX_SUBSTEPS = 2048,
+    SPLIT_MAX_ENVS = 1 << 20,
+    SPLIT_MAX_EXTRA = 4096,
+};
+
+SPLIT_HD static inline unsigned split_decide(const int *trips, unsigned alive, int groups, int sub, int left, int period, int trips_x4, int min_left) {
+    if (period <= 0 || groups < 2 || groups > SPLIT_MAX_GROUPS || sub <= 0 || sub >= SPLIT_MAX_SUBSTEPS || left <= 0 || left < min_left) return 0u;
+    unsigned hard = 0u;
+    int nhard = 0, keep = -1;
+    for (int j = 0; j < groups; j++) {
+        if (!((alive >> j) & 1u) || 4 * trips[j] < trips_x4 * period) continue;
+        hard |= 1u << j;
+        nhard++;
+        if (keep < 0 || trips[j] > trips[keep]) keep = j;
+    }
+    return nhard >= 2 ? hard & ~(1u << keep) : 0u;
+}
+
+struct SplitPlan {
+    int on;
+    int extra;
+    int period, trips_x4, min_left;
+};
+static inline SplitPlan split_plan(int enabled, int group, int const_instance, int schedule, int queued, int tasks, int n_envs, int slots,
+                                   int n_substeps, int period, float trips, int min_left, int extra) {
+    SplitPlan p = {0, 0, 0, 0, 0};
+    if (!enabled || group != 16 || !const_instance || !schedule || queued) return p;
+    if (period < 1 || period >= SPLIT_MAX_SUBSTEPS || !(trips >= 0.f) || trips > 1000.f || min_left < 1 || extra < 0 || extra > SPLIT_MAX_EXTRA) return p;
+    if (tasks < 1 || n_envs > SPLIT_MAX_ENVS || n_substeps >= SPLIT_MAX_SUBSTEPS || n_substeps < period + min_left) return p;
+    if (slots <= 0 || tasks + extra > slots) return p;
+    p.on = 1;
+    p.extra = extra;
+    p.period = period;
+    p.trips_x4 = (int)(4.f * trips + 0.5f);
+    p.min_left = min_left;
+    return p;
+}
diff --git a/hsr_env_amd/csrc/util_kernels.h b/hsr_env_amd/csrc/util_kernels.h
--- a/hsr_env_amd/csrc/util_kernels.h
+++ b/hsr_env_amd/csrc/util_kernels.h
@@ -157,6 +157,11 @@
     if (s.solo_servers > 0) for (int k = i; k < s.sq_cap; k += gridDim.x * blockDim.x) s.sq_items[k] = -1;
     if (i < R * T) s.q_items[i] = i < T ? i : -1;
 }
+__global__ void k_split_init(DevState s) {
+    const int i = blockIdx.x * blockDim.x + threadIdx.x;
+    if (i < SPLIT_CTL_WORDS) s.sq_ctl[i] = 0;
+    for (int k = i; k < s.sq_cap; k += gridDim.x * blockDim.x) s.sq_items[k] = -1;
+}
 template <int J> __device__ __forceinline__ void sched_local_stage(unsigned (&v)[8], int tid, int k) {
     unsigned w[8];
 #pragma unroll
diff --git a/hsr_env_amd/sim.py b/hsr_env_amd/sim.py
--- a/hsr_env_amd/sim.py
+++ b/hsr_env_amd/sim.py
@@ -81,6 +81,7 @@
     "hsr_batch_set_debug": (_int, [_vp, _int]),
     "hsr_batch_set_solo": (_int, [_vp, _int, _float]),
     "hsr_batch_solo_handovers": (_int, [_vp, _ip]),
+    "hsr_batch_set_split": (_int, [_vp, _int, _int, _float, _int, _int]),
     "hsr_batch_set_schedule": (_int, [_vp, _int]),
     "hsr_batch_set_mpr_warm": (_int, [_vp, _int]),
     "hsr_batch_set_queue": (_int, [_vp, _int, _int]),
@@ -458,6 +459,12 @@
         _check(self._L, self._L.hsr_batch_solo_handovers(self._b, C.byref(out)))
         return int(out.value)
 
+    def set_split(self, on: bool, period: int = 0, trips: float = -1.0, min_left: int = 0, extra_helpers: int = 0) -> bool:
+        rc = self._L.hsr_batch_set_split(self._b, int(on), int(period), float(trips), int(min_left), int(extra_helpers))
+        if rc < 0:
+            _check(self._L, rc)
+        return rc == 0
+
     def set_schedule(self, on: bool):
         _check(self._L, self._L.hsr_batch_set_schedule(self._b, int(on)))
 
diff --git a/include/hsrsim.h b/include/hsrsim.h
--- a/include/hsrsim.h
+++ b/include/hsrsim.h
@@ -93,6 +93,7 @@
 int hsr_batch_set_debug(hsr_batch *b, int on);
 int hsr_batch_set_solo(hsr_batch *b, int servers, float trips);
 int hsr_batch_solo_handovers(hsr_batch *b, int *out);
+int hsr_batch_set_split(hsr_batch *b, int on, int period, float trips, int min_left, int extra_helpers);
 int hsr_batch_set_schedule(hsr_batch *b, int on);
 int hsr_batch_set_mpr_warm(hsr_batch *b, int on);
 int hsr_batch_set_queue(hsr_batch *b, int mode, int chunk);
```

Result: faster. 523,200 env-steps/s, median of 6 (+2.2%).
